# OpenDriveLab/kai0

Measured on AMD Instinct MI355X. Metric: train samples/sec pi0.5 full FT, higher is better.
Workload: dtype bf16; 1 GPU; pi0.5 full fine-tune bf16, batch 32 per MI355X, 3-cam 224x224 (BASELINE.json configs[1]); global_batch=32, seq_len=1018, parallelism=dp1

## Files before the change

### include/kai0hip.h

```cpp
#ifndef KAI0HIP_H
#define KAI0HIP_H

#include <stdint.h>

#ifdef __cplusplus
extern "C" {
#endif

typedef void* kai0_stream_t;

const char* kai0_last_error(void);
int kai0_abi_version(void);
int kai0_device_info(int device, int* n_cu, int* lds_bytes, char* arch_name64);

typedef struct kai0_gemm_desc {
    const void* A;
    const void* B;
    void* C;
    int32_t M, N, K;
    int32_t a_kc, b_kc;
    int64_t lda, ldb, ldc;
    int32_t batch, batch_inner;
    int64_t sA1, sA2, sB1, sB2, sC1, sC2;
    int32_t a_rpb, b_rpb, c_rpb, _pad0;
    int64_t a_bs, a_off, b_bs, b_off, c_bs, c_off;
    const void* bias;
    int32_t bias_f32;
    float scale;
    int32_t act;
    int32_t out_f32;
    void* pre_out;
    const void* gate;
    int32_t gate_rpb;
    int32_t accumulate;
    int64_t gate_ld;
    const void* residual;
    int64_t ldr;
    int64_t sR1, sR2;
    int32_t split_k;
    int32_t c_nontemporal;
    void* workspace;
    int64_t workspace_bytes;
    const void* aux1;
    const void* aux2;
    int32_t nseg, _pad2;
    struct {
        void* dst;
        int64_t ld;
        int32_t n_begin, _pad;
    } seg[3];
    const float* rowvec;
    int64_t rv_s1, rv_s2, rv_ld;
    const void* B2;
    void* pre_out2;
    void* norm_out;
    const void* norm_w;
    const void* norm_b;
    float norm_eps;
    int32_t norm_kind;
    const void* rope_cos;
    const void* rope_sin;
    int32_t rope_half, rope_n_end;
    int32_t persist, general_epilogue, small_w8, _pad3;
} kai0_gemm_desc;

int kai0_gemm_bf16(const kai0_gemm_desc* d, kai0_stream_t stream);
int kai0_gemm_desc_size(void);

#define KAI0_GEMM_LOOP_PLAIN2 0
#define KAI0_GEMM_LOOP_PLAIN4 1
#define KAI0_GEMM_LOOP_QUADRANT 2
#define KAI0_GEMM_LOOP_RING 3
#define KAI0_GEMM_LOOP_PERSISTENT 4
typedef struct kai0_gemm_plan_t {
    int32_t tile;
    int32_t waves;
    int32_t loop;
    int32_t tiles_m, tiles_n;
    int32_t k_chunk;
    int32_t simple_epilogue;
    int32_t _pad;
} kai0_gemm_plan_t;
int kai0_gemm_plan(const kai0_gemm_desc* d, kai0_gemm_plan_t* out);
int kai0_gemm_plan_size(void);

typedef struct kai0_skinny_seg {
    void* dst;
    int64_t ld;
    int32_t n_begin, n_end;
    int32_t rope, _pad;
} kai0_skinny_seg;

typedef struct kai0_skinny_desc {
    const void* A;
    const void* W;
    int64_t lda, ldw;
    int32_t M, N, K;
    int32_t pair_stride, mode, split_k;
    int32_t a_rpb, c_rpb;
    int64_t a_bs, a_off, c_bs, c_off;
    kai0_skinny_seg seg[3];
    int32_t nseg, gate_rpb;
    const void* gate;
    int64_t gate_ld;
    const void* residual;
    int64_t ldr;
    const float* rope_cos;
    const float* rope_sin;
    int32_t rope_half;
    int32_t w_packed;
    void* workspace;
    int64_t workspace_bytes;
    const float* mod;
    int64_t mod_ld;
    int32_t mod_rpb;
    float eps;
    const float* rowsq_in;
    const float* cvec;
    int32_t rowsq_parts, _pad2;
    int64_t rowsq_ld;
    float* rowsq_out;
    int64_t rowsq_out_ld;
} kai0_skinny_desc;

int kai0_gemm_skinny_bf16(const kai0_skinny_desc* d, kai0_stream_t stream);
int kai0_skinny_desc_size(void);
int64_t kai0_skinny_workspace_bytes(int M, int N, int split_k);
int kai0_attn_decode(const void* Q, const void* K, const void* Vt, void* O, const int32_t* qcode, const int32_t* kcode,
                     int batch, int rows, int H, int HD, int Sk, int q0, int64_t q_bs, int64_t k_bs, int64_t k_ld,
                     int k_rows, int64_t vt_bs, int64_t vt_ld, int64_t qcode_ld, int64_t kcode_ld, float scale,
                     void* workspace, int64_t workspace_bytes, kai0_stream_t stream);
int kai0_attn_bwd_dq(const void* dO, const void* O, const void* P, const void* K, const void* V, void* dS, void* dQ, int batch,
                     int rows, int Sk, int HD, int64_t ldo, int64_t ldk, int64_t ldv, int64_t ldp, int64_t sO, int64_t sK,
                     int64_t sV, int64_t sP, float scale, kai0_stream_t stream);
typedef struct kai0_attn_bwd_desc {
    const void* dO; const void* O; const void* Q; const void* K; const void* V;
    const float* lse; const int32_t* qcode; const int32_t* kcode;
    void* P; void* dS; void* dQ;
    int32_t batch, rows, Sk, HD, H, _pad0;
    int64_t ldo, ldk, ldv, ldp, sO, sK, sV, sP, s_lse, qcode_ld, kcode_ld;
    float scale; int32_t _pad1;
} kai0_attn_bwd_desc;
int kai0_attn_bwd_dq2(const kai0_attn_bwd_desc* d, kai0_stream_t stream);
int kai0_attn_bwd_desc_size(void);
int64_t kai0_attn_decode_workspace_bytes(int batch, int rows);
int kai0_transpose_strided_bf16(const void* src, void* dst, int R, int C, int64_t src_ld, int64_t dst_ld, int batch,
                                int64_t src_bs, int64_t dst_bs, kai0_stream_t stream);

int kai0_rope_table(const int32_t* pos, const float* inv_freq, void* cos_out, void* sin_out, int64_t rows, int half, int out_bf16,
                    kai0_stream_t stream);
int kai0_prefix_codes(const void* const* img_masks, int ncam, const void* lang_mask, int B, int n_img, int T, int Hs, int32_t* qcode,
                      int32_t* kcode, int32_t* pos, kai0_stream_t stream);
int kai0_prefix_state_codes(const void* const* img_masks, int ncam, const void* lang_mask, int B, int n_img, int T, int n_state, int Hs,
                            int32_t* qcode, int32_t* kcode, int32_t* pos, kai0_stream_t stream);

int kai0_gemm_f32(const float* A, int64_t sam, int64_t sak, const float* B, int64_t sbk, int64_t sbn,
                  float* C, int64_t ldc, int M, int N, int K, const float* bias, int accumulate, int split_k,
                  void* workspace, int64_t workspace_bytes, kai0_stream_t stream);
int64_t kai0_gemm_f32_workspace_bytes(int M, int N, int split_k);

int kai0_linear_rows_f32(const float* x, const float* W, const float* bias, float* out, int64_t ldo, int M, int N, int K,
                         kai0_stream_t stream);

int kai0_rmsnorm_fwd(const void* x, const float* w, void* y, float* rstd, int64_t rows, int D, float eps,
                     kai0_stream_t stream);
int kai0_rmsnorm_bwd(const void* dy, const void* x, const float* w, const float* rstd, void* dx,
                     float* dw_partial, int dw_blocks, const void* dres, int64_t rows, int D, kai0_stream_t stream);
int kai0_adarms_fwd(const void* x, const float* mod, void* y, void* gate_out, float* rstd, int64_t rows,
                    int rows_per_batch, int D, float eps, kai0_stream_t stream);
int kai0_adarms_bwd(const void* dy, const void* dgate, const void* x, const float* mod, const float* rstd,
                    void* dx, float* dmod, const void* dres, int64_t rows, int rows_per_batch, int D,
                    kai0_stream_t stream);
int kai0_adarms_combine(const float* partials, int splits, int64_t split_stride, const void* gate_prev,
                        const void* residual, void* x_out, const float* mod, void* y, void* gate_out, int64_t rows,
                        int rows_per_batch, int D, float eps, kai0_stream_t stream);
int kai0_layernorm_fwd(const void* x, const void* w, const void* b, void* y, float* mean, float* rstd,
                       int64_t rows, int D, float eps, kai0_stream_t stream);
int kai0_layernorm_bwd(const void* dy, const void* x, const void* w, const float* mean, const float* rstd,
                       void* dx, float* dwb_partial, int dwb_blocks, const void* dres, int64_t rows, int D,
                       kai0_stream_t stream);
int kai0_reduce_partials(const float* partial, int blocks, int ncols, int64_t ld, void* out, int out_f32,
                         kai0_stream_t stream);
typedef struct kai0_reduce_item {
    const float* partial;
    void* out;
    int64_t ld;
    int32_t blocks, ncols;
    int32_t out_f32, _pad;
} kai0_reduce_item;
int kai0_reduce_partials_batch(const kai0_reduce_item* items, int n, kai0_stream_t stream);
int kai0_colsum_partials_bf16(const void* dy, int64_t M, int N, int64_t ld, float* scratch, int scratch_blocks,
                              int* blocks_used, kai0_stream_t stream);
int kai0_colsum_bf16(const void* dy, int64_t M, int N, int64_t ld, float* scratch, int scratch_blocks,
                     void* out, int out_f32, kai0_stream_t stream);

int kai0_rope_inplace(void* x, const int32_t* pos, const float* inv_freq, int B, int S, int64_t s_ld_rows,
                      int64_t row0, int H, int HD, int inverse, kai0_stream_t stream);
int kai0_rope_inplace2(void* x, int H, void* x2, int H2, const int32_t* pos, const float* inv_freq, int B, int S,
                       int64_t s_ld_rows, int64_t row0, int HD, kai0_stream_t stream);
int kai0_rope_copy(const void* src, void* dst, const int32_t* pos, const float* inv_freq, int B, int S, int H, int HD,
                   int64_t src_bs, int64_t src_ld, int64_t dst_bs, int64_t dst_ld, int64_t pos_bs, int inverse,
                   kai0_stream_t stream);

int kai0_softmax_mask_fwd(const void* scores, void* probs, const int32_t* qcode, const int32_t* kcode,
                          int B, int Sq, int H, int Sk, int64_t ld, int64_t batch_stride, int q0,
                          int64_t qcode_ld, int64_t kcode_ld, kai0_stream_t stream);
int kai0_siglip_attn_bwd(const void* q, const void* k, const void* v, const void* dO, const void* O, const void* P,
                         void* dq, void* dk, void* dv, int n_img, int S, int NH, int HD, int64_t ldp, int64_t ld_grad,
                         float scale, kai0_stream_t stream);
int kai0_siglip_attn_fwd(const void* q, const void* k, const void* v, void* o, float* lse, int n_img, int S, int NH, int HD,
                         int64_t ldq, int64_t ldk, int64_t ldv, int64_t ldo, int64_t sq, int64_t sk, int64_t sv, int64_t so,
                         float scale, kai0_stream_t stream);
int kai0_siglip_attn_bwd2(const void* q, const void* k, const void* v, const void* dO, const void* O, const float* lse,
                          void* dq, void* dk, void* dv, int n_img, int S, int NH, int HD, int64_t ld_grad, float scale,
                          kai0_stream_t stream);
int kai0_rowdot_bf16(const void* a, const void* b, float* out, int64_t rows, int D, kai0_stream_t stream);
int kai0_softmax_bwd(const void* probs, const void* dprobs, int dprobs_f32, void* dscores, int64_t rows, int Sk,
                     int64_t ld, float scale, kai0_stream_t stream);

typedef struct kai0_attn_desc {
    const void* Q; const void* K; const void* V; void* O; void* P;
    const int32_t* qcode; const int32_t* kcode;
    int32_t rows, Sk, HD, H, q0, batch, batch_inner, _pad0;
    int64_t ldq, ldk, ldv, ldo, ldp;
    int64_t sQ1, sQ2, sK1, sK2, sV1, sV2, sO1, sO2, sP;
    int64_t qcode_ld, kcode_ld;
    float scale;
    int32_t online;
    float* lse;
    int64_t s_lse;
} kai0_attn_desc;
int kai0_attn_fwd(const kai0_attn_desc* d, kai0_stream_t stream);
int kai0_attn_combine(const void* o_parts, const float* lse_parts, void* O, int parts, int rows, int HD, int64_t ldo,
                      int64_t part_stride, int64_t lse_stride, kai0_stream_t stream);
// ... 113 lines not shown
```

### kai0_amd/_lib.py

```python

from __future__ import annotations

import ctypes as C
import os
import pathlib

_HERE = pathlib.Path(__file__).resolve().parent
LIB_PATH = _HERE / "lib" / "libkai0hip.so"
ABI_VERSION = 2

c_p = C.c_void_p
c_i = C.c_int
c_i64 = C.c_int64
c_f = C.c_float


class GemmSeg(C.Structure):
    _fields_ = [("dst", c_p), ("ld", c_i64), ("n_begin", C.c_int32), ("_pad", C.c_int32)]


class GemmDesc(C.Structure):

    _fields_ = [
        ("A", c_p), ("B", c_p), ("C", c_p),
        ("M", C.c_int32), ("N", C.c_int32), ("K", C.c_int32),
        ("a_kc", C.c_int32), ("b_kc", C.c_int32),
        ("lda", c_i64), ("ldb", c_i64), ("ldc", c_i64),
        ("batch", C.c_int32), ("batch_inner", C.c_int32),
        ("sA1", c_i64), ("sA2", c_i64), ("sB1", c_i64), ("sB2", c_i64), ("sC1", c_i64), ("sC2", c_i64),
        ("a_rpb", C.c_int32), ("b_rpb", C.c_int32), ("c_rpb", C.c_int32), ("_pad0", C.c_int32),
        ("a_bs", c_i64), ("a_off", c_i64), ("b_bs", c_i64), ("b_off", c_i64), ("c_bs", c_i64), ("c_off", c_i64),
        ("bias", c_p), ("bias_f32", C.c_int32), ("scale", c_f),
        ("act", C.c_int32), ("out_f32", C.c_int32),
        ("pre_out", c_p), ("gate", c_p), ("gate_rpb", C.c_int32), ("accumulate", C.c_int32),
        ("gate_ld", c_i64), ("residual", c_p), ("ldr", c_i64), ("sR1", c_i64), ("sR2", c_i64),
        ("split_k", C.c_int32), ("c_nontemporal", C.c_int32), ("workspace", c_p), ("workspace_bytes", c_i64),
        ("aux1", c_p), ("aux2", c_p),
        ("nseg", C.c_int32), ("_pad2", C.c_int32), ("seg", GemmSeg * 3),
        ("rowvec", c_p), ("rv_s1", c_i64), ("rv_s2", c_i64), ("rv_ld", c_i64),
        ("B2", c_p), ("pre_out2", c_p),
        ("norm_out", c_p), ("norm_w", c_p), ("norm_b", c_p), ("norm_eps", C.c_float), ("norm_kind", C.c_int32),
        ("rope_cos", c_p), ("rope_sin", c_p), ("rope_half", C.c_int32), ("rope_n_end", C.c_int32),
        ("persist", C.c_int32), ("general_epilogue", C.c_int32), ("small_w8", C.c_int32), ("_pad3", C.c_int32),
    ]


class GemmPlan(C.Structure):

    _fields_ = [("tile", C.c_int32), ("waves", C.c_int32), ("loop", C.c_int32), ("tiles_m", C.c_int32), ("tiles_n", C.c_int32),
                ("k_chunk", C.c_int32), ("simple_epilogue", C.c_int32), ("_pad", C.c_int32)]


GEMM_LOOPS = ("plain2", "plain4", "quadrant", "ring", "persistent")


class AttnDesc(C.Structure):

    _fields_ = [
        ("Q", c_p), ("K", c_p), ("V", c_p), ("O", c_p), ("P", c_p), ("qcode", c_p), ("kcode", c_p),
        ("rows", C.c_int32), ("Sk", C.c_int32), ("HD", C.c_int32), ("H", C.c_int32), ("q0", C.c_int32),
        ("batch", C.c_int32), ("batch_inner", C.c_int32), ("_pad0", C.c_int32),
        ("ldq", c_i64), ("ldk", c_i64), ("ldv", c_i64), ("ldo", c_i64), ("ldp", c_i64),
        ("sQ1", c_i64), ("sQ2", c_i64), ("sK1", c_i64), ("sK2", c_i64), ("sV1", c_i64), ("sV2", c_i64),
        ("sO1", c_i64), ("sO2", c_i64), ("sP", c_i64), ("qcode_ld", c_i64), ("kcode_ld", c_i64),
        ("scale", c_f), ("online", C.c_int32), ("lse", c_p), ("s_lse", c_i64),
    ]


class AttnBwdDesc(C.Structure):

    _fields_ = [
        ("dO", c_p), ("O", c_p), ("Q", c_p), ("K", c_p), ("V", c_p), ("lse", c_p), ("qcode", c_p), ("kcode", c_p),
        ("P", c_p), ("dS", c_p), ("dQ", c_p),
        ("batch", C.c_int32), ("rows", C.c_int32), ("Sk", C.c_int32), ("HD", C.c_int32), ("H", C.c_int32), ("_pad0", C.c_int32),
        ("ldo", c_i64), ("ldk", c_i64), ("ldv", c_i64), ("ldp", c_i64), ("sO", c_i64), ("sK", c_i64), ("sV", c_i64), ("sP", c_i64),
        ("s_lse", c_i64), ("qcode_ld", c_i64), ("kcode_ld", c_i64),
        ("scale", c_f), ("_pad1", C.c_int32),
    ]


class SkinnySeg(C.Structure):
    _fields_ = [("dst", c_p), ("ld", c_i64), ("n_begin", C.c_int32), ("n_end", C.c_int32), ("rope", C.c_int32),
                ("_pad", C.c_int32)]


class ReduceItem(C.Structure):

    _fields_ = [("partial", c_p), ("out", c_p), ("ld", c_i64), ("blocks", C.c_int32), ("ncols", C.c_int32),
                ("out_f32", C.c_int32), ("_pad", C.c_int32)]


class PackPart(C.Structure):

    _fields_ = [("src", c_p), ("dst", c_p), ("src_bs", c_i64), ("src_ld", c_i64), ("dst_bs", c_i64), ("dst_ld", c_i64),
                ("B", C.c_int32), ("rows", C.c_int32), ("cols", C.c_int32), ("mode", C.c_int32), ("pos_off", C.c_int32),
                ("_pad", C.c_int32)]


class SkinnyDesc(C.Structure):

    _fields_ = [
        ("A", c_p), ("W", c_p), ("lda", c_i64), ("ldw", c_i64),
        ("M", C.c_int32), ("N", C.c_int32), ("K", C.c_int32),
        ("pair_stride", C.c_int32), ("mode", C.c_int32), ("split_k", C.c_int32),
        ("a_rpb", C.c_int32), ("c_rpb", C.c_int32),
        ("a_bs", c_i64), ("a_off", c_i64), ("c_bs", c_i64), ("c_off", c_i64),
        ("seg", SkinnySeg * 3), ("nseg", C.c_int32), ("gate_rpb", C.c_int32),
        ("gate", c_p), ("gate_ld", c_i64), ("residual", c_p), ("ldr", c_i64),
        ("rope_cos", c_p), ("rope_sin", c_p), ("rope_half", C.c_int32), ("w_packed", C.c_int32),
        ("workspace", c_p), ("workspace_bytes", c_i64),
        ("mod", c_p), ("mod_ld", c_i64), ("mod_rpb", C.c_int32), ("eps", c_f),
        ("rowsq_in", c_p), ("cvec", c_p), ("rowsq_parts", C.c_int32), ("_pad2", C.c_int32), ("rowsq_ld", c_i64),
        ("rowsq_out", c_p), ("rowsq_out_ld", c_i64),
    ]


_PROTOS: dict[str, list] = {
    "kai0_abi_version": [],
    "kai0_gemm_desc_size": [],
    "kai0_device_info": [c_i, C.POINTER(c_i), C.POINTER(c_i), C.c_char_p],
    "kai0_gemm_bf16": [C.POINTER(GemmDesc), c_p],
    "kai0_gemm_plan": [C.POINTER(GemmDesc), C.POINTER(GemmPlan)],
    "kai0_gemm_plan_size": [],
    "kai0_attn_fwd": [C.POINTER(AttnDesc), c_p],
    "kai0_attn_desc_size": [],
    "kai0_attn_combine": [c_p, c_p, c_p, c_i, c_i, c_i, c_i64, c_i64, c_i64, c_p],
    "kai0_attn_bwd_dq2": [C.POINTER(AttnBwdDesc), c_p],
    "kai0_attn_bwd_desc_size": [],
    "kai0_siglip_attn_fwd": [c_p, c_p, c_p, c_p, c_p, c_i, c_i, c_i, c_i, c_i64, c_i64, c_i64, c_i64, c_i64, c_i64, c_i64, c_i64, c_f, c_p],
    "kai0_siglip_attn_bwd2": [c_p, c_p, c_p, c_p, c_p, c_p, c_p, c_p, c_p, c_i, c_i, c_i, c_i, c_i64, c_f, c_p],
    "kai0_gemm_skinny_bf16": [C.POINTER(SkinnyDesc), c_p],
    "kai0_skinny_desc_size": [],
    "kai0_attn_decode": [c_p, c_p, c_p, c_p, c_p, c_p, c_i, c_i, c_i, c_i, c_i, c_i, c_i64, c_i64, c_i64, c_i, c_i64, c_i64,
                         c_i64, c_i64, c_f, c_p, c_i64, c_p],
    "kai0_attn_bwd_dq": [c_p, c_p, c_p, c_p, c_p, c_p, c_p, c_i, c_i, c_i, c_i, c_i64, c_i64, c_i64, c_i64, c_i64, c_i64, c_i64, c_i64,
                         c_f, c_p],
    "kai0_transpose_strided_bf16": [c_p, c_p, c_i, c_i, c_i64, c_i64, c_i, c_i64, c_i64, c_p],
    "kai0_rope_table": [c_p, c_p, c_p, c_p, c_i64, c_i, c_i, c_p],
    "kai0_prefix_codes": [c_p, c_i, c_p, c_i, c_i, c_i, c_i, c_p, c_p, c_p, c_p],
    "kai0_prefix_state_codes": [c_p, c_i, c_p, c_i, c_i, c_i, c_i, c_i, c_p, c_p, c_p, c_p],
    "kai0_gemm_f32": [c_p, c_i64, c_i64, c_p, c_i64, c_i64, c_p, c_i64, c_i, c_i, c_i, c_p, c_i, c_i, c_p, c_i64, c_p],
    "kai0_linear_rows_f32": [c_p, c_p, c_p, c_p, c_i64, c_i, c_i, c_i, c_p],
    "kai0_rmsnorm_fwd": [c_p, c_p, c_p, c_p, c_i64, c_i, c_f, c_p],
    "kai0_rmsnorm_bwd": [c_p, c_p, c_p, c_p, c_p, c_p, c_i, c_p, c_i64, c_i, c_p],
    "kai0_adarms_fwd": [c_p, c_p, c_p, c_p, c_p, c_i64, c_i, c_i, c_f, c_p],
    "kai0_adarms_combine": [c_p, c_i, c_i64, c_p, c_p, c_p, c_p, c_p, c_p, c_i64, c_i, c_i, c_f, c_p],
    "kai0_adarms_bwd": [c_p, c_p, c_p, c_p, c_p, c_p, c_p, c_p, c_i64, c_i, c_i, c_p],
    "kai0_layernorm_fwd": [c_p, c_p, c_p, c_p, c_p, c_p, c_i64, c_i, c_f, c_p],
    "kai0_layernorm_bwd": [c_p, c_p, c_p, c_p, c_p, c_p, c_p, c_i, c_p, c_i64, c_i, c_p],
    "kai0_reduce_partials": [c_p, c_i, c_i, c_i64, c_p, c_i, c_p],
    "kai0_colsum_bf16": [c_p, c_i64, c_i, c_i64, c_p, c_i, c_p, c_i, c_p],
    "kai0_reduce_partials_batch": [c_p, c_i, c_p],
    "kai0_pack_rows": [c_p, c_i, c_p, c_i64, c_p, c_i, c_p],
    "kai0_sampled_checksum": [c_p, c_i, c_i, c_p, c_p],
    "kai0_colsum_partials_bf16": [c_p, c_i64, c_i, c_i64, c_p, c_i, c_p, c_p],
    "kai0_rope_inplace": [c_p, c_p, c_p, c_i, c_i, c_i64, c_i64, c_i, c_i, c_i, c_p],
    "kai0_rope_inplace2": [c_p, c_i, c_p, c_i, c_p, c_p, c_i, c_i, c_i64, c_i64, c_i, c_p],
    "kai0_rope_copy": [c_p, c_p, c_p, c_p, c_i, c_i, c_i, c_i, c_i64, c_i64, c_i64, c_i64, c_i64, c_i, c_p],
    "kai0_softmax_mask_fwd": [c_p, c_p, c_p, c_p, c_i, c_i, c_i, c_i, c_i64, c_i64, c_i, c_i64, c_i64, c_p],
    "kai0_siglip_attn_bwd": [c_p, c_p, c_p, c_p, c_p, c_p, c_p, c_p, c_p, c_i, c_i, c_i, c_i, c_i64, c_i64, c_f, c_p],
    "kai0_rowdot_bf16": [c_p, c_p, c_p, c_i64, c_i, c_p],
    "kai0_softmax_bwd": [c_p, c_p, c_i, c_p, c_i64, c_i, c_i64, c_f, c_p],
    "kai0_geglu_fwd": [c_p, c_p, c_p, c_i64, c_p],
    "kai0_geglu_bwd": [c_p, c_p, c_p, c_p, c_p, c_i64, c_p],
    "kai0_gelu_bwd": [c_p, c_p, c_p, c_i64, c_p],
    "kai0_silu_fwd_f32": [c_p, c_p, c_i64, c_p],
    "kai0_silu_bwd_f32": [c_p, c_p, c_p, c_i64, c_p],
    "kai0_gated_fwd": [c_p, c_p, c_p, c_p, c_i64, c_i, c_i, c_p],
    "kai0_gated_bwd": [c_p, c_p, c_p, c_p, c_p, c_i64, c_i, c_i, c_p],
    "kai0_embed_gather": [c_p, c_p, c_p, c_i, c_i, c_i, c_f, c_i64, c_i64, c_i64, c_p],
    "kai0_embed_grad": [c_p, c_p, c_p, c_i, c_i, c_i, c_f, c_i64, c_i64, c_i64, c_p],
    "kai0_cast_f32_to_bf16": [c_p, c_p, c_i64, c_p],
    "kai0_cast_bf16_to_f32": [c_p, c_p, c_i64, c_p],
    "kai0_add_bf16": [c_p, c_p, c_p, c_i64, c_p],
    "kai0_add_f32": [c_p, c_p, c_p, c_i64, c_p],
    "kai0_transpose_bf16": [c_p, c_p, c_i, c_i, c_p],
    "kai0_copy_rows_bf16": [c_p, c_p, c_i, c_i, c_i, c_i64, c_i64, c_i64, c_i64, c_i64, c_i64, c_p],
    "kai0_patch_im2col": [c_p, c_p, c_i, c_i, c_i, c_i, c_p],
    "kai0_add_pos_cast": [c_p, c_p, c_p, c_i64, c_i, c_i, c_p],
    "kai0_time_sincos": [c_p, c_p, c_i, c_i, C.c_double, C.c_double, c_p],
    "kai0_flow_mix": [c_p, c_p, c_p, c_p, c_p, c_i, c_i, c_p],
    "kai0_mse_fwd": [c_p, c_p, c_p, c_i64, c_p],
    "kai0_mse_bwd": [c_p, c_p, c_p, c_p, c_i64, c_p],
    "kai0_euler_step": [c_p, c_p, c_f, c_i64, c_p],
    "kai0_denoise_glue": [c_p, c_p, c_i64, c_i, c_f, c_p, c_p, c_p, c_f, c_p, c_p, c_p, c_i64, c_i, c_i, c_p, c_p],
    "kai0_denoise_glue_rows": [c_p, c_p, c_i64, c_i, c_f, c_p, c_p, c_p, c_f, c_p, c_p, c_p, c_i64, c_i, c_i, c_p, c_i, c_i64, c_i64, c_p],
    "kai0_linear_f32_rows": [c_p, c_i64, c_p, c_i64, c_p, c_i, c_i, c_i, c_i, c_p, c_i64, c_p, c_i64, c_i, c_i64, c_i64, c_p, c_i64, c_p],
    "kai0_rtc_error": [c_p, c_p, c_p, c_p, c_i, c_f, c_p, c_i64, c_i, c_i, c_p],
    "kai0_rtc_update": [c_p, c_p, c_p, c_p, c_f, c_f, c_f, c_i64, c_i, c_p],
    "kai0_sumsq": [c_p, c_i, c_i64, c_p, c_p, c_p],
    "kai0_sum_chunks": [c_p, c_i, c_i, c_i64, c_i64, c_p, c_p],
    "kai0_clip_coef": [c_p, c_f, c_p, c_p, c_p],
    "kai0_adamw": [c_p, c_p, c_p, c_p, c_i, c_p, c_i, c_i64, c_f, c_f, c_f, c_f, c_f, c_f, c_f, c_p, c_p],
    "kai0_adamw_rows": [c_p, c_p, c_p, c_p, c_i, c_p, c_i, c_i64, c_i, c_p, c_f, c_f, c_f, c_f, c_f, c_f, c_f, c_p, c_p],
    "kai0_adamw_ema": [c_p, c_p, c_p, c_p, c_p, c_i, c_p, c_i, c_i64, c_f, c_f, c_f, c_f, c_f, c_f, c_f, c_f, c_p, c_p],
    "kai0_adamw_rows_ema": [c_p, c_p, c_p, c_p, c_p, c_i, c_p, c_i, c_i64, c_i, c_p, c_f, c_f, c_f, c_f, c_f, c_f, c_f, c_f, c_p, c_p],
    "kai0_grad_accum": [c_p, c_p, c_i, c_i64, c_i, c_p, c_p, c_p],
    "kai0_mix": [C.POINTER(c_p), c_i, C.POINTER(c_f), c_i, c_p, c_i, c_i64, c_p],
    "kai0_multi_dot": [c_p, c_i, C.POINTER(c_p), c_i, c_i, c_i64, c_p, c_p, c_p],
    "kai0_lora_down": [c_p, c_i64, c_p, c_i64, c_p, c_i64, c_i, c_i, c_i, c_p],
    "kai0_lora_wgrad": [c_p, c_i64, c_p, c_i64, c_p, c_i64, c_i, c_i, c_i, c_f, c_i, c_i, c_p, c_i64, c_p],
    "kai0_frames_to_chw": [c_p, c_p, c_i, c_i, c_i, c_i, c_i, c_i, c_i, c_i, c_i, c_p],
    "kai0_prefix_gather": [c_p, c_p, c_p, c_p, c_i, c_i, c_i, c_i, c_i, c_i64, c_p],
# ... 65 lines not shown
```

### kai0_amd/csrc/gemm_bf16.hip

```cpp
#include "common.h"
#include "../../include/kai0hip.h"
#include <stdlib.h>
#include <algorithm>
#include <atomic>
#include <type_traits>

namespace {

constexpr int BK = 64;

#ifdef KAI0_ABLATE
#define KAI0_ABL(p) ((p).ablate)
#else
#define KAI0_ABL(p) 0
#endif

struct RowMap {
    int32_t rpb;
    int64_t bs, off;
    __device__ __forceinline__ int64_t operator()(int r) const {
        if (rpb == 0) return r;
        const int q = r / rpb;
        return (int64_t)q * bs + (r - q * rpb) + off;
    }
};

struct GemmArgs {
    const bf16_t* A;
    const bf16_t* B;
    void* C;
    int M, N, K;
    int64_t lda, ldb, ldc;
    int batch_inner;
    int64_t sA1, sA2, sB1, sB2, sC1, sC2;
    RowMap amap, bmap, cmap;
    const void* bias;
    int bias_f32;
    float scale;
    int act;
    int out_f32;
    bf16_t* pre_out;
    const bf16_t* aux1;
    const bf16_t* aux2;
    const bf16_t* gate;
    int gate_rpb;
    int accumulate;
    int64_t gate_ld;
    const bf16_t* residual;
    int64_t ldr, sR1, sR2;
    int tiles_m, tiles_n;
    int ablate;
    int nt_c;
    int simple_epi;
    int nt_pre;
    const float* rowvec;
    int64_t rv_s1, rv_s2, rv_ld;
    int nseg;
    bf16_t* seg_dst[3];
    int64_t seg_ld[3];
    int seg_begin[3];
    float* ws;
    int split_k, k_chunk;
    const bf16_t* B2;
    bf16_t* pre_out2;
    bf16_t* norm_out;
    const void* norm_w;
    const bf16_t* norm_b;
    float norm_eps;
    int norm_kind;
    const bf16_t* rope_cos;
    const bf16_t* rope_sin;
    int rope_half, rope_n_end;
};

typedef __attribute__((ext_vector_type(4))) int i32x4_t;
constexpr uint32_t OOB = 0x80000000u;
__device__ __forceinline__ void glds16(__amdgpu_buffer_rsrc_t rsrc, uint32_t voff, char* lds_dst_wave_uniform) {
    __builtin_amdgcn_raw_ptr_buffer_load_lds(rsrc, (LDS_PTR(void))lds_dst_wave_uniform, 16, (int)voff, 0, 0, 0);
}


__device__ __forceinline__ void store_pre8(bf16_t* dst, bf16x8 v, int nt) {
    if (nt) __builtin_nontemporal_store(v, reinterpret_cast<bf16x8*>(dst));
    else *reinterpret_cast<bf16x8*>(dst) = v;
}

__device__ __forceinline__ void epilogue8(const GemmArgs& p, float (&v)[8], int row, int ccol, int64_t cz, int64_t rz,
                                          int64_t vz, void* cbase, bool raw_f32, const bf16x8* res_pre = nullptr) {
    const bool rnd = !raw_f32;
    auto R = [rnd](float x) { return rnd ? rbf(x) : x; };
    const int64_t orow = p.cmap(row);
    if (p.act == 4) {
        const bf16x8 pv = *reinterpret_cast<const bf16x8*>(p.aux1 + cz + orow * p.ldc + ccol);
        const float dsum = p.rowvec[vz + (int64_t)row * p.rv_ld];
        bf16x8 ov;
#pragma unroll
        for (int e = 0; e < 8; ++e) ov[e] = f2bf((bf2f(pv[e]) * (v[e] - dsum)) * p.scale);
        *reinterpret_cast<bf16x8*>(reinterpret_cast<bf16_t*>(cbase) + cz + orow * p.ldc + ccol) = ov;
        return;
    }
    if (p.bias != nullptr) {
        if (p.bias_f32) {
            const float* bp = reinterpret_cast<const float*>(p.bias) + ccol;
#pragma unroll
            for (int e = 0; e < 8; ++e) v[e] += bp[e];
        } else {
            bf16x8 bv = *reinterpret_cast<const bf16x8*>(reinterpret_cast<const bf16_t*>(p.bias) + ccol);
#pragma unroll
            for (int e = 0; e < 8; ++e) v[e] += bf2f(bv[e]);
        }
    }
#pragma unroll
    for (int e = 0; e < 8; ++e) v[e] = R(v[e]);
    if (p.scale != 1.0f) {
#pragma unroll
        for (int e = 0; e < 8; ++e) v[e] = R(v[e] * p.scale);
    }
    if (p.act == 1) {
        if (p.pre_out != nullptr) {
            bf16x8 pv;
#pragma unroll
            for (int e = 0; e < 8; ++e) pv[e] = f2bf(v[e]);
            store_pre8(p.pre_out + cz + orow * p.ldc + ccol, pv, p.nt_pre);
        }
#pragma unroll
        for (int e = 0; e < 8; e += 2) {
            const f32x2 a = gelu_tanh2(f32x2{v[e], v[e + 1]});
            v[e] = R(a[0]);
            v[e + 1] = R(a[1]);
        }
    } else if (p.act == 2) {
        if (p.pre_out != nullptr) {
            bf16x8 uv;
#pragma unroll
            for (int e = 0; e < 8; ++e) uv[e] = f2bf(v[e]);
            *reinterpret_cast<bf16x8*>(p.pre_out + cz + orow * p.ldc + ccol) = uv;
        }
        const bf16x8 gv = *reinterpret_cast<const bf16x8*>(p.aux1 + cz + orow * p.ldc + ccol);
#pragma unroll
        for (int e = 0; e < 8; e += 2) {
            const f32x2 a = gelu_tanh2(f32x2{bf2f(gv[e]), bf2f(gv[e + 1])});
            v[e] = R(R(a[0]) * v[e]);
            v[e + 1] = R(R(a[1]) * v[e + 1]);
        }
    } else if (p.act == 3) {
        const bf16x8 gv = *reinterpret_cast<const bf16x8*>(p.aux1 + cz + orow * p.ldc + ccol);
        const bf16x8 uv = *reinterpret_cast<const bf16x8*>(p.aux2 + cz + orow * p.ldc + ccol);
        bf16x8 du;
#pragma unroll
        for (int e = 0; e < 8; e += 2) {
            f32x2 gl, gr;
            gelu_tanh_both2(f32x2{bf2f(gv[e]), bf2f(gv[e + 1])}, gl, gr);
            du[e] = f2bf(v[e] * R(gl[0]));
            du[e + 1] = f2bf(v[e + 1] * R(gl[1]));
            v[e] = R(R(v[e] * bf2f(uv[e])) * gr[0]);
            v[e + 1] = R(R(v[e + 1] * bf2f(uv[e + 1])) * gr[1]);
        }
        *reinterpret_cast<bf16x8*>(p.pre_out + cz + orow * p.ldc + ccol) = du;
    } else if (p.act == 5) {
        const bf16x8 pv = *reinterpret_cast<const bf16x8*>(p.aux1 + cz + orow * p.ldc + ccol);
#pragma unroll
        for (int e = 0; e < 8; e += 2) {
            f32x2 gl, gr;
            gelu_tanh_both2(f32x2{bf2f(pv[e]), bf2f(pv[e + 1])}, gl, gr);
            v[e] = R(v[e] * gr[0]);
            v[e + 1] = R(v[e + 1] * gr[1]);
        }
    }
    if (p.gate != nullptr) {
        bf16x8 gv = *reinterpret_cast<const bf16x8*>(p.gate + (int64_t)(row / p.gate_rpb) * p.gate_ld + ccol);
#pragma unroll
        for (int e = 0; e < 8; ++e) v[e] = R(v[e] * bf2f(gv[e]));
    }
    if (p.residual != nullptr) {
        bf16x8 rv = res_pre != nullptr ? *res_pre : *reinterpret_cast<const bf16x8*>(p.residual + rz + orow * p.ldr + ccol);
#pragma unroll
        for (int e = 0; e < 8; ++e) v[e] = R(v[e] + bf2f(rv[e]));
    }
    if (raw_f32) {
        float* cp = reinterpret_cast<float*>(cbase) + cz + orow * p.ldc + ccol;
        if (p.accumulate) {
            f32x4 o0 = *reinterpret_cast<const f32x4*>(cp);
            f32x4 o1 = *reinterpret_cast<const f32x4*>(cp + 4);
#pragma unroll
            for (int e = 0; e < 4; ++e) { v[e] += o0[e]; v[4 + e] += o1[e]; }
        }
        *reinterpret_cast<f32x4*>(cp) = f32x4{v[0], v[1], v[2], v[3]};
        *reinterpret_cast<f32x4*>(cp + 4) = f32x4{v[4], v[5], v[6], v[7]};
    } else {
        bf16_t* cp = reinterpret_cast<bf16_t*>(cbase) + cz + orow * p.ldc + ccol;
        if (p.nseg > 0) {
            int si = 0;
            if (p.nseg > 1 && ccol >= p.seg_begin[1]) si = 1;
            if (p.nseg > 2 && ccol >= p.seg_begin[2]) si = 2;
            cp = p.seg_dst[si] + orow * p.seg_ld[si] + (ccol - p.seg_begin[si]);
        }
        if (p.accumulate) {
            bf16x8 ov = *reinterpret_cast<const bf16x8*>(cp);
#pragma unroll
            for (int e = 0; e < 8; ++e) v[e] += bf2f(ov[e]);
        }
        bf16x8 ov;
#pragma unroll
        for (int e = 0; e < 8; ++e) ov[e] = f2bf(v[e]);
        store_pre8(cp, ov, p.nt_c);
    }
}

#define N_ALIGNED8(n) (((n) & 7) == 0)

#define SIMPLE_EPILOGUE_APPLIES(simple_epi, act, split_k, gate, out_f32, scale, c_rpb, n) \
    ((simple_epi) && (act) <= 1 && (split_k) == 1 && (gate) == nullptr && !(out_f32) && (scale) == 1.0f && (c_rpb) == 0 && (N_ALIGNED8(n)))

__device__ __forceinline__ void lds_barrier() {
    __builtin_amdgcn_sched_barrier(0);
    asm volatile("s_waitcnt lgkmcnt(0)" ::: "memory");
    __builtin_amdgcn_s_barrier();
    asm volatile("" ::: "memory");
    __builtin_amdgcn_sched_barrier(0);
}

template <bool A_KC, bool B_KC, int WM, int WN, int MT, int NT, bool PP, int NS = 2, int BKT = 64, int SCH = 0>
__global__ __launch_bounds__(WM * WN * 64, (WM * WN * 64) / 256) void gemm_bf16_kernel(const GemmArgs p) {
    static_assert(PP ? (WM == 2 && WN == 4 && MT == 8 && ((SCH == 1 && NS == 2 && BKT == 64) || (SCH == 3 && NS == 4 && BKT == 32)))
                     : (SCH == 0 && NS >= 2 && BKT == 64),
                  "K loops: plain multi-stage (SCH 0, 64 deep), quadrant (SCH 1: 256x256x64, 2 stages), ring (SCH 3: 256x256x32, 4 slots)");
    constexpr int BK = BKT;
    constexpr int NWAVES = WM * WN;
    constexpr int TBM = WM * MT * 16, TBN = WN * NT * 16;
    constexpr int A_TILE = TBM * BK * 2, B_TILE = TBN * BK * 2;
    constexpr int STAGE = A_TILE + B_TILE;
    constexpr int NA = A_TILE / 1024 / NWAVES;
    constexpr int NB = B_TILE / 1024 / NWAVES;
    constexpr int KC_CPR = BK / 8;
    constexpr int KC_RPP = 64 / KC_CPR;
    constexpr int A_ROWB = TBM * 2, B_ROWB = TBN * 2;
    constexpr int A_LPR = A_ROWB / 16, B_LPR = B_ROWB / 16;
    constexpr int A_RPP = 64 / A_LPR, B_RPP = 64 / B_LPR;
    constexpr int GROUP = TBM == 128 ? 8 : 4;
    static_assert(NA >= 1 && NB >= 1 && NT == 4 && ((MT % 4) == 0 || MT == 2), "unsupported tile configuration");
    constexpr int AH = MT >= 4 ? 4 : MT;
    static_assert(A_KC || (64 % A_LPR) == 0, "contraction-strided A needs a power-of-two tile height");
    extern __shared__ __attribute__((aligned(16))) char smem[];

    const int tid = threadIdx.x;
    const int lane = tid & 63;
    const int wave = __builtin_amdgcn_readfirstlane(tid >> 6);
    const int wm = wave / WN, wn = wave % WN;
    if constexpr (MT <= 4) {
        asm volatile("" ::"s"(p.A), "s"(p.B), "s"(p.M), "s"(p.N), "s"(p.K), "s"(p.lda), "s"(p.ldb), "s"(p.tiles_m), "s"(p.tiles_n),
                     "s"(p.split_k), "s"(p.k_chunk), "s"(p.batch_inner), "s"(p.amap.rpb), "s"(p.bmap.rpb), "s"(p.act), "s"(p.sA1),
                     "s"(p.sB1), "s"(p.sA2), "s"(p.sB2));
    }
    const int nwg = gridDim.x;
    int pid = blockIdx.x;
    {
        const int q = nwg >> 3, r = nwg & 7;
        const int xcd = pid & 7, idx = pid >> 3;
        pid = (xcd < r ? xcd * (q + 1) : r * (q + 1) + (xcd - r) * q) + idx;
    }
    int tile_m, tile_n;
    {
        const int width = GROUP * p.tiles_n;
        const int group = pid / width;
        const int first_m = group * GROUP;
        const int gsz = min(p.tiles_m - first_m, GROUP);
        const int in_g = pid - group * width;
        tile_m = first_m + in_g % gsz;
        tile_n = in_g / gsz;
    }
    const int ks_id = blockIdx.y % p.split_k;
    const int z = blockIdx.y / p.split_k;
    const int kbeg = ks_id * p.k_chunk;
    const int kend = min(p.K, kbeg + p.k_chunk);
    const int z1 = z / p.batch_inner, z2 = z - z1 * p.batch_inner;
    const bf16_t* __restrict__ Ab = p.A + z1 * p.sA1 + z2 * p.sA2;
    const bf16_t* __restrict__ Bb = p.B + z1 * p.sB1 + z2 * p.sB2;
    const int m0 = tile_m * TBM, n0 = tile_n * TBN;
    const __amdgpu_buffer_rsrc_t a_rsrc = __builtin_amdgcn_make_buffer_rsrc((void*)Ab, 0, (int)OOB, 0x00020000);
    const __amdgpu_buffer_rsrc_t b_rsrc = __builtin_amdgcn_make_buffer_rsrc((void*)Bb, 0, (int)OOB, 0x00020000);
    const bool pair = p.act == 6;
    const __amdgpu_buffer_rsrc_t b2_rsrc = __builtin_amdgcn_make_buffer_rsrc((void*)(pair ? p.B2 : Bb), 0, (int)OOB, 0x00020000);

    uint32_t a_off[NA], b_off[NB];
    const int kc_chunk = BK == 64 ? ((lane & 7) ^ (lane >> 3)) * 8 : ((lane & 3) ^ (((lane >> 2) & 8) ? 3 : 0)) * 8;
    if constexpr (A_KC) {
#pragma unroll
        for (int j = 0; j < NA; ++j) {
            const int R = m0 + (wave * NA + j) * KC_RPP + lane / KC_CPR;
            a_off[j] = R < p.M ? (uint32_t)((p.amap(R) * p.lda + kc_chunk) * 2) : OOB;
        }
    } else {
#pragma unroll
        for (int j = 0; j < NA; ++j) {
            const int r = (wave * NA + j) * A_RPP + lane / A_LPR;
            const int key = (r & 3) | (((r >> 3) & 1) << 2);
            const int col = m0 + ((lane % A_LPR) ^ (key << 1)) * 8;
            a_off[j] = col < p.M ? (uint32_t)(col * 2) : OOB;
        }
    }
    if constexpr (B_KC) {
#pragma unroll
        for (int j = 0; j < NB; ++j) {
            const int rt = (wave * NB + j) * KC_RPP + lane / KC_CPR;
            int R = n0 + rt;
            bool ok = R < p.N;
            if (pair) {
                R = (n0 >> 1) + ((rt >> 6) << 5) + (rt & 31);
                ok = R < (p.N >> 1);
            }
            b_off[j] = ok ? (uint32_t)((p.bmap(R) * p.ldb + kc_chunk) * 2) : OOB;
        }
    } else {
#pragma unroll
        for (int j = 0; j < NB; ++j) {
            const int r = (wave * NB + j) * B_RPP + lane / B_LPR;
            const int key = (r & 3) | (((r >> 3) & 1) << 2);
            const int col = n0 + ((lane % B_LPR) ^ (key << 1)) * 8;
            b_off[j] = col < p.N ? (uint32_t)(col * 2) : OOB;
        }
    }
    const uint32_t lda2 = (uint32_t)p.lda * 2, ldb2 = (uint32_t)p.ldb * 2;

    auto stage = [&](int kt, int slot) {
        char* sa = smem + slot * STAGE + wave * (NA * 1024);
        char* sb = smem + slot * STAGE + A_TILE + wave * (NB * 1024);
        const int k0 = kbeg + kt * BK;
        const bool kc_in = (k0 + kc_chunk) < kend;
#pragma unroll
        for (int j = 0; j < NA; ++j) {
            uint32_t off;
            if constexpr (A_KC) {
                off = kc_in ? a_off[j] + (uint32_t)k0 * 2 : OOB;
            } else {
                const int kr = k0 + (wave * NA + j) * A_RPP + lane / A_LPR;
                off = kr < kend ? a_off[j] + (uint32_t)p.amap(kr) * lda2 : OOB;
            }
            glds16(a_rsrc, off, sa + j * 1024);
        }
#pragma unroll
        for (int j = 0; j < NB; ++j) {
            uint32_t off;
            if constexpr (B_KC) {
                off = kc_in ? b_off[j] + (uint32_t)k0 * 2 : OOB;
            } else {
                const int kr = k0 + (wave * NB + j) * B_RPP + lane / B_LPR;
                off = kr < kend ? b_off[j] + (uint32_t)p.bmap(kr) * ldb2 : OOB;
            }
            glds16((B_KC && BK == 64 && pair && (((wave * NB + j) * KC_RPP) & 32)) ? b2_rsrc : b_rsrc, off, sb + j * 1024);
        }
    };

    auto piece_off = [&](int kt, int idx) -> uint32_t {
        const int k0 = kbeg + kt * BK;
        const bool kc_in = (k0 + kc_chunk) < kend;
        if (idx < NA) {
            if constexpr (A_KC) {
                return kc_in ? a_off[idx] + (uint32_t)k0 * 2 : OOB;
            } else {
                const int kr = k0 + (wave * NA + idx) * A_RPP + lane / A_LPR;
                return kr < kend ? a_off[idx] + (uint32_t)p.amap(kr) * lda2 : OOB;
            }
        } else {
            const int j = idx - NA;
            if constexpr (B_KC) {
                return kc_in ? b_off[j] + (uint32_t)k0 * 2 : OOB;
            } else {
                const int kr = k0 + (wave * NB + j) * B_RPP + lane / B_LPR;
                return kr < kend ? b_off[j] + (uint32_t)p.bmap(kr) * ldb2 : OOB;
            }
        }
    };
    auto piece_issue = [&](uint32_t off, int slot, int idx) {
        if (idx < NA) glds16(a_rsrc, off, smem + slot * STAGE + wave * (NA * 1024) + idx * 1024);
        else glds16(b_rsrc, off, smem + slot * STAGE + A_TILE + wave * (NB * 1024) + (idx - NA) * 1024);
    };
// ... 105 lines not shown
                    hb_lds[x] = h * 16384 + q * 1024;
                    hb_kr[x] = r;
                    hb_off[x] = col < p.N ? (uint32_t)(col * 2) : OOB;
                }
            }
        auto issue_half = [&](bool isb, int h, int t) {
            const int k0 = kbeg + t * BK;
            const bool kc_in = (k0 + kc_chunk) < kend;
            char* base = smem + (t & 1) * STAGE + (isb ? A_TILE : 0);
#pragma unroll
            for (int j = 0; j < 2; ++j) {
                const int x = h * 2 + j;
                const uint32_t o = isb ? hb_off[x] : ha_off[x];
                uint32_t off = OOB;
                if (isb ? B_KC : A_KC) {
                    if (kc_in && o != OOB) off = o + (uint32_t)k0 * 2;
                } else {
                    const int kr = k0 + (isb ? hb_kr[x] : ha_kr[x]);
                    if (kr < kend && o != OOB) off = o + (uint32_t)(isb ? p.bmap(kr) : p.amap(kr)) * (isb ? ldb2 : lda2);
                }
                if (KAI0_ABL(p) == 1) off = OOB;
                glds16(isb ? ((pair && h == 1) ? b2_rsrc : b_rsrc) : a_rsrc, off, base + (isb ? hb_lds[x] : ha_lds[x]));
            }
        };
        issue_half(false, 0, 0);
        issue_half(true, 1, 0);
        issue_half(true, 0, 0);
        issue_half(false, 1, 0);
        issue_half(false, 0, 1);
        issue_half(true, 1, 1);
        asm volatile("s_waitcnt vmcnt(6)" ::: "memory");
        lds_barrier();
        if (grp == 1) lds_barrier();
        bf16x8 af[4][2], bq[2][2];
        auto read_a = [&](const char* ta, int h) {
#pragma unroll
            for (int i = 0; i < 4; ++i)
#pragma unroll
                for (int ks = 0; ks < 2; ++ks)
                    af[i][ks] = A_KC ? load_frag(ta, true, A_ROWB, wm * 128 + (h * 4 + i) * 16, ks)
                                     : load_frag(ta + h * 16384, false, 256, wm * 64 + i * 16, ks);
        };
        auto read_b = [&](const char* tb, int h) {
#pragma unroll
            for (int j = 0; j < 2; ++j)
#pragma unroll
                for (int ks = 0; ks < 2; ++ks)
                    bq[j][ks] = B_KC ? load_frag(tb, true, B_ROWB, wn * 64 + (h * 2 + j) * 16, ks)
                                     : load_frag(tb + h * 16384, false, 256, wn * 32 + j * 16, ks);
        };
        auto quad = [&](auto ahc, auto bhc) {
            constexpr int ah = decltype(ahc)::value, bh = decltype(bhc)::value;
            __builtin_amdgcn_s_setprio(1);
#pragma unroll
            for (int ks = 0; ks < 2; ++ks)
#pragma unroll
                for (int i = 0; i < 4; ++i)
#pragma unroll
                    for (int j = 0; j < 2; ++j)
                        acc[ah * 4 + i][bh * 2 + j] =
                            __builtin_amdgcn_mfma_f32_16x16x32_bf16(af[i][ks], bq[j][ks], acc[ah * 4 + i][bh * 2 + j], 0, 0, 0);
            __builtin_amdgcn_s_setprio(0);
        };
        using I0 = std::integral_constant<int, 0>;
        using I1 = std::integral_constant<int, 1>;
        for (int t = 0; t < nk; ++t) {
            const char* ta = smem + (t & 1) * STAGE;
            const char* tb = ta + A_TILE;
            read_b(tb, 0);
            __builtin_amdgcn_sched_barrier(0);
            read_a(ta, 0);
            __builtin_amdgcn_sched_barrier(0);
            issue_half(true, 0, t + 1);
            lds_barrier();
            quad(I0{}, I0{});
            lds_barrier();
            read_b(tb, 1);
            __builtin_amdgcn_sched_barrier(0);
            issue_half(false, 1, t + 1);
            asm volatile("s_waitcnt vmcnt(8)" ::: "memory");
            lds_barrier();
            quad(I0{}, I1{});
            lds_barrier();
            read_a(ta, 1);
            __builtin_amdgcn_sched_barrier(0);
            issue_half(false, 0, t + 2);
            lds_barrier();
            quad(I1{}, I1{});
            lds_barrier();
            read_b(tb, 0);
            __builtin_amdgcn_sched_barrier(0);
            issue_half(true, 1, t + 2);
            asm volatile("s_waitcnt vmcnt(6)" ::: "memory");
            lds_barrier();
            quad(I1{}, I0{});
            lds_barrier();
        }
        asm volatile("s_waitcnt vmcnt(0)" ::: "memory");
        if (grp == 0) lds_barrier();
        lds_barrier();
    } else {
#pragma unroll
        for (int st = 0; st < NS - 1; ++st)
            if (st < nk) stage(st, st);
        int slot_c = 0, slot_p = NS - 1;
        for (int kt = 0; kt < nk; ++kt) {
            if constexpr (NS == 2) {
                asm volatile("s_waitcnt vmcnt(0)" ::: "memory");
            } else {
                if (kt + NS - 2 < nk) asm volatile("s_waitcnt vmcnt(%0)" ::"n"((NS - 2) * (NA + NB)) : "memory");
                else asm volatile("s_waitcnt vmcnt(0)" ::: "memory");
            }
            lds_barrier();
            if (kt + NS - 1 < nk && KAI0_ABL(p) != 1) stage(kt + NS - 1, slot_p);
            const char* ta = smem + slot_c * STAGE;
            const char* tb = ta + A_TILE;
    #pragma unroll
            for (int ks = 0; ks < BK / 32; ++ks) {
                bf16x8 bfr[NT];
    #pragma unroll
                for (int t = 0; t < NT; ++t) bfr[t] = load_frag(tb, B_KC, B_ROWB, wn * (NT * 16) + t * 16, ks);
    #pragma unroll
                for (int h = 0; h < MT / AH; ++h) {
                    bf16x8 af[AH];
    #pragma unroll
                    for (int t = 0; t < AH; ++t) af[t] = load_frag(ta, A_KC, A_ROWB, wm * (MT * 16) + (h * AH + t) * 16, ks);
    #pragma unroll
                    for (int i = 0; i < AH; ++i)
    #pragma unroll
                        for (int j = 0; j < NT; ++j)
                            acc[h * AH + i][j] = __builtin_amdgcn_mfma_f32_16x16x32_bf16(af[i], bfr[j], acc[h * AH + i][j], 0, 0, 0);
                }
            }
            slot_c = slot_c + 1 == NS ? 0 : slot_c + 1;
            slot_p = slot_p + 1 == NS ? 0 : slot_p + 1;
        }
        lds_barrier();
    }

    float* slab = reinterpret_cast<float*>(smem + wave * (AH * 4096));
    const int64_t cz = z1 * p.sC1 + z2 * p.sC2;
    const int64_t rz = z1 * p.sR1 + z2 * p.sR2;
    const int64_t vz = z1 * p.rv_s1 + z2 * p.rv_s2;
    constexpr bool ILM = SCH == 1 && !A_KC, ILN = SCH == 1 && !B_KC;
    const int ccol = ILN ? n0 + ((lane & 7) >> 2) * 128 + wn * 32 + ((lane & 7) & 3) * 8 : n0 + wn * 64 + (lane & 7) * 8;
    auto row_base = [&](int h) { return ILM ? m0 + h * 128 + wm * 64 : m0 + wm * (MT * 16) + h * 64; };
    const bool col_ok = ccol < ((p.N + 7) & ~7);
    const bool fused_fast = p.act >= 2 && p.split_k == 1 && p.bias == nullptr && p.gate == nullptr && p.residual == nullptr &&
                            !p.accumulate && !p.out_f32 && p.nseg == 0 && (p.act == 4 || p.scale == 1.0f) &&
                            (p.act != 3 || p.pre_out != nullptr);
    const bool plain_fast = p.act <= 1 && p.split_k == 1 && (p.bias != nullptr || p.residual != nullptr) && p.gate == nullptr &&
                            !p.accumulate && !p.out_f32 && p.nseg == 0 && (N_ALIGNED8(p.N));
    const bool simple_fast = MT == 8 && SIMPLE_EPILOGUE_APPLIES(p.simple_epi, p.act, p.split_k, p.gate, p.out_f32, p.scale, p.cmap.rpb, p.N);
    auto epi_half = [&](auto hc) {
        constexpr int h = decltype(hc)::value;
        if constexpr (((MT == 4 && WM == 2) || (MT == 2 && WM == 4)) && WN == 2 && A_KC && B_KC) if (p.act == 7) {
            const bool rot = n0 < p.rope_n_end;
            const int fi = ((n0 >> 7) & 1) * 64 + (lane & 7) * 8;
            const int rcol = rot ? (n0 >> 8) * 256 + wn * 128 + fi : n0 + wn * 64 + (lane & 7) * 8;
            const int rbase = row_base(h) + (lane >> 3);
            bf16x8 cs[AH * 2], sn[AH * 2];
#pragma unroll
            for (int it = 0; it < AH * 2; ++it) {
                const int64_t tr = (int64_t)min(rbase + it * 8, p.M - 1) * p.rope_half + fi;
                cs[it] = *reinterpret_cast<const bf16x8*>(p.rope_cos + (rot ? tr : 0));
                sn[it] = *reinterpret_cast<const bf16x8*>(p.rope_sin + (rot ? tr : 0));
            }
#pragma unroll
            for (int i = 0; i < AH; ++i)
#pragma unroll
                for (int j = 0; j < 4; ++j)
#pragma unroll
                    for (int r = 0; r < 4; ++r) slab[(i * 16 + 4 * g + r) * 64 + j * 16 + l15] = acc[i][j][r];
            lds_barrier();
            const float* pslab = reinterpret_cast<const float*>(smem + (wave ^ 1) * (AH * 4096));
            int si = 0;
            if (p.nseg > 1 && rcol >= p.seg_begin[1]) si = 1;
            if (p.nseg > 2 && rcol >= p.seg_begin[2]) si = 2;
            const bool rcol_ok = rcol < p.N;
#pragma unroll
            for (int it = 0; it < AH * 2; ++it) {
                const int lr = it * 8 + (lane >> 3);
                const int row = rbase + it * 8;
                const int so = lr * 64 + (lane & 7) * 8;
                const f32x4 v0 = *reinterpret_cast<const f32x4*>(slab + so), v1 = *reinterpret_cast<const f32x4*>(slab + so + 4);
                const f32x4 w0 = *reinterpret_cast<const f32x4*>(pslab + so), w1 = *reinterpret_cast<const f32x4*>(pslab + so + 4);
                if (row >= p.M || !rcol_ok) continue;
                const float x[8] = {v0[0], v0[1], v0[2], v0[3], v1[0], v1[1], v1[2], v1[3]};
                const float y[8] = {w0[0], w0[1], w0[2], w0[3], w1[0], w1[1], w1[2], w1[3]};
                bf16x8 ov;
#pragma unroll
                for (int e = 0; e < 8; ++e) {
                    const float xe = rbf(x[e]), ye = rbf(y[e]);
                    const float c = bf2f(cs[it][e]), sv = bf2f(sn[it][e]);
                    ov[e] = rot ? f2bf(rbf(xe * c) + rbf((wn == 0 ? -ye : ye) * sv)) : f2bf(xe);
                }
                const int64_t orow = p.cmap(row);
                bf16_t* cp = p.nseg > 0 ? p.seg_dst[si] + orow * p.seg_ld[si] + (rcol - p.seg_begin[si])
                                        : reinterpret_cast<bf16_t*>(p.C) + cz + orow * p.ldc + rcol;
                *reinterpret_cast<bf16x8*>(cp) = ov;
            }
            return;
        }
        if constexpr (MT != 2) if (pair) {
#pragma unroll
            for (int i = 0; i < 4; ++i)
#pragma unroll
                for (int j = 0; j < 4; ++j)
#pragma unroll
                    for (int r = 0; r < 4; ++r) slab[(i * 16 + 4 * g + r) * 64 + j * 16 + l15] = acc[h * 4 + i][j][r];
            asm volatile("s_waitcnt lgkmcnt(0)" ::: "memory");
            __builtin_amdgcn_wave_barrier();
            const int ocol = (n0 >> 1) + wn * 32 + (lane & 3) * 8;
            const bool ocol_ok = ocol < (p.N >> 1);
            bf16_t* cb = reinterpret_cast<bf16_t*>(p.C);
#pragma unroll
            for (int it = 0; it < 4; ++it) {
                const int lr = it * 16 + (lane >> 2);
                const int row = row_base(h) + lr;
                const float* sp = slab + lr * 64 + (lane & 3) * 8;
                const f32x4 g0 = *reinterpret_cast<const f32x4*>(sp), g1 = *reinterpret_cast<const f32x4*>(sp + 4);
                const f32x4 u0 = *reinterpret_cast<const f32x4*>(sp + 32), u1 = *reinterpret_cast<const f32x4*>(sp + 36);
                if (row >= p.M || !ocol_ok) continue;
                const float gv[8] = {g0[0], g0[1], g0[2], g0[3], g1[0], g1[1], g1[2], g1[3]};
                const float uv[8] = {u0[0], u0[1], u0[2], u0[3], u1[0], u1[1], u1[2], u1[3]};
                bf16x8 gb, ub, hb;
#pragma unroll
                for (int e = 0; e < 8; e += 2) {
                    const f32x2 gr = rbf2(f32x2{gv[e], gv[e + 1]}), ur = rbf2(f32x2{uv[e], uv[e + 1]});
                    const f32x2 hv = rbf2(gelu_tanh2(gr)) * ur;
                    gb[e] = f2bf(gr[0]);
                    gb[e + 1] = f2bf(gr[1]);
                    ub[e] = f2bf(ur[0]);
                    ub[e + 1] = f2bf(ur[1]);
                    hb[e] = f2bf(hv[0]);
                    hb[e + 1] = f2bf(hv[1]);
                }
                const int64_t o = cz + p.cmap(row) * p.ldc + ocol;
                *reinterpret_cast<bf16x8*>(cb + o) = hb;
                if (p.pre_out != nullptr) store_pre8(p.pre_out + o, gb, p.nt_pre);
                if (p.pre_out2 != nullptr) store_pre8(p.pre_out2 + o, ub, p.nt_pre);
            }
            asm volatile("s_waitcnt lgkmcnt(0)" ::: "memory");
            __builtin_amdgcn_wave_barrier();
            return;
        }
        if constexpr (MT != 2) if (fused_fast) {
            bf16x8 s0[8], s1[8];
            float ds[8];
            const int rbase = row_base(h) + (lane >> 3);
#pragma unroll
            for (int it = 0; it < 8; ++it) {
                const int row = rbase + it * 8;
                s0[it] = bf16x8{};
                s1[it] = bf16x8{};
                ds[it] = 0.f;
                if (row < p.M && col_ok) {
                    const int64_t o = cz + p.cmap(row) * p.ldc + ccol;
                    s0[it] = *reinterpret_cast<const bf16x8*>(p.aux1 + o);
                    if (p.act == 3) s1[it] = *reinterpret_cast<const bf16x8*>(p.aux2 + o);
                    if (p.act == 4) ds[it] = p.rowvec[vz + (int64_t)row * p.rv_ld];
                }
            }
#pragma unroll
            for (int i = 0; i < 4; ++i)
#pragma unroll
                for (int j = 0; j < 4; ++j)
#pragma unroll
                    for (int r = 0; r < 4; ++r) slab[(i * 16 + 4 * g + r) * 64 + j * 16 + l15] = acc[h * 4 + i][j][r];
            asm volatile("s_waitcnt lgkmcnt(0)" ::: "memory");
            __builtin_amdgcn_wave_barrier();
            bf16_t* cb = reinterpret_cast<bf16_t*>(p.C);
#pragma unroll
            for (int it = 0; it < 8; ++it) {
                const int row = rbase + it * 8;
                const float* sp = slab + (it * 8 + (lane >> 3)) * 64 + (lane & 7) * 8;
                const f32x4 v0 = *reinterpret_cast<const f32x4*>(sp);
                const f32x4 v1 = *reinterpret_cast<const f32x4*>(sp + 4);
                const float v[8] = {v0[0], v0[1], v0[2], v0[3], v1[0], v1[1], v1[2], v1[3]};
                if (row >= p.M || !col_ok) continue;
                const int64_t o = cz + p.cmap(row) * p.ldc + ccol;
                bf16x8 ov;
                if (p.act == 2) {
                    if (p.pre_out != nullptr) {
                        bf16x8 uv;
#pragma unroll
                        for (int e = 0; e < 8; ++e) uv[e] = f2bf(v[e]);
                        *reinterpret_cast<bf16x8*>(p.pre_out + o) = uv;
                    }
#pragma unroll
                    for (int e = 0; e < 8; e += 2) {
                        const f32x2 r = rbf2(gelu_tanh2(f32x2{bf2f(s0[it][e]), bf2f(s0[it][e + 1])})) * rbf2(f32x2{v[e], v[e + 1]});
                        ov[e] = f2bf(r[0]);
                        ov[e + 1] = f2bf(r[1]);
                    }
                } else if (p.act == 3) {
                    bf16x8 du;
#pragma unroll
                    for (int e = 0; e < 8; e += 2) {
                        const f32x2 dh = rbf2(f32x2{v[e], v[e + 1]});
                        f32x2 gl, gr;
                        gelu_tanh_both2(f32x2{bf2f(s0[it][e]), bf2f(s0[it][e + 1])}, gl, gr);
                        const f32x2 a = dh * rbf2(gl);
                        const f32x2 b = rbf2(dh * f32x2{bf2f(s1[it][e]), bf2f(s1[it][e + 1])}) * gr;
                        du[e] = f2bf(a[0]);
                        du[e + 1] = f2bf(a[1]);
                        ov[e] = f2bf(b[0]);
                        ov[e + 1] = f2bf(b[1]);
                    }
                    *reinterpret_cast<bf16x8*>(p.pre_out + o) = du;
                } else if (p.act == 5) {
#pragma unroll
                    for (int e = 0; e < 8; e += 2) {
                        f32x2 gl, gr;
                        gelu_tanh_both2(f32x2{bf2f(s0[it][e]), bf2f(s0[it][e + 1])}, gl, gr);
                        const f32x2 b = rbf2(f32x2{v[e], v[e + 1]}) * gr;
                        ov[e] = f2bf(b[0]);
                        ov[e + 1] = f2bf(b[1]);
                    }
                } else {
#pragma unroll
                    for (int e = 0; e < 8; ++e) ov[e] = f2bf((bf2f(s0[it][e]) * (v[e] - ds[it])) * p.scale);
                }
                *reinterpret_cast<bf16x8*>(cb + o) = ov;
            }
            asm volatile("s_waitcnt lgkmcnt(0)" ::: "memory");
            __builtin_amdgcn_wave_barrier();
            return;
        }
        if constexpr (MT <= 4) if (plain_fast) {
            float bv[8] = {0.f, 0.f, 0.f, 0.f, 0.f, 0.f, 0.f, 0.f};
            if (p.bias != nullptr && col_ok) {
                if (p.bias_f32) {
                    const f32x4 b0 = *reinterpret_cast<const f32x4*>(reinterpret_cast<const float*>(p.bias) + ccol);
                    const f32x4 b1 = *reinterpret_cast<const f32x4*>(reinterpret_cast<const float*>(p.bias) + ccol + 4);
#pragma unroll
                    for (int e = 0; e < 4; ++e) { bv[e] = b0[e]; bv[4 + e] = b1[e]; }
                } else {
                    const bf16x8 b = *reinterpret_cast<const bf16x8*>(reinterpret_cast<const bf16_t*>(p.bias) + ccol);
#pragma unroll
                    for (int e = 0; e < 8; ++e) bv[e] = bf2f(b[e]);
                }
            }
            bf16x8 rs[AH * 2];
            const int rbase = row_base(h) + (lane >> 3);
#pragma unroll
            for (int it = 0; it < AH * 2; ++it) {
                const int row = rbase + it * 8;
                rs[it] = bf16x8{};
                if (p.residual != nullptr && row < p.M && col_ok) rs[it] = *reinterpret_cast<const bf16x8*>(p.residual + rz + p.cmap(row) * p.ldr + ccol);
            }
#pragma unroll
            for (int i = 0; i < AH; ++i)
#pragma unroll
                for (int j = 0; j < 4; ++j)
#pragma unroll
                    for (int r = 0; r < 4; ++r) slab[(i * 16 + 4 * g + r) * 64 + j * 16 + l15] = acc[h * AH + i][j][r];
            asm volatile("s_waitcnt lgkmcnt(0)" ::: "memory");
            __builtin_amdgcn_wave_barrier();
            bf16_t* cb = reinterpret_cast<bf16_t*>(p.C);
#pragma unroll
            for (int it = 0; it < AH * 2; ++it) {
                const int row = rbase + it * 8;
                const float* sp = slab + (it * 8 + (lane >> 3)) * 64 + (lane & 7) * 8;
                const f32x4 v0 = *reinterpret_cast<const f32x4*>(sp);
                const f32x4 v1 = *reinterpret_cast<const f32x4*>(sp + 4);
                if (row >= p.M || !col_ok) continue;
                float v[8] = {v0[0], v0[1], v0[2], v0[3], v1[0], v1[1], v1[2], v1[3]};
                const int64_t o = cz + p.cmap(row) * p.ldc + ccol;
#pragma unroll
                for (int e = 0; e < 8; ++e) v[e] = rbf(v[e] + bv[e]);
                if (p.scale != 1.0f) {
#pragma unroll
                    for (int e = 0; e < 8; ++e) v[e] = rbf(v[e] * p.scale);
                }
                if (p.act == 1) {
                    if (p.pre_out != nullptr) {
                        bf16x8 pv;
#pragma unroll
                        for (int e = 0; e < 8; ++e) pv[e] = f2bf(v[e]);
                        store_pre8(p.pre_out + o, pv, p.nt_pre);
                    }
#pragma unroll
                    for (int e = 0; e < 8; e += 2) {
                        const f32x2 a = gelu_tanh2(f32x2{v[e], v[e + 1]});
                        v[e] = rbf(a[0]);
                        v[e + 1] = rbf(a[1]);
                    }
                }
                if (p.residual != nullptr) {
#pragma unroll
                    for (int e = 0; e < 8; ++e) v[e] = rbf(v[e] + bf2f(rs[it][e]));
                }
                bf16x8 ov;
#pragma unroll
                for (int e = 0; e < 8; ++e) ov[e] = f2bf(v[e]);
                *reinterpret_cast<bf16x8*>(cb + o) = ov;
            }
            asm volatile("s_waitcnt lgkmcnt(0)" ::: "memory");
            __builtin_amdgcn_wave_barrier();
            return;
        }
        if constexpr (MT == 8) if (simple_fast) {
            const bool has_bias = p.bias != nullptr, has_res = p.residual != nullptr, gelu = p.act == 1;
            const int M_ = p.M, nt_pre_ = p.nt_pre, nt_c_ = p.nt_c;
            const bf16_t* res_ = p.residual;
            bf16_t* pre_ = p.pre_out;
            const int64_t ldr_ = p.ldr, ldc_ = p.ldc;
            float bv[8] = {0.f, 0.f, 0.f, 0.f, 0.f, 0.f, 0.f, 0.f};
            if (has_bias && col_ok) {
                if (p.bias_f32) {
                    const f32x4 b0 = *reinterpret_cast<const f32x4*>(reinterpret_cast<const float*>(p.bias) + ccol);
                    const f32x4 b1 = *reinterpret_cast<const f32x4*>(reinterpret_cast<const float*>(p.bias) + ccol + 4);
#pragma unroll
                    for (int e = 0; e < 4; ++e) { bv[e] = b0[e]; bv[4 + e] = b1[e]; }
                } else {
                    const bf16x8 b = *reinterpret_cast<const bf16x8*>(reinterpret_cast<const bf16_t*>(p.bias) + ccol);
#pragma unroll
                    for (int e = 0; e < 8; ++e) bv[e] = bf2f(b[e]);
                }
            }
            bf16_t* cl = reinterpret_cast<bf16_t*>(p.C) + cz + ccol;
            int64_t ldl = p.ldc;
            if (p.nseg > 0) {
                cl = p.seg_dst[0] + (ccol - p.seg_begin[0]);
                ldl = p.seg_ld[0];
                if (p.nseg > 1 && ccol >= p.seg_begin[1]) {
                    cl = p.seg_dst[1] + (ccol - p.seg_begin[1]);
                    ldl = p.seg_ld[1];
                }
                if (p.nseg > 2 && ccol >= p.seg_begin[2]) {
                    cl = p.seg_dst[2] + (ccol - p.seg_begin[2]);
                    ldl = p.seg_ld[2];
                }
            }
            const int rbase = row_base(h) + (lane >> 3);
            auto res_row = [&](int it) -> bf16x8 {
                const int row = rbase + it * 8;
                return (has_res && row < M_ && col_ok) ? *reinterpret_cast<const bf16x8*>(res_ + rz + (int64_t)row * ldr_ + ccol) : bf16x8{};
            };
            const bool accum = p.accumulate != 0;
            auto old_row = [&](int it) -> bf16x8 {
                const int row = rbase + it * 8;
                return (accum && row < M_ && col_ok) ? *reinterpret_cast<const bf16x8*>(cl + (int64_t)row * ldl) : bf16x8{};
            };
            bf16x8 rnext = res_row(0), onext = old_row(0);
#pragma unroll
            for (int i = 0; i < 4; ++i)
#pragma unroll
                for (int j = 0; j < 4; ++j)
#pragma unroll
                    for (int r = 0; r < 4; ++r) slab[(i * 16 + 4 * g + r) * 64 + j * 16 + l15] = acc[h * 4 + i][j][r];
            asm volatile("s_waitcnt lgkmcnt(0)" ::: "memory");
            __builtin_amdgcn_wave_barrier();
#pragma unroll
            for (int it = 0; it < 8; ++it) {
                const int row = rbase + it * 8;
                const float* sp = slab + (it * 8 + (lane >> 3)) * 64 + (lane & 7) * 8;
                const f32x4 v0 = *reinterpret_cast<const f32x4*>(sp);
                const f32x4 v1 = *reinterpret_cast<const f32x4*>(sp + 4);
                const bf16x8 rv = rnext, ov0 = onext;
                if (it + 1 < 8) {
                    rnext = res_row(it + 1);
                    onext = old_row(it + 1);
                }
                if (row >= M_ || !col_ok) continue;
                float v[8] = {v0[0], v0[1], v0[2], v0[3], v1[0], v1[1], v1[2], v1[3]};
                if (has_bias) {
#pragma unroll
                    for (int e = 0; e < 8; ++e) v[e] += bv[e];
                }
#pragma unroll
                for (int e = 0; e < 8; ++e) v[e] = rbf(v[e]);
                if (gelu) {
                    if (pre_ != nullptr) {
                        bf16x8 pv;
#pragma unroll
                        for (int e = 0; e < 8; ++e) pv[e] = f2bf(v[e]);
                        store_pre8(pre_ + cz + (int64_t)row * ldc_ + ccol, pv, nt_pre_);
                    }
#pragma unroll
                    for (int e = 0; e < 8; e += 2) {
                        const f32x2 a = gelu_tanh2(f32x2{v[e], v[e + 1]});
                        v[e] = rbf(a[0]);
                        v[e + 1] = rbf(a[1]);
                    }
                }
                if (has_res) {
#pragma unroll
                    for (int e = 0; e < 8; ++e) v[e] = rbf(v[e] + bf2f(rv[e]));
                }
                if (accum) {
#pragma unroll
                    for (int e = 0; e < 8; ++e) v[e] += bf2f(ov0[e]);
                }
                bf16x8 ov;
#pragma unroll
                for (int e = 0; e < 8; ++e) ov[e] = f2bf(v[e]);
                store_pre8(cl + (int64_t)row * ldl, ov, nt_c_);
            }
            asm volatile("s_waitcnt lgkmcnt(0)" ::: "memory");
            __builtin_amdgcn_wave_barrier();
            return;
        }
#pragma unroll
        for (int i = 0; i < AH; ++i)
#pragma unroll
            for (int j = 0; j < 4; ++j)
#pragma unroll
                for (int r = 0; r < 4; ++r) slab[(i * 16 + 4 * g + r) * 64 + j * 16 + l15] = acc[h * AH + i][j][r];
        asm volatile("s_waitcnt lgkmcnt(0)" ::: "memory");
        __builtin_amdgcn_wave_barrier();
#pragma unroll 1
        for (int it = 0; it < AH * 2; ++it) {
            const int lr = it * 8 + (lane >> 3);
            const int row = row_base(h) + lr;
            if (row >= p.M || !col_ok) continue;
            const float* sp = slab + lr * 64 + (lane & 7) * 8;
            f32x4 v0 = *reinterpret_cast<const f32x4*>(sp);
            f32x4 v1 = *reinterpret_cast<const f32x4*>(sp + 4);
            float v[8] = {v0[0], v0[1], v0[2], v0[3], v1[0], v1[1], v1[2], v1[3]};
            if (p.split_k > 1) {
                float* wp = reinterpret_cast<float*>(p.ws) + ((int64_t)blockIdx.y * p.M + row) * p.N + ccol;
                *reinterpret_cast<f32x4*>(wp) = v0;
                *reinterpret_cast<f32x4*>(wp + 4) = v1;
            } else {
                epilogue8(p, v, row, ccol, cz, rz, vz, p.C, p.out_f32 != 0);
            }
        }
        asm volatile("s_waitcnt lgkmcnt(0)" ::: "memory");
        __builtin_amdgcn_wave_barrier();
    };
    epi_half(std::integral_constant<int, 0>{});
    if constexpr (MT / 4 > 1) epi_half(std::integral_constant<int, 1>{});
    if constexpr (MT / 4 > 2) epi_half(std::integral_constant<int, 2>{});
    static_assert(MT / 4 <= 3, "extend the epilogue parts");
}

constexpr int PS_SLOTS = 1024;
__device__ unsigned int g_ps_ctr[PS_SLOTS][16];

#ifdef KAI0_PS_TRACE
__device__ long long g_ps_trace[256][8];
#define PS_STAMP(i)                                              \
    do {                                                         \
        const long long n_ = __builtin_amdgcn_s_memrealtime();   \
        t_acc[i] += n_ - t_prev;                                 \
        t_prev = n_;                                             \
    } while (0)
#else
#define PS_STAMP(i) do { } while (0)
#endif

__global__ __launch_bounds__(512, 1) void gemm_nt_persistent_kernel(const GemmArgs p, unsigned int* __restrict__ ctr) {
    constexpr int TBM = 256, TBN = 256, A_TILE = TBM * BK * 2, STAGE = 2 * A_TILE, GROUP = 4, MT = 8;
    extern __shared__ __attribute__((aligned(16))) char smem[];
    const int tid = threadIdx.x, lane = tid & 63;
    const int wave = __builtin_amdgcn_readfirstlane(tid >> 6);
    const int wm = wave >> 2, wn = wave & 3, grp = wm;
    const int l15 = lane & 15, g = lane >> 4;
    int* mbox = reinterpret_cast<int*>(smem + 2 * STAGE);
    float* slab = reinterpret_cast<float*>(smem + 2 * STAGE + wave * 4096);
    const int ntile = p.tiles_m * p.tiles_n;
    const int qq = ntile >> 3, rr = ntile & 7;
    const int x0 = blockIdx.x & 7;
    auto draw = [&]() -> unsigned { return __hip_atomic_fetch_add(ctr + x0, 1u, __ATOMIC_RELAXED, __HIP_MEMORY_SCOPE_AGENT); };
    auto resolve = [&](unsigned t) -> int {
        for (int a = 0; a < 8; ++a) {
            const int x = (x0 + a) & 7;
            const int len = qq + (x < rr ? 1 : 0);
            if (a > 0) t = __hip_atomic_fetch_add(ctr + x, 1u, __ATOMIC_RELAXED, __HIP_MEMORY_SCOPE_AGENT);
            if ((int)t < len) return (x < rr ? x * (qq + 1) : rr * (qq + 1) + (x - rr) * qq) + (int)t;
        }
        return -1;
    };
    auto next_ticket = [&]() -> int { return resolve(draw()); };
    const __amdgpu_buffer_rsrc_t a_rsrc = __builtin_amdgcn_make_buffer_rsrc((void*)p.A, 0, (int)OOB, 0x00020000);
    const __amdgpu_buffer_rsrc_t b_rsrc = __builtin_amdgcn_make_buffer_rsrc((void*)p.B, 0, (int)OOB, 0x00020000);
    const bool pair = p.act == 6;
    const __amdgpu_buffer_rsrc_t b2_rsrc = __builtin_amdgcn_make_buffer_rsrc((void*)(pair ? p.B2 : p.B), 0, (int)OOB, 0x00020000);
    const int kc_chunk = ((lane & 7) ^ (lane >> 3)) * 8;
    const int nk = (p.K + BK - 1) / BK;

    const uint32_t lda2 = (uint32_t)p.lda * 2, ldb2 = (uint32_t)p.ldb * 2, kc2 = (uint32_t)kc_chunk * 2;
    auto arow_fix = [](int) -> uint32_t { return 0u; };
    int m0 = 0, n0 = 0;
    uint32_t ha_off[4], hb_off[4];
    int ha_lds[4], hb_lds[4];
#pragma unroll
    for (int h = 0; h < 2; ++h)
#pragma unroll
        for (int j = 0; j < 2; ++j) {
            const int q = 2 * wave + j, x = h * 2 + j;
            ha_lds[x] = ((q >> 3) * 128 + h * 64 + (q & 7) * 8) * 128;
            hb_lds[x] = ((q >> 2) * 64 + h * 32 + (q & 3) * 8) * 128;
        }
    auto setup = [&](int pid) {
        const int width = GROUP * p.tiles_n;
        const int group = pid / width, first_m = group * GROUP;
        const int gsz = min(p.tiles_m - first_m, GROUP);
        const int in_g = pid - group * width;
        m0 = (first_m + in_g % gsz) * TBM;
        n0 = (in_g / gsz) * TBN;
#pragma unroll
        for (int h = 0; h < 2; ++h)
#pragma unroll
            for (int j = 0; j < 2; ++j) {
                const int q = 2 * wave + j, x = h * 2 + j;
                const int Ra = m0 + (q >> 3) * 128 + h * 64 + (q & 7) * 8 + (lane >> 3);
                ha_off[x] = Ra < p.M ? (uint32_t)Ra * lda2 + kc2 + arow_fix(Ra) : OOB;
                int Rb = n0 + (q >> 2) * 64 + h * 32 + (q & 3) * 8 + (lane >> 3);
                bool ok = Rb < p.N;
                if (pair) {
                    Rb = (n0 >> 1) + (q >> 2) * 32 + (q & 3) * 8 + (lane >> 3);
                    ok = Rb < (p.N >> 1);
                }
                hb_off[x] = ok ? (uint32_t)Rb * ldb2 + kc2 : OOB;
            }
    };
    auto issue_half = [&](bool isb, int h, int t) {
        const int k0 = t * BK;
        const bool kc_in = (k0 + kc_chunk) < p.K;
        char* base = smem + (t & 1) * STAGE + (isb ? A_TILE : 0);
#pragma unroll
        for (int j = 0; j < 2; ++j) {
            const int x = h * 2 + j;
            const uint32_t o = isb ? hb_off[x] : ha_off[x];
            const uint32_t off = (kc_in && o != OOB) ? o + (uint32_t)k0 * 2 : OOB;
            glds16(isb ? ((pair && h == 1) ? b2_rsrc : b_rsrc) : a_rsrc, off, base + (isb ? hb_lds[x] : ha_lds[x]));
        }
    };
    auto prologue_issue = [&]() {
        issue_half(false, 0, 0);
        issue_half(true, 1, 0);
        issue_half(true, 0, 0);
        issue_half(false, 1, 0);
        issue_half(false, 0, 1);
        issue_half(true, 1, 1);
    };
    auto frag = [&](const char* tile, int row0, int ks) -> bf16x8 {
        const int row = row0 + l15;
        return *reinterpret_cast<const bf16x8*>(tile + row * 128 + (((ks * 4 + g) ^ (row & 7)) << 4));
    };

    if (tid == 0) {
        const int t0 = next_ticket();
        mbox[0] = t0;
        mbox[1] = t0 >= 0 ? next_ticket() : -1;
    }
    __syncthreads();
    int cur = mbox[0], nxt = mbox[1];
    __syncthreads();
    if (cur >= 0) {
        setup(cur);
        prologue_issue();
        asm volatile("s_waitcnt vmcnt(6)" ::: "memory");
        lds_barrier();
        if (grp == 1) lds_barrier();
    }
    const int64_t cz = 0, rz = 0, vz = 0;
#ifdef KAI0_PS_TRACE
    long long t_acc[5] = {0, 0, 0, 0, 0};
    long long t_prev = __builtin_amdgcn_s_memrealtime();
#endif
    while (cur >= 0) {
        f32x4 acc[MT][4];
#pragma unroll
        for (int i = 0; i < MT; ++i)
#pragma unroll
            for (int j = 0; j < 4; ++j) acc[i][j] = f32x4{0.f, 0.f, 0.f, 0.f};
        bf16x8 af[4][2], bq[2][2];
        auto read_a = [&](const char* ta, int h) {
#pragma unroll
            for (int i = 0; i < 4; ++i)
#pragma unroll
                for (int ks = 0; ks < 2; ++ks) af[i][ks] = frag(ta, wm * 128 + (h * 4 + i) * 16, ks);
        };
        auto read_b = [&](const char* tb, int h) {
#pragma unroll
            for (int j = 0; j < 2; ++j)
#pragma unroll
                for (int ks = 0; ks < 2; ++ks) bq[j][ks] = frag(tb, wn * 64 + (h * 2 + j) * 16, ks);
        };
        auto quad = [&](auto ahc, auto bhc) {
            constexpr int ah = decltype(ahc)::value, bh = decltype(bhc)::value;
            __builtin_amdgcn_s_setprio(1);
#pragma unroll
            for (int ks = 0; ks < 2; ++ks)
#pragma unroll
                for (int i = 0; i < 4; ++i)
#pragma unroll
                    for (int j = 0; j < 2; ++j)
                        acc[ah * 4 + i][bh * 2 + j] =
                            __builtin_amdgcn_mfma_f32_16x16x32_bf16(af[i][ks], bq[j][ks], acc[ah * 4 + i][bh * 2 + j], 0, 0, 0);
            __builtin_amdgcn_s_setprio(0);
        };
        using I0 = std::integral_constant<int, 0>;
        using I1 = std::integral_constant<int, 1>;
        PS_STAMP(0);
        for (int t = 0; t < nk; ++t) {
            const char* ta = smem + (t & 1) * STAGE;
            const char* tb = ta + A_TILE;
            read_b(tb, 0);
            __builtin_amdgcn_sched_barrier(0);
            read_a(ta, 0);
            __builtin_amdgcn_sched_barrier(0);
            issue_half(true, 0, t + 1);
            lds_barrier();
            quad(I0{}, I0{});
            lds_barrier();
            read_b(tb, 1);
            __builtin_amdgcn_sched_barrier(0);
            issue_half(false, 1, t + 1);
            asm volatile("s_waitcnt vmcnt(8)" ::: "memory");
            lds_barrier();
            quad(I0{}, I1{});
            lds_barrier();
            read_a(ta, 1);
            __builtin_amdgcn_sched_barrier(0);
            issue_half(false, 0, t + 2);
            lds_barrier();
            quad(I1{}, I1{});
            lds_barrier();
            read_b(tb, 0);
            __builtin_amdgcn_sched_barrier(0);
            issue_half(true, 1, t + 2);
            asm volatile("s_waitcnt vmcnt(6)" ::: "memory");
            lds_barrier();
            quad(I1{}, I0{});
            lds_barrier();
        }
        asm volatile("s_waitcnt vmcnt(0)" ::: "memory");
        if (grp == 0) lds_barrier();
        lds_barrier();

        PS_STAMP(1);
        const int m0c = m0, n0c = n0;
        int nn = -1;
        unsigned raw = 0;
        if (tid == 0 && nxt >= 0) raw = draw();
        if (nxt >= 0) {
            setup(nxt);
            prologue_issue();
        }
        const int ccol = n0c + wn * 64 + (lane & 7) * 8;
        const bool col_ok = ccol < ((p.N + 7) & ~7);
        const bool fused_fast = p.act >= 2 && p.act <= 5 && p.bias == nullptr && p.gate == nullptr && p.residual == nullptr && !p.accumulate &&
                                !p.out_f32 && p.nseg == 0 && (p.act == 4 || p.scale == 1.0f) && (p.act != 3 || p.pre_out != nullptr);
        const bool simple_fast = SIMPLE_EPILOGUE_APPLIES(p.simple_epi, p.act, p.split_k, p.gate, p.out_f32, p.scale, p.cmap.rpb, p.N);
        auto to_slab = [&](int ti) {
            __builtin_amdgcn_wave_barrier();
#pragma unroll
            for (int j = 0; j < 4; ++j)
#pragma unroll
                for (int r = 0; r < 4; ++r) slab[(4 * g + r) * 64 + j * 16 + l15] = acc[ti][j][r];
            asm volatile("s_waitcnt lgkmcnt(0)" ::: "memory");
            __builtin_amdgcn_wave_barrier();
        };
        if (pair) {
            const int ocol = (n0c >> 1) + wn * 32 + (lane & 3) * 8;
            const bool ocol_ok = ocol < (p.N >> 1);
            bf16_t* cb = reinterpret_cast<bf16_t*>(p.C);
#pragma unroll
            for (int ti = 0; ti < MT; ++ti) {
                to_slab(ti);
                const int row = m0c + wm * 128 + ti * 16 + (lane >> 2);
                const float* sp = slab + (lane >> 2) * 64 + (lane & 3) * 8;
                const f32x4 g0 = *reinterpret_cast<const f32x4*>(sp), g1 = *reinterpret_cast<const f32x4*>(sp + 4);
                const f32x4 u0 = *reinterpret_cast<const f32x4*>(sp + 32), u1 = *reinterpret_cast<const f32x4*>(sp + 36);
                if (row < p.M && ocol_ok) {
                    const float gv[8] = {g0[0], g0[1], g0[2], g0[3], g1[0], g1[1], g1[2], g1[3]};
                    const float uv[8] = {u0[0], u0[1], u0[2], u0[3], u1[0], u1[1], u1[2], u1[3]};
                    bf16x8 gb, ub, hb;
#pragma unroll
                    for (int e = 0; e < 8; e += 2) {
                        const f32x2 gr = rbf2(f32x2{gv[e], gv[e + 1]}), ur = rbf2(f32x2{uv[e], uv[e + 1]});
                        const f32x2 hv = rbf2(gelu_tanh2(gr)) * ur;
                        gb[e] = f2bf(gr[0]); gb[e + 1] = f2bf(gr[1]);
                        ub[e] = f2bf(ur[0]); ub[e + 1] = f2bf(ur[1]);
                        hb[e] = f2bf(hv[0]); hb[e + 1] = f2bf(hv[1]);
                    }
                    const int64_t o = p.cmap(row) * p.ldc + ocol;
                    *reinterpret_cast<bf16x8*>(cb + o) = hb;
                    if (p.pre_out != nullptr) store_pre8(p.pre_out + o, gb, p.nt_pre);
                    if (p.pre_out2 != nullptr) store_pre8(p.pre_out2 + o, ub, p.nt_pre);
                }
            }
        } else if (fused_fast) {
            bf16_t* cb = reinterpret_cast<bf16_t*>(p.C);
#pragma unroll
            for (int h = 0; h < 2; ++h) {
                bf16x8 s0[8], s1[8];
                float ds[8];
                const int rbase = m0c + wm * 128 + h * 64 + (lane >> 3);
#pragma unroll
                for (int it = 0; it < 8; ++it) {
                    const int row = rbase + it * 8;
                    s0[it] = bf16x8{};
                    s1[it] = bf16x8{};
                    ds[it] = 0.f;
                    if (row < p.M && col_ok) {
                        const int64_t o = p.cmap(row) * p.ldc + ccol;
                        s0[it] = *reinterpret_cast<const bf16x8*>(p.aux1 + o);
                        if (p.act == 3) s1[it] = *reinterpret_cast<const bf16x8*>(p.aux2 + o);
                        if (p.act == 4) ds[it] = p.rowvec[(int64_t)row * p.rv_ld];
                    }
                }
#pragma unroll
                for (int i = 0; i < 4; ++i) {
                    to_slab(h * 4 + i);
#pragma unroll
                    for (int it2 = 0; it2 < 2; ++it2) {
                        const int it = 2 * i + it2;
                        const int row = rbase + it * 8;
                        const float* sp = slab + (it2 * 8 + (lane >> 3)) * 64 + (lane & 7) * 8;
                        const f32x4 v0 = *reinterpret_cast<const f32x4*>(sp), v1 = *reinterpret_cast<const f32x4*>(sp + 4);
                        const float v[8] = {v0[0], v0[1], v0[2], v0[3], v1[0], v1[1], v1[2], v1[3]};
                        if (row >= p.M || !col_ok) continue;
                        const int64_t o = p.cmap(row) * p.ldc + ccol;
                        bf16x8 ov;
                        if (p.act == 2) {
                            if (p.pre_out != nullptr) {
                                bf16x8 uv;
#pragma unroll
                                for (int e = 0; e < 8; ++e) uv[e] = f2bf(v[e]);
                                *reinterpret_cast<bf16x8*>(p.pre_out + o) = uv;
                            }
#pragma unroll
                            for (int e = 0; e < 8; e += 2) {
                                const f32x2 r = rbf2(gelu_tanh2(f32x2{bf2f(s0[it][e]), bf2f(s0[it][e + 1])})) * rbf2(f32x2{v[e], v[e + 1]});
                                ov[e] = f2bf(r[0]);
                                ov[e + 1] = f2bf(r[1]);
                            }
                        } else if (p.act == 3) {
                            bf16x8 du;
#pragma unroll
                            for (int e = 0; e < 8; e += 2) {
                                const f32x2 dh = rbf2(f32x2{v[e], v[e + 1]});
                                f32x2 gl, gr;
                                gelu_tanh_both2(f32x2{bf2f(s0[it][e]), bf2f(s0[it][e + 1])}, gl, gr);
                                const f32x2 a = dh * rbf2(gl);
                                const f32x2 b = rbf2(dh * f32x2{bf2f(s1[it][e]), bf2f(s1[it][e + 1])}) * gr;
                                du[e] = f2bf(a[0]); du[e + 1] = f2bf(a[1]);
                                ov[e] = f2bf(b[0]); ov[e + 1] = f2bf(b[1]);
                            }
                            *reinterpret_cast<bf16x8*>(p.pre_out + o) = du;
                        } else if (p.act == 5) {
#pragma unroll
                            for (int e = 0; e < 8; e += 2) {
                                f32x2 gl, gr;
                                gelu_tanh_both2(f32x2{bf2f(s0[it][e]), bf2f(s0[it][e + 1])}, gl, gr);
                                const f32x2 b = rbf2(f32x2{v[e], v[e + 1]}) * gr;
                                ov[e] = f2bf(b[0]); ov[e + 1] = f2bf(b[1]);
                            }
                        } else {
#pragma unroll
                            for (int e = 0; e < 8; ++e) ov[e] = f2bf((bf2f(s0[it][e]) * (v[e] - ds[it])) * p.scale);
                        }
                        *reinterpret_cast<bf16x8*>(cb + o) = ov;
                    }
                }
            }
        } else if (simple_fast) {
            const bool has_bias = p.bias != nullptr, has_res = p.residual != nullptr, gelu = p.act == 1;
            const int M_ = p.M, nt_pre_ = p.nt_pre, nt_c_ = p.nt_c;
            const bf16_t* res_ = p.residual;
            bf16_t* pre_ = p.pre_out;
            const int64_t ldr_ = p.ldr, ldc_ = p.ldc;
            float bv[8] = {0.f, 0.f, 0.f, 0.f, 0.f, 0.f, 0.f, 0.f};
            if (has_bias && col_ok) {
                if (p.bias_f32) {
                    const f32x4 b0 = *reinterpret_cast<const f32x4*>(reinterpret_cast<const float*>(p.bias) + ccol);
                    const f32x4 b1 = *reinterpret_cast<const f32x4*>(reinterpret_cast<const float*>(p.bias) + ccol + 4);
#pragma unroll
                    for (int e = 0; e < 4; ++e) { bv[e] = b0[e]; bv[4 + e] = b1[e]; }
                } else {
                    const bf16x8 b = *reinterpret_cast<const bf16x8*>(reinterpret_cast<const bf16_t*>(p.bias) + ccol);
#pragma unroll
                    for (int e = 0; e < 8; ++e) bv[e] = bf2f(b[e]);
                }
            }
            bf16_t* cl = reinterpret_cast<bf16_t*>(p.C) + ccol;
            int64_t ldl = p.ldc;
            if (p.nseg > 0) {
                cl = p.seg_dst[0] + (ccol - p.seg_begin[0]);
                ldl = p.seg_ld[0];
                if (p.nseg > 1 && ccol >= p.seg_begin[1]) {
                    cl = p.seg_dst[1] + (ccol - p.seg_begin[1]);
                    ldl = p.seg_ld[1];
                }
                if (p.nseg > 2 && ccol >= p.seg_begin[2]) {
                    cl = p.seg_dst[2] + (ccol - p.seg_begin[2]);
                    ldl = p.seg_ld[2];
                }
            }
            const int rbase = m0c + wm * 128 + (lane >> 3);
            auto res_row = [&](int k) -> bf16x8 {
                const int row = rbase + k * 8;
                return (has_res && row < M_ && col_ok) ? *reinterpret_cast<const bf16x8*>(res_ + (int64_t)row * ldr_ + ccol) : bf16x8{};
            };
            const bool accum = p.accumulate != 0;
            auto old_row = [&](int k) -> bf16x8 {
                const int row = rbase + k * 8;
                return (accum && row < M_ && col_ok) ? *reinterpret_cast<const bf16x8*>(cl + (int64_t)row * ldl) : bf16x8{};
            };
            bf16x8 rnext = res_row(0), onext = old_row(0);
#pragma unroll
            for (int ti = 0; ti < MT; ++ti) {
                to_slab(ti);
#pragma unroll
                for (int it2 = 0; it2 < 2; ++it2) {
                    const int k = ti * 2 + it2;
                    const int row = rbase + k * 8;
                    const float* sp = slab + (it2 * 8 + (lane >> 3)) * 64 + (lane & 7) * 8;
                    const f32x4 v0 = *reinterpret_cast<const f32x4*>(sp), v1 = *reinterpret_cast<const f32x4*>(sp + 4);
                    const bf16x8 rv = rnext, ov0 = onext;
                    if (k + 1 < 2 * MT) {
                        rnext = res_row(k + 1);
                        onext = old_row(k + 1);
                    }
                    if (row >= M_ || !col_ok) continue;
                    float v[8] = {v0[0], v0[1], v0[2], v0[3], v1[0], v1[1], v1[2], v1[3]};
                    if (has_bias) {
#pragma unroll
                        for (int e = 0; e < 8; ++e) v[e] += bv[e];
                    }
#pragma unroll
                    for (int e = 0; e < 8; ++e) v[e] = rbf(v[e]);
                    if (gelu) {
                        if (pre_ != nullptr) {
                            bf16x8 pv;
#pragma unroll
                            for (int e = 0; e < 8; ++e) pv[e] = f2bf(v[e]);
                            store_pre8(pre_ + (int64_t)row * ldc_ + ccol, pv, nt_pre_);
                        }
#pragma unroll
                        for (int e = 0; e < 8; e += 2) {
                            const f32x2 a = gelu_tanh2(f32x2{v[e], v[e + 1]});
                            v[e] = rbf(a[0]);
                            v[e + 1] = rbf(a[1]);
                        }
                    }
                    if (has_res) {
#pragma unroll
                        for (int e = 0; e < 8; ++e) v[e] = rbf(v[e] + bf2f(rv[e]));
                    }
                    if (accum) {
#pragma unroll
                        for (int e = 0; e < 8; ++e) v[e] += bf2f(ov0[e]);
                    }
                    bf16x8 ov;
#pragma unroll
                    for (int e = 0; e < 8; ++e) ov[e] = f2bf(v[e]);
                    store_pre8(cl + (int64_t)row * ldl, ov, nt_c_);
                }
            }
        } else {
#pragma unroll
            for (int ti = 0; ti < MT; ++ti) {
                to_slab(ti);
#pragma unroll 1
                for (int it2 = 0; it2 < 2; ++it2) {
                    const int lr = it2 * 8 + (lane >> 3);
                    const int row = m0c + wm * 128 + ti * 16 + lr;
                    if (row >= p.M || !col_ok) continue;
                    const float* sp = slab + lr * 64 + (lane & 7) * 8;
                    const f32x4 v0 = *reinterpret_cast<const f32x4*>(sp), v1 = *reinterpret_cast<const f32x4*>(sp + 4);
                    float v[8] = {v0[0], v0[1], v0[2], v0[3], v1[0], v1[1], v1[2], v1[3]};
                    epilogue8(p, v, row, ccol, cz, rz, vz, p.C, p.out_f32 != 0);
                }
            }
        }
        PS_STAMP(2);
        __builtin_amdgcn_wave_barrier();
        if (tid == 0) mbox[0] = nxt >= 0 ? resolve(raw) : -1;
        asm volatile("s_waitcnt vmcnt(0)" ::: "memory");
        lds_barrier();
        nn = mbox[0];
        cur = nxt;
        nxt = nn;
        lds_barrier();
        if (cur >= 0 && grp == 1) lds_barrier();
        PS_STAMP(3);
#ifdef KAI0_PS_TRACE
        t_acc[4] += 1;
#endif
    }
#ifdef KAI0_PS_TRACE
    if (tid == 0 && blockIdx.x < 256)
        for (int i = 0; i < 5; ++i) g_ps_trace[blockIdx.x][i] = t_acc[i];
#endif
    if (tid == 0) {
        __builtin_amdgcn_fence(__ATOMIC_RELEASE, "agent");
        const unsigned done = __hip_atomic_fetch_add(ctr + 8, 1u, __ATOMIC_RELAXED, __HIP_MEMORY_SCOPE_AGENT);
        if (done == gridDim.x - 1) {
#pragma unroll
            for (int i = 0; i < 9; ++i) __hip_atomic_store(ctr + i, 0u, __ATOMIC_RELAXED, __HIP_MEMORY_SCOPE_AGENT);
        }
    }
}

__global__ __launch_bounds__(256) void splitk_reduce_kernel(const GemmArgs p) {
    const int z = blockIdx.y;
    const int z1 = z / p.batch_inner, z2 = z - z1 * p.batch_inner;
    const int n8 = (p.N + 7) >> 3;
    const int64_t total = (int64_t)p.M * n8;
    const float* w0 = p.ws + (int64_t)z * p.split_k * p.M * p.N;
    const int64_t cz = z1 * p.sC1 + z2 * p.sC2, rz = z1 * p.sR1 + z2 * p.sR2, vz = z1 * p.rv_s1 + z2 * p.rv_s2;
    for (int64_t i = (int64_t)blockIdx.x * 256 + threadIdx.x; i < total; i += (int64_t)gridDim.x * 256) {
        const int row = (int)(i / n8);
        const int col = (int)(i - (int64_t)row * n8) * 8;
        float acc[8] = {0.f, 0.f, 0.f, 0.f, 0.f, 0.f, 0.f, 0.f};
        bf16x8 rpre = {};
        const bool has_res = p.residual != nullptr && p.act != 4;
        if (has_res) rpre = *reinterpret_cast<const bf16x8*>(p.residual + rz + p.cmap(row) * p.ldr + col);
        if (p.split_k <= 8) {
            f32x4 a[8], b[8];
#pragma unroll
            for (int sp = 0; sp < 8; ++sp) {
                const float* wp = w0 + ((int64_t)min(sp, p.split_k - 1) * p.M + row) * p.N + col;
                a[sp] = *reinterpret_cast<const f32x4*>(wp);
                b[sp] = *reinterpret_cast<const f32x4*>(wp + 4);
            }
#pragma unroll
            for (int sp = 0; sp < 8; ++sp) {
                const float m = sp < p.split_k ? 1.0f : 0.0f;
                acc[0] += m * a[sp][0]; acc[1] += m * a[sp][1]; acc[2] += m * a[sp][2]; acc[3] += m * a[sp][3];
                acc[4] += m * b[sp][0]; acc[5] += m * b[sp][1]; acc[6] += m * b[sp][2]; acc[7] += m * b[sp][3];
            }
        } else
        for (int sp = 0; sp < p.split_k; ++sp) {
            const float* wp = w0 + ((int64_t)sp * p.M + row) * p.N + col;
            f32x4 a = *reinterpret_cast<const f32x4*>(wp);
            f32x4 b = *reinterpret_cast<const f32x4*>(wp + 4);
            acc[0] += a[0]; acc[1] += a[1]; acc[2] += a[2]; acc[3] += a[3];
            acc[4] += b[0]; acc[5] += b[1]; acc[6] += b[2]; acc[7] += b[3];
        }
        epilogue8(p, acc, row, col, cz, rz, vz, p.C, p.out_f32 != 0, has_res ? &rpre : nullptr);
    }
}

template <int KIND>
__global__ __launch_bounds__(256) void splitk_reduce_norm_kernel(const GemmArgs p) {
    __shared__ float red[4];
    const int row = blockIdx.x;
    const int n8 = p.N >> 3;
    const bool live = (int)threadIdx.x < n8;
    const int col = min((int)threadIdx.x, n8 - 1) * 8;
    float wv[8], bv[8];
    if constexpr (KIND == 1) {
        const f32x4 w0 = *reinterpret_cast<const f32x4*>(reinterpret_cast<const float*>(p.norm_w) + col);
        const f32x4 w1 = *reinterpret_cast<const f32x4*>(reinterpret_cast<const float*>(p.norm_w) + col + 4);
#pragma unroll
        for (int e = 0; e < 4; ++e) { wv[e] = w0[e]; wv[4 + e] = w1[e]; bv[e] = bv[4 + e] = 0.f; }
    } else {
        const bf16x8 w8 = *reinterpret_cast<const bf16x8*>(reinterpret_cast<const bf16_t*>(p.norm_w) + col);
        const bf16x8 b8 = *reinterpret_cast<const bf16x8*>(p.norm_b + col);
#pragma unroll
        for (int e = 0; e < 8; ++e) { wv[e] = bf2f(w8[e]); bv[e] = bf2f(b8[e]); }
    }
    bf16x8 rpre = {};
    const bool has_res = p.residual != nullptr;
    if (has_res) rpre = *reinterpret_cast<const bf16x8*>(p.residual + p.cmap(row) * p.ldr + col);
    float acc[8] = {0.f, 0.f, 0.f, 0.f, 0.f, 0.f, 0.f, 0.f};
    if (p.split_k <= 8) {
        f32x4 a[8], b[8];
#pragma unroll
        for (int sp = 0; sp < 8; ++sp) {
            const float* wp = p.ws + ((int64_t)min(sp, p.split_k - 1) * p.M + row) * p.N + col;
            a[sp] = *reinterpret_cast<const f32x4*>(wp);
            b[sp] = *reinterpret_cast<const f32x4*>(wp + 4);
        }
#pragma unroll
        for (int sp = 0; sp < 8; ++sp) {
            const float m = sp < p.split_k ? 1.0f : 0.0f;
            acc[0] += m * a[sp][0]; acc[1] += m * a[sp][1]; acc[2] += m * a[sp][2]; acc[3] += m * a[sp][3];
            acc[4] += m * b[sp][0]; acc[5] += m * b[sp][1]; acc[6] += m * b[sp][2]; acc[7] += m * b[sp][3];
        }
    } else {
        for (int sp = 0; sp < p.split_k; ++sp) {
            const float* wp = p.ws + ((int64_t)sp * p.M + row) * p.N + col;
            const f32x4 a = *reinterpret_cast<const f32x4*>(wp), b = *reinterpret_cast<const f32x4*>(wp + 4);
            acc[0] += a[0]; acc[1] += a[1]; acc[2] += a[2]; acc[3] += a[3];
            acc[4] += b[0]; acc[5] += b[1]; acc[6] += b[2]; acc[7] += b[3];
        }
    }
    if (live) epilogue8(p, acc, row, col, 0, 0, 0, p.C, false, has_res ? &rpre : nullptr);
    float x[8];
#pragma unroll
    for (int e = 0; e < 8; ++e) x[e] = live ? rbf(acc[e]) : 0.f;
    float y[8];
    if constexpr (KIND == 1) {
        float ss = 0.f;
#pragma unroll
        for (int e = 0; e < 8; ++e) ss += x[e] * x[e];
        const float rstd = rsqrtf(block_sum<4>(ss, red) / (float)p.N + p.norm_eps);
#pragma unroll
        for (int e = 0; e < 8; ++e) y[e] = (x[e] * rstd) * (1.0f + wv[e]);
    } else {
        float sm = 0.f;
#pragma unroll
        for (int e = 0; e < 8; ++e) sm += x[e];
        const float mean = block_sum<4>(sm, red) / (float)p.N;
        float vs = 0.f;
#pragma unroll
        for (int e = 0; e < 8; ++e) {
            const float d = x[e] - mean;
            vs += live ? d * d : 0.f;
        }
        const float rstd = rsqrtf(block_sum<4>(vs, red) / (float)p.N + p.norm_eps);
#pragma unroll
        for (int e = 0; e < 8; ++e) y[e] = (x[e] - mean) * rstd * wv[e] + bv[e];
    }
    if (live) {
        bf16x8 o;
#pragma unroll
        for (int e = 0; e < 8; ++e) o[e] = f2bf(y[e]);
        *reinterpret_cast<bf16x8*>(p.norm_out + (int64_t)row * p.N + col) = o;
    }
}

constexpr int layout_bit(bool a_kc, bool b_kc) { return 1 << (2 * a_kc + b_kc); }
constexpr int L_NT = layout_bit(true, true), L_NN = layout_bit(true, false), L_TT = layout_bit(false, true), L_TN = layout_bit(false, false);
constexpr int L_ALL = L_NT | L_NN | L_TT | L_TN;

template <int LAYOUTS, int WM, int WN, int MT, int NT, bool PP, int NS = 2, int BKT = 64, int SCH = 0>
int launch_cfg(const kai0_gemm_desc* d, GemmArgs& p, int batch, hipStream_t s) {
    constexpr int TBM = WM * MT * 16, TBN = WN * NT * 16;
    constexpr int LDS = NS * (TBM + TBN) * BKT * 2;
    p.tiles_m = (d->M + TBM - 1) / TBM;
    p.tiles_n = (p.N + TBN - 1) / TBN;
    dim3 grid(p.tiles_m * p.tiles_n, batch * p.split_k, 1), block(WM * WN * 64, 1, 1);
#define KAI0_LAUNCH(AK, BK_)                                                                                      \
    if constexpr ((LAYOUTS & layout_bit(AK, BK_)) != 0)                                                          \
        if ((d->a_kc != 0) == AK && (d->b_kc != 0) == BK_) {                                                      \
            static bool attr_set = false;                                                                         \
            auto kern = gemm_bf16_kernel<AK, BK_, WM, WN, MT, NT, PP, NS, BKT, SCH>;                              \
            if (!attr_set) {                                                                                      \
                hipError_t e = hipFuncSetAttribute((const void*)kern, hipFuncAttributeMaxDynamicSharedMemorySize, LDS); \
                if (e != hipSuccess) {                                                                            \
                    kai0_set_error("kai0_gemm_bf16: cannot reserve %d B of LDS: %s", LDS, hipGetErrorString(e));  \
                    return -2;                                                                                    \
                }                                                                                                 \
                attr_set = true;                                                                                  \
            }                                                                                                     \
            hipLaunchKernelGGL(kern, grid, block, LDS, s, p);                                                     \
            return 0;                                                                                             \
        }
    KAI0_LAUNCH(true, true)
    KAI0_LAUNCH(true, false)
    KAI0_LAUNCH(false, true)
    KAI0_LAUNCH(false, false)
#undef KAI0_LAUNCH
    kai0_set_error("kai0_gemm_bf16: the %d x %d tile configuration (%d waves, %d stages) is not built for a_kc=%d b_kc=%d", TBM, TBN,
                   WM * WN, NS, d->a_kc, d->b_kc);
    return -3;
}

}

#ifdef KAI0_PS_TRACE
KAI0_API int kai0_debug_ps_trace(long long* host_out) {
    return (int)hipMemcpyFromSymbol(host_out, HIP_SYMBOL(g_ps_trace), sizeof(long long) * 256 * 8);
}
#endif

static int gemm_validate(const kai0_gemm_desc* d) {
    KAI0_REQUIRE(d != nullptr, "kai0_gemm_bf16: null descriptor");
    KAI0_REQUIRE(d->M > 0 && d->N > 0 && d->K > 0, "kai0_gemm_bf16: empty problem M=%d N=%d K=%d", d->M, d->N,
                 d->K);
    KAI0_REQUIRE(d->A && d->B && d->C, "kai0_gemm_bf16: null operand");
    KAI0_REQUIRE((d->lda % 8) == 0 && (d->ldb % 8) == 0 && (d->ldc % 8) == 0,
                 "kai0_gemm_bf16: leading dims must be multiples of 8 (lda=%lld ldb=%lld ldc=%lld)",
                 (long long)d->lda, (long long)d->ldb, (long long)d->ldc);
    KAI0_REQUIRE((d->N % 8) == 0 || (d->b_kc && d->ldc >= ((d->N + 7) & ~7) && !d->bias && !d->gate && !d->residual &&
                                     !d->pre_out && !d->accumulate),
                 "kai0_gemm_bf16: N=%d not a multiple of 8 needs b_kc, padded C rows and a plain epilogue", d->N);
    KAI0_REQUIRE((d->K % 8) == 0 || (!d->a_kc && !d->b_kc), "kai0_gemm_bf16: K=%d must be a multiple of 8 for "
                 "K-contiguous operands", d->K);
    KAI0_REQUIRE(d->a_kc || (d->M % 8) == 0, "kai0_gemm_bf16: M=%d must be a multiple of 8 when A is [K][M]",
                 d->M);
    KAI0_REQUIRE(((uintptr_t)d->A % 16) == 0 && ((uintptr_t)d->B % 16) == 0 && ((uintptr_t)d->C % 16) == 0,
                 "kai0_gemm_bf16: operands must be 16-byte aligned");
    KAI0_REQUIRE(d->batch <= 1 || (((d->sA1 | d->sA2 | d->sB1 | d->sB2) & 7) == 0 && ((d->sC1 | d->sC2) & (d->out_f32 ? 3 : 7)) == 0),
                 "kai0_gemm_bf16: batch strides must be multiples of 8 elements (16 B)");
    KAI0_REQUIRE(d->gate == nullptr || d->gate_rpb > 0, "kai0_gemm_bf16: gate needs gate_rpb > 0");
    KAI0_REQUIRE(d->act >= 0 && d->act <= 7, "kai0_gemm_bf16: unknown act %d", d->act);
    KAI0_REQUIRE(d->persist >= 0 && d->persist <= 2 && d->small_w8 >= 0 && d->small_w8 <= 2 && d->general_epilogue >= 0 &&
                     d->general_epilogue <= 1,
                 "kai0_gemm_bf16: hook out of range (persist=%d, small_w8=%d: 0..2; general_epilogue=%d: 0..1)", d->persist, d->small_w8,
                 d->general_epilogue);
    KAI0_REQUIRE(d->act != 7 || (d->rope_cos && d->rope_sin && d->rope_half == 128 && d->rope_n_end > 0 && (d->rope_n_end % 256) == 0 &&
                                 d->rope_n_end <= d->N && (d->N % 128) == 0 && d->a_kc && d->b_kc && d->batch <= 1 && d->split_k <= 1 &&
                                 !d->out_f32 && !d->accumulate && !d->bias && !d->gate && !d->residual && !d->pre_out &&
                                 (d->scale == 0.0f || d->scale == 1.0f) && d->b_rpb == 0 && ((uintptr_t)d->rope_cos % 16) == 0 &&
                                 ((uintptr_t)d->rope_sin % 16) == 0),
                 "kai0_gemm_bf16: act=7 (RoPE epilogue) needs bf16 cos / sin tables [M][128], rope_n_end %% 256 == 0, N %% 128 == 0, K-contiguous "
                 "operands, one batch entry, no split-K, a plain bf16 output");
    KAI0_REQUIRE(d->act != 6 || (d->B2 && d->a_kc && d->b_kc && d->batch <= 1 && d->split_k <= 1 && !d->out_f32 && !d->accumulate &&
                                 d->nseg == 0 && !d->bias && !d->gate && !d->residual && (d->scale == 0.0f || d->scale == 1.0f) &&
                                 (d->N % 32) == 0 && d->b_rpb == 0 && ((uintptr_t)d->B2 % 16) == 0),
                 "kai0_gemm_bf16: act=6 (GeGLU pair) needs B2 = up weight, K-contiguous operands, N %% 32 == 0, one batch entry, a "
                 "plain bf16 output");
    KAI0_REQUIRE(d->norm_kind == 0 ||
                     ((d->norm_kind == 1 || d->norm_kind == 2) && d->split_k > 1 && d->norm_out && d->norm_w && (d->norm_kind == 1 || d->norm_b) &&
                      d->batch <= 1 && !d->out_f32 && d->nseg == 0 && (d->N % 8) == 0 && d->N <= 2048 && d->act == 0 && !d->gate &&
                      !d->rowvec && ((uintptr_t)d->norm_out % 16) == 0 && ((uintptr_t)d->norm_w % 16) == 0),
                 "kai0_gemm_bf16: a fused norm (norm_kind=%d) needs split_k > 1, norm_out / norm_w (/ norm_b), one batch entry, a plain "
                 "bf16 output with N %% 8 == 0, N <= 2048, no activation / gate", d->norm_kind);
    KAI0_REQUIRE(d->act != 5 || (d->aux1 && !d->out_f32 && !d->accumulate && d->nseg == 0 && (d->N % 8) == 0),
                 "kai0_gemm_bf16: act=5 (fused GELU backward) needs aux1 = pre-activation, plain bf16 output");
    KAI0_REQUIRE(d->act != 4 || (d->aux1 && d->rowvec && !d->out_f32 && !d->accumulate && d->nseg == 0 && (d->N % 8) == 0),
                 "kai0_gemm_bf16: act=4 (fused softmax backward) needs aux1 = P, rowvec = D, plain bf16 output");
    KAI0_REQUIRE(d->act < 2 || d->act >= 4 || ((d->pre_out || d->act == 2) && d->aux1 && (d->act == 2 || d->aux2) && !d->out_f32 && (d->N % 8) == 0),
                 "kai0_gemm_bf16: act=%d (fused GeGLU) needs pre_out and aux inputs, bf16 output", d->act);
    KAI0_REQUIRE(d->nseg >= 0 && d->nseg <= 3, "kai0_gemm_bf16: nseg=%d", d->nseg);
    if (d->nseg > 0) {
        KAI0_REQUIRE(!d->out_f32 && !d->accumulate && (d->batch <= 1) && (d->act < 2 || d->act == 7) && !d->pre_out && (d->N % 8) == 0,
                     "kai0_gemm_bf16: column segments need a plain bf16 epilogue, batch 1");
        KAI0_REQUIRE(d->act != 4, "kai0_gemm_bf16: column segments and act=4 are exclusive");
        for (int i = 0; i < d->nseg; ++i)
            KAI0_REQUIRE(d->seg[i].dst && (d->seg[i].ld % 8) == 0 && (d->seg[i].n_begin % 8) == 0 &&
                             ((uintptr_t)d->seg[i].dst % 16) == 0 && d->seg[i].n_begin == (i ? d->seg[i].n_begin : 0) &&
                             (i == 0 || d->seg[i].n_begin > d->seg[i - 1].n_begin),
                         "kai0_gemm_bf16: segment %d (dst, ld %% 8, ascending n_begin %% 8, first at 0)", i);
    }
    {
        const int64_t a_rows = d->a_rpb ? ((int64_t)((d->a_kc ? d->M : d->K) / d->a_rpb) + 1) * d->a_bs + d->a_off
                                        : (d->a_kc ? d->M : d->K);
        const int64_t b_rows = d->b_rpb ? ((int64_t)((d->b_kc ? d->N : d->K) / d->b_rpb) + 1) * d->b_bs + d->b_off
                                        : (d->b_kc ? d->N : d->K);
        KAI0_REQUIRE(a_rows * d->lda * 2 < (int64_t)0x7FFF0000 && b_rows * d->ldb * 2 < (int64_t)0x7FFF0000,
                     "kai0_gemm_bf16: an operand spans more than 2 GiB per batch entry (A %lld rows, B %lld rows)",
                     (long long)a_rows, (long long)b_rows);
    }
    if (d->split_k > 1) {
        const int batch = d->batch > 0 ? d->batch : 1;
        KAI0_REQUIRE(d->workspace != nullptr && d->workspace_bytes >= (int64_t)batch * d->split_k * d->M * d->N * 4,
                     "kai0_gemm_bf16: split_k=%d needs a workspace of batch*split*M*N*4 bytes", d->split_k);
        KAI0_REQUIRE((d->N % 8) == 0, "kai0_gemm_bf16: split_k needs N %% 8 == 0");
    }
    return 0;
}

static kai0_gemm_plan_t gemm_select(const kai0_gemm_desc* d) {
    kai0_gemm_plan_t pl{};
    const int batch = d->batch > 0 ? d->batch : 1;
    const int split = d->split_k > 1 ? d->split_k : 1;
    const int N = d->act == 6 ? 2 * d->N : d->N;
    const int k_chunk = split > 1 ? ((d->K + split - 1) / split + BK - 1) / BK * BK : d->K;
    const int64_t big_tiles = (int64_t)((d->M + 255) / 256) * ((N + 255) / 256) * batch * split;
    const bool big = d->act != 7 && big_tiles >= 160 && d->K >= 256;
    const int64_t small_blocks = (int64_t)((d->M + 127) / 128) * ((N + 127) / 128) * batch * split;
    const bool deep = small_blocks <= 256 && k_chunk >= 256;
    const bool w8 = !big && d->a_kc && d->b_kc && (d->act <= 1 || d->act == 7) && (d->small_w8 == 2 || (d->small_w8 == 0 && deep));
    const int persist = d->persist == 1 ? 0 : (d->persist == 2 ? 2 : 1);
    const bool ps_ok = persist && big && d->a_kc && d->b_kc && batch == 1 && split == 1 &&
                       big_tiles >= (persist == 2 ? 512 : 2048) &&
                       (d->K % 8) == 0 && !d->rowvec && d->a_rpb == 0 && d->b_rpb == 0;
    const bool ps_rule = N >= 8192 || d->K >= 8192;
    pl.tile = big ? 256 : 128;
    pl.waves = big || w8 ? 8 : 4;
    if (ps_ok && (persist == 2 || ps_rule)) pl.loop = KAI0_GEMM_LOOP_PERSISTENT;
    else if (big && d->a_kc && d->b_kc) pl.loop = KAI0_GEMM_LOOP_QUADRANT;
    else if (big && !d->a_kc && !d->b_kc) pl.loop = KAI0_GEMM_LOOP_RING;
    else if (big) pl.loop = KAI0_GEMM_LOOP_PLAIN2;
    else if (w8 || deep) pl.loop = KAI0_GEMM_LOOP_PLAIN4;
    else pl.loop = KAI0_GEMM_LOOP_PLAIN2;
    pl.tiles_m = (d->M + pl.tile - 1) / pl.tile;
    pl.tiles_n = (N + pl.tile - 1) / pl.tile;
    pl.k_chunk = k_chunk;
    pl.simple_epilogue = big && SIMPLE_EPILOGUE_APPLIES(d->general_epilogue == 0, d->act, split, d->gate, d->out_f32,
                                                        (d->scale == 0.0f ? 1.0f : d->scale), d->c_rpb, N);
    return pl;
}

KAI0_API int kai0_gemm_plan_size(void) { return (int)sizeof(kai0_gemm_plan_t); }

KAI0_API int kai0_gemm_plan(const kai0_gemm_desc* d, kai0_gemm_plan_t* out) {
    KAI0_REQUIRE(out != nullptr, "kai0_gemm_plan: null result");
    if (int rc = gemm_validate(d)) return rc;
    *out = gemm_select(d);
    return 0;
}

KAI0_API int kai0_gemm_bf16(const kai0_gemm_desc* d, kai0_stream_t stream) {
    if (int rc = gemm_validate(d)) return rc;
    const int batch = d->batch > 0 ? d->batch : 1;
    GemmArgs p;
    p.A = (const bf16_t*)d->A;
    p.B = (const bf16_t*)d->B;
    p.C = d->C;
    p.M = d->M; p.N = d->act == 6 ? 2 * d->N : d->N; p.K = d->K;
    p.B2 = (const bf16_t*)d->B2;
    p.pre_out2 = (bf16_t*)d->pre_out2;
    p.norm_out = (bf16_t*)d->norm_out;
    p.norm_w = d->norm_w;
    p.norm_b = (const bf16_t*)d->norm_b;
    p.norm_eps = d->norm_eps;
    p.norm_kind = d->norm_kind;
    p.rope_cos = (const bf16_t*)d->rope_cos;
    p.rope_sin = (const bf16_t*)d->rope_sin;
    p.rope_half = d->rope_half;
    p.rope_n_end = d->rope_n_end;
    p.lda = d->lda; p.ldb = d->ldb; p.ldc = d->ldc;
    p.batch_inner = d->batch_inner > 0 ? d->batch_inner : 1;
    p.sA1 = d->sA1; p.sA2 = d->sA2; p.sB1 = d->sB1; p.sB2 = d->sB2; p.sC1 = d->sC1; p.sC2 = d->sC2;
    p.amap = RowMap{d->a_rpb, d->a_bs, d->a_off};
    p.bmap = RowMap{d->b_rpb, d->b_bs, d->b_off};
    p.cmap = RowMap{d->c_rpb, d->c_bs, d->c_off};
    p.bias = d->bias; p.bias_f32 = d->bias_f32;
    p.scale = d->scale == 0.0f ? 1.0f : d->scale;
    p.act = d->act; p.out_f32 = d->out_f32;
    p.pre_out = (bf16_t*)d->pre_out;
    p.aux1 = (const bf16_t*)d->aux1;
    p.aux2 = (const bf16_t*)d->aux2;
    p.gate = (const bf16_t*)d->gate; p.gate_rpb = d->gate_rpb; p.gate_ld = d->gate_ld;
    p.accumulate = d->accumulate;
    p.residual = (const bf16_t*)d->residual; p.ldr = d->ldr; p.sR1 = d->sR1; p.sR2 = d->sR2;
#ifdef KAI0_ABLATE
    static const int ablate = [] { const char* e = getenv("KAI0_GEMM_ABLATE"); return e ? atoi(e) : 0; }();
    p.ablate = ablate;
#else
    p.ablate = 0;
#endif
    p.nt_pre = 1;
    p.nt_c = d->c_nontemporal != 0;
    p.simple_epi = d->general_epilogue == 0;
    p.rowvec = d->rowvec; p.rv_s1 = d->rv_s1; p.rv_s2 = d->rv_s2; p.rv_ld = d->rv_ld;
    p.nseg = d->nseg;
    for (int i = 0; i < 3; ++i) {
        p.seg_dst[i] = i < d->nseg ? (bf16_t*)d->seg[i].dst : nullptr;
        p.seg_ld[i] = i < d->nseg ? d->seg[i].ld : 0;
        p.seg_begin[i] = i < d->nseg ? d->seg[i].n_begin : 0;
    }
    const kai0_gemm_plan_t pl = gemm_select(d);
    const int split = d->split_k > 1 ? d->split_k : 1;
    p.split_k = split;
    p.k_chunk = pl.k_chunk;
    p.ws = split > 1 ? (float*)d->workspace : nullptr;
    hipStream_t s = (hipStream_t)stream;
    int rc;
    if (pl.loop == KAI0_GEMM_LOOP_PERSISTENT) {
        const int64_t big_tiles = (int64_t)pl.tiles_m * pl.tiles_n;
        constexpr int LDS = 2 * 2 * 256 * 64 * 2 + 8 * 4096;
        struct PsDev { unsigned int* ctr = nullptr; int cus = 0; };
        static PsDev ps_dev[64];
        static std::atomic<unsigned> next_slot{0};
        int dv = 0;
        KAI0_REQUIRE(hipGetDevice(&dv) == hipSuccess && dv >= 0 && dv < 64, "kai0_gemm_bf16: hipGetDevice");
        PsDev& pd = ps_dev[dv];
        if (pd.ctr == nullptr) {
            void* sym = nullptr;
            hipError_t e = hipGetSymbolAddress(&sym, HIP_SYMBOL(g_ps_ctr));
            if (e == hipSuccess) e = hipFuncSetAttribute((const void*)gemm_nt_persistent_kernel, hipFuncAttributeMaxDynamicSharedMemorySize, LDS);
            hipDeviceProp_t pr;
            if (e == hipSuccess) e = hipGetDeviceProperties(&pr, dv);
            KAI0_REQUIRE(e == hipSuccess, "kai0_gemm_bf16: persistent kernel setup failed: %s", hipGetErrorString(e));
            pd.cus = pr.multiProcessorCount > 0 ? pr.multiProcessorCount : 256;
            pd.ctr = (unsigned int*)sym;
        }
        unsigned int* ctr_base = pd.ctr;
        p.tiles_m = (d->M + 255) / 256;
        p.tiles_n = (p.N + 255) / 256;
        const int nblk = (int)std::min<int64_t>(big_tiles, pd.cus);
        unsigned int* ctr = ctr_base + (size_t)(next_slot.fetch_add(1) % PS_SLOTS) * 16;
        hipLaunchKernelGGL(gemm_nt_persistent_kernel, dim3(nblk), dim3(512), LDS, s, p, ctr);
        return kai0_check_launch("kai0_gemm_bf16 (persistent)");
    }
    if (pl.tile == 256 && pl.loop == KAI0_GEMM_LOOP_QUADRANT) rc = launch_cfg<L_NT, 2, 4, 8, 4, true, 2, 64, 1>(d, p, batch, s);
    else if (pl.tile == 256 && pl.loop == KAI0_GEMM_LOOP_RING) rc = launch_cfg<L_TN, 2, 4, 8, 4, true, 4, 32, 3>(d, p, batch, s);
    else if (pl.tile == 256) rc = launch_cfg<L_NN | L_TT, 2, 4, 8, 4, false>(d, p, batch, s);
    else if (pl.waves == 8) rc = launch_cfg<L_NT, 4, 2, 2, 4, false, 4>(d, p, batch, s);
    else if (pl.loop == KAI0_GEMM_LOOP_PLAIN4) rc = launch_cfg<L_ALL, 2, 2, 4, 4, false, 4>(d, p, batch, s);
    else rc = launch_cfg<L_ALL, 2, 2, 4, 4, false>(d, p, batch, s);
    if (rc) return rc;
    rc = kai0_check_launch("kai0_gemm_bf16");
    if (rc || split == 1) return rc;
    if (d->norm_kind != 0) {
        if (d->norm_kind == 1) hipLaunchKernelGGL(splitk_reduce_norm_kernel<1>, dim3(d->M), dim3(256), 0, s, p);
        else hipLaunchKernelGGL(splitk_reduce_norm_kernel<2>, dim3(d->M), dim3(256), 0, s, p);
        return kai0_check_launch("kai0_gemm_bf16(split-K reduce + norm)");
    }
    const int64_t items = (int64_t)d->M * (d->N / 8);
    int rb = (int)((items + 255) / 256);
    if (rb > 2048) rb = 2048;
    hipLaunchKernelGGL(splitk_reduce_kernel, dim3(rb, batch, 1), dim3(256), 0, s, p);
    return kai0_check_launch("kai0_gemm_bf16(split-K reduce)");
}
```

### kai0_amd/ops.py

```python

from __future__ import annotations

import contextlib
import ctypes as C
import os
import math

import torch

from . import _lib
from ._lib import AttnBwdDesc, AttnDesc, GemmDesc

BF16 = torch.bfloat16
F32 = torch.float32

NORM_PARTIAL_BLOCKS = 512
COLSUM_BLOCKS = 256


def _stream() -> int:
    return torch.cuda.current_stream().cuda_stream


def _p(t: torch.Tensor | None) -> int | None:
    return None if t is None else t.data_ptr()


def _chk(t: torch.Tensor, dtype, name: str) -> None:
    if not t.is_cuda:
        raise _lib.Kai0HipError(f"{name}: expected a CUDA (HIP) tensor; the product path has no CPU fallback")
    if t.dtype != dtype:
        raise TypeError(f"{name}: expected {dtype}, got {t.dtype}")
    if not t.is_contiguous():
        raise ValueError(f"{name}: expected a contiguous tensor")


GEMM_TUNING = {"persist": {"0": 1, "2": 2}.get(os.environ.get("KAI0_GEMM_PERSIST", "1"), 0), "general_epilogue": 0,
               "small_w8": {"0": 1, "2": 2}.get(os.environ.get("KAI0_GEMM_W8", "1"), 0)}


@contextlib.contextmanager
def gemm_tuning(**kw):
    unknown = set(kw) - set(GEMM_TUNING)
    if unknown:
        raise KeyError(f"gemm_tuning: unknown hook(s) {sorted(unknown)}")
    old = dict(GEMM_TUNING)
    GEMM_TUNING.update(kw)
    try:
        yield
    finally:
        GEMM_TUNING.update(old)


def gemm(
    A: torch.Tensor, B: torch.Tensor, out: torch.Tensor, *, M: int, N: int, K: int, a_kc: bool = True,
    b_kc: bool = True, lda: int, ldb: int, ldc: int, batch: int = 1, batch_inner: int = 1,
    sA=(0, 0), sB=(0, 0), sC=(0, 0), a_map=None, b_map=None, c_map=None, bias: torch.Tensor | None = None,
    scale: float = 1.0, act: int = 0, pre_out: torch.Tensor | None = None, gate: torch.Tensor | None = None,
    gate_rpb: int = 0, gate_ld: int = 0, residual: torch.Tensor | None = None, ldr: int = 0, sR=(0, 0),
    accumulate: bool = False, a_off_elems: int = 0, b_off_elems: int = 0, c_off_elems: int = 0, split_k: int = 1,
    aux1: torch.Tensor | None = None, aux2: torch.Tensor | None = None, segs=None, rowvec=None, rv=(0, 0, 1),
    B2: torch.Tensor | None = None, pre_out2: torch.Tensor | None = None, norm=None, nt_out: bool = False, rope=None,
    _plan: "_lib.GemmPlan | None" = None,
) -> torch.Tensor:
    for t in (A, B, out):
        if not t.is_cuda:
            raise _lib.Kai0HipError("gemm: expected CUDA (HIP) tensors; the product path has no CPU fallback")
    if A.dtype != BF16 or B.dtype != BF16:
        raise TypeError(f"gemm: bf16 operands expected, got {A.dtype} / {B.dtype}")
    d = GemmDesc()
    d.A = A.data_ptr() + 2 * a_off_elems
    d.B = B.data_ptr() + 2 * b_off_elems
    out_f32 = out.dtype == F32
    d.C = out.data_ptr() + (4 if out_f32 else 2) * c_off_elems
    d.M, d.N, d.K = M, N, K
    d.a_kc, d.b_kc = int(a_kc), int(b_kc)
    d.lda, d.ldb, d.ldc = lda, ldb, ldc
    d.batch, d.batch_inner = batch, batch_inner
    d.sA1, d.sA2 = sA
    d.sB1, d.sB2 = sB
    d.sC1, d.sC2 = sC
    if a_map:
        d.a_rpb, d.a_bs, d.a_off = a_map
    if b_map:
        d.b_rpb, d.b_bs, d.b_off = b_map
    if c_map:
        d.c_rpb, d.c_bs, d.c_off = c_map
    if bias is not None:
        d.bias = bias.data_ptr()
        d.bias_f32 = int(bias.dtype == F32)
    d.scale = scale
    d.act = act
    d.out_f32 = int(out_f32)
    d.pre_out = _p(pre_out)
    d.aux1, d.aux2 = _p(aux1), _p(aux2)
    if rope is not None:
        rc, rs, half, n_end = rope
        if rc.dtype != BF16 or rs.dtype != BF16 or not rc.is_contiguous() or not rs.is_contiguous() or rc.shape != (M, half) or rs.shape != (M, half):
            raise TypeError("gemm: rope tables must be contiguous bf16 [M, half]")
        d.rope_cos, d.rope_sin, d.rope_half, d.rope_n_end = rc.data_ptr(), rs.data_ptr(), half, n_end
    if B2 is not None:
        if B2.dtype != BF16 or not B2.is_cuda:
            raise TypeError("gemm: B2 must be a bf16 HIP tensor")
        d.B2 = B2.data_ptr()
    d.pre_out2 = _p(pre_out2)
    if gate is not None:
        d.gate = gate.data_ptr()
        d.gate_rpb = gate_rpb
        d.gate_ld = gate_ld
    if residual is not None:
        d.residual = residual.data_ptr()
        d.ldr = ldr
        d.sR1, d.sR2 = sR
    d.accumulate = int(accumulate)
    d.c_nontemporal = int(nt_out)
    if rowvec is not None:
        if rowvec.dtype != F32:
            raise TypeError("gemm: rowvec must be f32")
        d.rowvec = rowvec.data_ptr()
        d.rv_s1, d.rv_s2, d.rv_ld = rv
    if segs:
        d.nseg = len(segs)
        for i, (dst, ld, nb) in enumerate(segs):
            d.seg[i].dst, d.seg[i].ld, d.seg[i].n_begin = dst.data_ptr(), ld, nb
    if split_k > 1 and _plan is not None:
        d.split_k, d.workspace, d.workspace_bytes = split_k, d.A, batch * split_k * M * N * 4
    elif split_k > 1:
        ws = _workspace(batch * split_k * M * N * 4, A.device)
        d.split_k, d.workspace, d.workspace_bytes = split_k, ws.data_ptr(), ws.numel()
    if norm is not None:
        kind, nout, nw, nb, neps = norm
        _chk(nout, BF16, "gemm: norm_out")
        _chk(nw, F32 if kind == 1 else BF16, "gemm: norm weight")
        d.norm_kind, d.norm_out, d.norm_w, d.norm_eps = int(kind), nout.data_ptr(), nw.data_ptr(), float(neps)
        if nb is not None:
            _chk(nb, BF16, "gemm: norm bias")
            d.norm_b = nb.data_ptr()
    d.persist, d.general_epilogue, d.small_w8 = GEMM_TUNING["persist"], GEMM_TUNING["general_epilogue"], GEMM_TUNING["small_w8"]
    if _plan is not None:
        _lib.call("kai0_gemm_plan", C.byref(d), C.byref(_plan))
        return out
    _lib.call("kai0_gemm_bf16", C.byref(d), _stream())
    return out


def gemm_plan(A: torch.Tensor, B: torch.Tensor, out: torch.Tensor, **kw) -> dict:
    pl = _lib.GemmPlan()
    gemm(A, B, out, _plan=pl, **kw)
    return {"tile": pl.tile, "waves": pl.waves, "loop": _lib.GEMM_LOOPS[pl.loop], "tiles_m": pl.tiles_m, "tiles_n": pl.tiles_n,
            "k_chunk": pl.k_chunk, "simple_epilogue": bool(pl.simple_epilogue)}


def skinny_split_k(N: int, K: int) -> int:
    if K % 512:
        raise _lib.Kai0HipError(f"skinny gemm: K={K} must be a multiple of 512")
    tiles = N // 32
    if K % 1024 == 0 and tiles * (K // 1024) >= 190:
        return K // 1024
    return K // 512


def skinny_workspace(M: int, N: int, split_k: int, device) -> torch.Tensor:
    return torch.empty((max(split_k, 1), M, N), dtype=F32, device=device)


def skinny_gemm(A, W, *, M: int, N: int, K: int, lda: int, ldw: int, mode: int = 0, pair_stride: int = 16, segs=None,
                split_k: int = 1, workspace=None, a_map=None, c_map=None, gate=None, gate_rpb: int = 0, gate_ld: int = 0,
                residual=None, ldr: int = 0, rope_cos=None, rope_sin=None, rope_half: int = 0, mod=None, mod_ld: int = 0,
                mod_rpb: int = 0, eps: float = 1e-6, w_packed: bool = False, rowsq_in=None, rowsq_parts: int = 0, cvec=None,
                rowsq_out=None):
    for t in (A, W):
        if not t.is_cuda or t.dtype != BF16:
            raise _lib.Kai0HipError("skinny_gemm: expected bf16 CUDA (HIP) tensors; the product path has no CPU fallback")
    d = _lib.SkinnyDesc()
    d.A, d.W, d.lda, d.ldw = A.data_ptr(), W.data_ptr(), lda, ldw
    d.M, d.N, d.K = M, N, K
    d.pair_stride, d.mode, d.split_k = pair_stride, mode, split_k
    d.w_packed = int(w_packed)
    if a_map:
        d.a_rpb, d.a_bs, d.a_off = a_map
    if c_map:
        d.c_rpb, d.c_bs, d.c_off = c_map
    d.nseg = len(segs or ())
    for i, (dst, ld, nb, ne, rope) in enumerate(segs or ()):
        if not dst.is_cuda or dst.dtype != BF16:
            raise _lib.Kai0HipError("skinny_gemm: destinations must be bf16 CUDA (HIP) tensors")
        d.seg[i].dst, d.seg[i].ld, d.seg[i].n_begin, d.seg[i].n_end, d.seg[i].rope = dst.data_ptr(), ld, nb, ne, int(rope)
    if gate is not None:
        d.gate, d.gate_rpb, d.gate_ld = gate.data_ptr(), gate_rpb, gate_ld
    if residual is not None:
        d.residual, d.ldr = residual.data_ptr(), ldr
    if rope_cos is not None:
        d.rope_cos, d.rope_sin, d.rope_half = rope_cos.data_ptr(), rope_sin.data_ptr(), rope_half
    if split_k > 1:
        if workspace is None or workspace.dtype != F32:
            raise _lib.Kai0HipError("skinny_gemm: split_k > 1 writes f32 partial products into `workspace` (skinny_workspace)")
        d.workspace, d.workspace_bytes = workspace.data_ptr(), workspace.numel() * 4
    elif split_k == -1 and workspace is not None:
        d.workspace, d.workspace_bytes = workspace.data_ptr(), workspace.numel() * workspace.element_size()
    if mod is not None:
        if mod.dtype != F32 or not mod.is_cuda or mod.stride(-1) != 1:
            raise _lib.Kai0HipError("skinny_gemm: mod must be an f32 CUDA (HIP) tensor with unit inner stride")
        d.mod, d.mod_ld, d.mod_rpb, d.eps = mod.data_ptr(), mod_ld, mod_rpb, eps
    if rowsq_in is not None:
        _chk(rowsq_in, F32, "rowsq_in")
        _chk(cvec, F32, "cvec")
        d.rowsq_in, d.cvec, d.rowsq_parts, d.rowsq_ld, d.eps = rowsq_in.data_ptr(), cvec.data_ptr(), rowsq_parts, rowsq_in.stride(0), eps
    if rowsq_out is not None:
        _chk(rowsq_out, F32, "rowsq_out")
        d.rowsq_out, d.rowsq_out_ld = rowsq_out.data_ptr(), rowsq_out.stride(0)
    _lib.call("kai0_gemm_skinny_bf16", C.byref(d), _stream())


def pack_skinny_weight(w: torch.Tensor) -> torch.Tensor:
    N, K = w.shape
    if N % 16 or K % 32:
        raise ValueError(f"pack_skinny_weight: N % 16 == 0 and K % 32 == 0 required, got {tuple(w.shape)}")
    return w.view(N // 16, 16, K // 32, 4, 8).permute(0, 2, 3, 1, 4).contiguous().view(N, K)


def adarms_combine(partials, gate_prev, residual, mod, rows_per_batch: int, eps: float = 1e-6):
    S, rows, D = partials.shape
    Bn = rows // rows_per_batch
    dev = partials.device
    x = torch.empty((rows, D), dtype=BF16, device=dev)
    y = torch.empty((rows, D), dtype=BF16, device=dev)
    gate = torch.empty((Bn, D), dtype=BF16, device=dev)
    _lib.call("kai0_adarms_combine", partials.data_ptr(), S, rows * D, _p(gate_prev), _p(residual), x.data_ptr(),
              mod.data_ptr(), y.data_ptr(), gate.data_ptr(), rows, rows_per_batch, D, eps, _stream())
    return x, y, gate


def attn_decode(Q, K, Vt, O, qcode, kcode, *, batch, rows, H, HD, Sk, q0, q_bs, k_bs, k_ld, k_rows, vt_bs, vt_ld, scale):
    for t in (Q, K, Vt, O):
        if not t.is_cuda or t.dtype != BF16:
            raise _lib.Kai0HipError("attn_decode: expected bf16 CUDA (HIP) tensors; the product path has no CPU fallback")
    ws = _workspace(int(_lib.load().kai0_attn_decode_workspace_bytes(batch, rows)), Q.device)
    _lib.call("kai0_attn_decode", Q.data_ptr(), K.data_ptr(), Vt.data_ptr(), O.data_ptr(), _p(qcode), _p(kcode), batch, rows,
              H, HD, Sk, q0, q_bs, k_bs, k_ld, k_rows, vt_bs, vt_ld, qcode.stride(0) if qcode is not None else 0,
              kcode.stride(0) if kcode is not None else 0, scale, ws.data_ptr(), ws.numel(), _stream())


def transpose_strided(src, dst, *, R, C, src_ld, dst_ld, batch=1, src_bs=0, dst_bs=0):
    _lib.call("kai0_transpose_strided_bf16", src.data_ptr(), dst.data_ptr(), R, C, src_ld, dst_ld, batch, src_bs, dst_bs,
              _stream())


def rowdot(a, b, D: int):
    if a.dtype != BF16 or b.dtype != BF16 or not a.is_contiguous() or not b.is_contiguous() or a.numel() != b.numel():
        raise _lib.Kai0HipError("rowdot: two contiguous bf16 tensors of the same size expected")
    rows = a.numel() // D
    out = torch.empty((rows,), dtype=F32, device=a.device)
    _lib.call("kai0_rowdot_bf16", a.data_ptr(), b.data_ptr(), out.data_ptr(), rows, D, _stream())
    return out


def rope_permutation(n_total: int, n_rope_end: int, half: int = 128) -> torch.Tensor:
    if half != 128 or n_rope_end % 256 != 0 or n_rope_end > n_total:
        raise ValueError("rope_permutation: head_dim 256 (half 128), rotated range a whole number of heads")
    pc = torch.arange(n_total)
    real = (pc // 256) * 256 + ((pc % 128) // 64) * 128 + 64 * ((pc % 256) // 128) + pc % 64
    return torch.where(pc < n_rope_end, real, pc)


def rope_table(pos, inv_freq, bf16: bool = False):
    pos = pos.contiguous()
    if pos.dtype != torch.int32:
        raise TypeError("rope_table: pos must be int32")
    rows, half = pos.numel(), inv_freq.numel()
    cos = torch.empty((rows, half), dtype=BF16 if bf16 else F32, device=pos.device)
    sin = torch.empty((rows, half), dtype=BF16 if bf16 else F32, device=pos.device)
    _lib.call("kai0_rope_table", pos.data_ptr(), inv_freq.data_ptr(), cos.data_ptr(), sin.data_ptr(), rows, half, int(bf16), _stream())
    return cos, sin


def prefix_codes(img_masks, lang_mask, n_img: int, Hs: int, n_state: int = 0):
    B, T = lang_mask.shape
    ms = [m.contiguous() for m in img_masks]
    lm = lang_mask.contiguous()
    for m in (*ms, lm):
        if m.dtype != torch.bool or not m.is_cuda:
            raise TypeError("prefix_codes: bool CUDA (HIP) masks expected")
    if any(m.shape != (B,) for m in ms):
        raise ValueError("prefix_codes: camera masks must be [B]")
    S = len(ms) * n_img + T + n_state + Hs
    q, k, p = (torch.empty((B, S), dtype=torch.int32, device=lm.device) for _ in range(3))
    ptrs = (C.c_void_p * len(ms))(*[m.data_ptr() for m in ms])
    if n_state:
        _lib.call("kai0_prefix_state_codes", C.addressof(ptrs), len(ms), lm.data_ptr(), B, n_img, T, n_state, Hs, q.data_ptr(), k.data_ptr(),
                  p.data_ptr(), _stream())
        return q, k, p
    _lib.call("kai0_prefix_codes", C.addressof(ptrs), len(ms), lm.data_ptr(), B, n_img, T, Hs, q.data_ptr(), k.data_ptr(), p.data_ptr(), _stream())
    return q, k, p


_WS: dict = {}


def _workspace(nbytes: int, device) -> torch.Tensor:
    key = (device.index, _stream())
    ws = _WS.get(key)
    if ws is None or ws.numel() < nbytes:
        ws = torch.empty(max(nbytes, 64 << 20), dtype=torch.uint8, device=device)
# ... 433 lines not shown
        _chk(w, F32, "rmsnorm.w")
        rows, D = x.shape
        y = torch.empty_like(x)
        rstd = torch.empty((rows,), dtype=F32, device=x.device)
        _lib.call("kai0_rmsnorm_fwd", x.data_ptr(), w.data_ptr(), y.data_ptr(), rstd.data_ptr(), rows, D, eps, _stream())
        ctx.save_for_backward(x, w, rstd)
        return x.view_as(x), y

    @staticmethod
    def backward(ctx, dres, dy):
        x, w, rstd = ctx.saved_tensors
        rows, D = x.shape
        if dy is None:
            return dres, None, None
        dy = dy.contiguous()
        dres = dres.contiguous() if dres is not None else None
        dx = torch.empty_like(x)
        nb = NORM_PARTIAL_BLOCKS
        part = torch.empty((nb, D), dtype=F32, device=x.device)
        _lib.call("kai0_rmsnorm_bwd", dy.data_ptr(), x.data_ptr(), w.data_ptr(), rstd.data_ptr(), dx.data_ptr(),
                  part.data_ptr(), nb, _p(dres), rows, D, _stream())
        dw = None
        if ctx.needs_input_grad[1]:
            dw = _grad_dst(w, F32)
            _reduce_partials(w, part, nb, D, D, dw)
        return dx, _grad_ret(w, dw), None


def rmsnorm_res(x, w, eps=1e-6):
    return RMSNormFn.apply(x, w, eps)


def rmsnorm(x, w, eps=1e-6):
    return RMSNormFn.apply(x, w, eps)[1]


class AdaRMSFn(torch.autograd.Function):

    @staticmethod
    def forward(ctx, x, mod, rows_per_batch: int, eps: float):
        _chk(x, BF16, "adarms.x")
        _chk(mod, F32, "adarms.mod")
        rows, D = x.shape
        Bn = rows // rows_per_batch
        y = torch.empty_like(x)
        gate = torch.empty((Bn, D), dtype=BF16, device=x.device)
        rstd = torch.empty((rows,), dtype=F32, device=x.device)
        _lib.call("kai0_adarms_fwd", x.data_ptr(), mod.data_ptr(), y.data_ptr(), gate.data_ptr(), rstd.data_ptr(), rows,
                  rows_per_batch, D, eps, _stream())
        ctx.save_for_backward(x, mod, rstd)
        ctx.rpb = rows_per_batch
        return x.view_as(x), y, gate

    @staticmethod
    def backward(ctx, dres, dy, dgate):
        x, mod, rstd = ctx.saved_tensors
        rows, D = x.shape
        if dy is None:
            dy = torch.zeros_like(x)
        dy = dy.contiguous()
        dgate = dgate.contiguous() if dgate is not None else None
        dres = dres.contiguous() if dres is not None else None
        dx = torch.empty_like(x)
        dmod = torch.empty_like(mod)
        _lib.call("kai0_adarms_bwd", dy.data_ptr(), _p(dgate), x.data_ptr(), mod.data_ptr(), rstd.data_ptr(),
                  dx.data_ptr(), dmod.data_ptr(), _p(dres), rows, ctx.rpb, D, _stream())
        return dx, dmod, None, None


def adarms_res(x, mod, rows_per_batch, eps=1e-6):
    return AdaRMSFn.apply(x, mod, rows_per_batch, eps)


def adarms(x, mod, rows_per_batch, eps=1e-6):
    _, y, gate = AdaRMSFn.apply(x, mod, rows_per_batch, eps)
    return y, gate


class LayerNormFn(torch.autograd.Function):

    @staticmethod
    def forward(ctx, x, w, b, eps: float):
        _chk(x, BF16, "layernorm.x")
        rows, D = x.shape
        y = torch.empty_like(x)
        mean = torch.empty((rows,), dtype=F32, device=x.device)
        rstd = torch.empty((rows,), dtype=F32, device=x.device)
        _lib.call("kai0_layernorm_fwd", x.data_ptr(), w.data_ptr(), b.data_ptr(), y.data_ptr(), mean.data_ptr(),
                  rstd.data_ptr(), rows, D, eps, _stream())
        ctx.save_for_backward(x, w, b, mean, rstd)
        return x.view_as(x), y

    @staticmethod
    def backward(ctx, dres, dy):
        x, w, b, mean, rstd = ctx.saved_tensors
        if dy is None:
            return dres, None, None, None
        dy = dy.contiguous()
        dres = dres.contiguous() if dres is not None else None
        rows, D = x.shape
        dx = torch.empty_like(x)
        nb = NORM_PARTIAL_BLOCKS
        part = torch.empty((nb, 2 * D), dtype=F32, device=x.device)
        _lib.call("kai0_layernorm_bwd", dy.data_ptr(), x.data_ptr(), w.data_ptr(), mean.data_ptr(), rstd.data_ptr(),
                  dx.data_ptr(), part.data_ptr(), nb, _p(dres), rows, D, _stream())
        dw, db = _grad_dst(w, w.dtype), _grad_dst(b, b.dtype)
        _reduce_partials(w, part, nb, D, 2 * D, dw)
        _reduce_partials(b, part, nb, D, 2 * D, db, col0=D)
        return dx, _grad_ret(w, dw), _grad_ret(b, db), None


def layernorm_res(x, w, b, eps=1e-6):
    return LayerNormFn.apply(x, w, b, eps)


def layernorm(x, w, b, eps=1e-6):
    return LayerNormFn.apply(x, w, b, eps)[1]


class GegluFn(torch.autograd.Function):
    @staticmethod
    def forward(ctx, g, u):
        _chk(g, BF16, "geglu.g")
        _chk(u, BF16, "geglu.u")
        h = torch.empty_like(g)
        _lib.call("kai0_geglu_fwd", g.data_ptr(), u.data_ptr(), h.data_ptr(), g.numel(), _stream())
        ctx.save_for_backward(g, u)
        return h

    @staticmethod
    def backward(ctx, dh):
        g, u = ctx.saved_tensors
        dh = dh.contiguous()
        dg = torch.empty_like(g)
        du = torch.empty_like(u)
        _lib.call("kai0_geglu_bwd", dh.data_ptr(), g.data_ptr(), u.data_ptr(), dg.data_ptr(), du.data_ptr(), g.numel(),
                  _stream())
        return dg, du


def geglu(g, u):
    return GegluFn.apply(g, u)


_GEGLU_PAIR = True


def set_geglu_pair(on: bool) -> bool:
    global _GEGLU_PAIR
    old, _GEGLU_PAIR = _GEGLU_PAIR, bool(on)
    return old


class GegluMlpFn(torch.autograd.Function):

    @staticmethod
    def forward(ctx, x, wg, wu, wd, residual):
        _chk(x, BF16, "geglu_mlp.x")
        M, D = x.shape
        F = wg.shape[0]
        u = torch.empty((M, F), dtype=BF16, device=x.device)
        h = torch.empty((M, F), dtype=BF16, device=x.device)
        if _GEGLU_PAIR and F % 32 == 0:
            g = torch.empty((M, F), dtype=BF16, device=x.device)
            gemm(x, wg, h, M=M, N=F, K=D, lda=D, ldb=D, ldc=F, act=6, B2=wu, pre_out=g, pre_out2=u)
        else:
            g = linear_fwd(x, wg)
            gemm(x, wu, h, M=M, N=F, K=D, lda=D, ldb=D, ldc=F, act=2, pre_out=u, aux1=g, split_k=1)
        out = linear_fwd(h, wd, residual=residual)
        ctx.save_for_backward(x, wg, wu, wd, g, u, h)
        ctx.has_res = residual is not None
        return out

    @staticmethod
    def backward(ctx, dout):
        x, wg, wu, wd, g, u, h = ctx.saved_tensors
        dout = dout.contiguous()
        M, D = x.shape
        F = wg.shape[0]
        dev = x.device

        def wgrad(dy, inp, w, n, k):
            dw = _grad_dst(w, BF16)
            gemm(dy, inp, dw, M=n, N=k, K=M, a_kc=False, b_kc=False, lda=n, ldb=k, ldc=k, split_k=pick_split_k_wgrad(n, k, M), nt_out=True)
            return dw

        dwd = wgrad(dout, h, wd, D, F) if ctx.needs_input_grad[3] else None
        dg = torch.empty((M, F), dtype=BF16, device=dev)
        du = torch.empty((M, F), dtype=BF16, device=dev)
        wdt = transpose(wd)
        gemm(dout, wdt, dg, M=M, N=F, K=D, lda=D, ldb=D, ldc=F, act=3, pre_out=du, aux1=g, aux2=u)
        del wdt
        dwg = wgrad(dg, x, wg, F, D) if ctx.needs_input_grad[1] else None
        dwu = wgrad(du, x, wu, F, D) if ctx.needs_input_grad[2] else None
        dx = None
        if ctx.needs_input_grad[0]:
            dx = torch.empty((M, D), dtype=BF16, device=dev)
            wgt = transpose(wg)
            gemm(dg, wgt, dx, M=M, N=D, K=F, lda=F, ldb=F, ldc=D, split_k=1)
            wut = transpose(wu)
            gemm(du, wut, dx, M=M, N=D, K=F, lda=F, ldb=F, ldc=D, accumulate=True, split_k=1)
            del wgt, wut
        return dx, _grad_ret(wg, dwg), _grad_ret(wu, dwu), _grad_ret(wd, dwd), (dout if ctx.has_res else None)


_PAD_MLP_ROWS = True


class GeluMlpFn(torch.autograd.Function):

    @staticmethod
    def forward(ctx, x, w1, b1, w2, b2, residual):
        _chk(x, BF16, "gelu_mlp.x")
        M, D = x.shape
        F = w1.shape[0]
        ldh = round_up(F, 64) if _PAD_MLP_ROWS else F
        dev = x.device
        pre = torch.empty((M, ldh), dtype=BF16, device=dev)
        h = torch.empty((M, ldh), dtype=BF16, device=dev)
        gemm(x, w1, h, M=M, N=F, K=D, lda=D, ldb=D, ldc=ldh, bias=b1, act=1, pre_out=pre, split_k=1)
        out = torch.empty((M, w2.shape[0]), dtype=BF16, device=dev)
        gemm(h, w2, out, M=M, N=w2.shape[0], K=F, lda=ldh, ldb=F, ldc=w2.shape[0], bias=b2, residual=residual,
             ldr=w2.shape[0], split_k=pick_split_k(M, w2.shape[0], F))
        ctx.save_for_backward(x, w1, w2, pre, h)
        ctx.biases = (b1, b2)
        ctx.has_res = residual is not None
        return out

    @staticmethod
    def backward(ctx, dout):
        x, w1, w2, pre, h = ctx.saved_tensors
        b1, b2 = ctx.biases
        dout = dout.contiguous()
        M, D = x.shape
        F, Do = w1.shape[0], w2.shape[0]
        ldh = pre.shape[1]
        dev = x.device
        big = M >= 4096

        def colsum(dy, N, ld, b):
            return _bias_grads(dy, M, N, ld, [(b, 0, N)])[0]

        dw2 = db2 = dw1 = db1 = dx = None
        if ctx.needs_input_grad[3]:
            dw2 = _grad_dst(w2, BF16)
            gemm(dout, h, dw2, M=Do, N=F, K=M, a_kc=False, b_kc=False, lda=Do, ldb=ldh, ldc=F, split_k=pick_split_k_wgrad(Do, F, M), nt_out=True)
            dw2 = _grad_ret(w2, dw2)
        if b2 is not None and ctx.needs_input_grad[4]:
            db2 = colsum(dout, Do, Do, b2)
        dpre = torch.empty((M, ldh), dtype=BF16, device=dev)
        if big:
            w2t = transpose(w2)
            gemm(dout, w2t, dpre, M=M, N=F, K=Do, lda=Do, ldb=Do, ldc=ldh, act=5, aux1=pre)
            del w2t
        else:
            gemm(dout, w2, dpre, M=M, N=F, K=Do, a_kc=True, b_kc=False, lda=Do, ldb=F, ldc=ldh, act=5, aux1=pre)
        if ctx.needs_input_grad[1]:
            dw1 = _grad_dst(w1, BF16)
            gemm(dpre, x, dw1, M=F, N=D, K=M, a_kc=False, b_kc=False, lda=ldh, ldb=D, ldc=D, split_k=pick_split_k_wgrad(F, D, M), nt_out=True)
            dw1 = _grad_ret(w1, dw1)
        if b1 is not None and ctx.needs_input_grad[2]:
            db1 = colsum(dpre, F, ldh, b1)
        if ctx.needs_input_grad[0]:
            dx = torch.empty((M, D), dtype=BF16, device=dev)
            if big:
                w1t = transpose(w1)
                gemm(dpre, w1t, dx, M=M, N=D, K=F, lda=ldh, ldb=F, ldc=D)
                del w1t
            else:
                gemm(dpre, w1, dx, M=M, N=D, K=F, a_kc=True, b_kc=False, lda=ldh, ldb=D, ldc=D, split_k=pick_split_k(M, D, F))
        return dx, dw1, db1, dw2, db2, (dout if ctx.has_res else None)


def gelu_mlp(x, w1, b1, w2, b2, residual=None):
    return GeluMlpFn.apply(x, w1, b1, w2, b2, residual)


def geglu_mlp(x, wg, wu, wd, residual=None):
    return GegluMlpFn.apply(x, wg, wu, wd, residual)


class GatedResidualFn(torch.autograd.Function):

    @staticmethod
    def forward(ctx, x, y, gate, rows_per_batch: int):
        rows, D = x.shape
        out = torch.empty_like(x)
        _lib.call("kai0_gated_fwd", x.data_ptr(), y.data_ptr(), gate.data_ptr(), out.data_ptr(), rows, rows_per_batch, D,
                  _stream())
        ctx.save_for_backward(y, gate)
        ctx.rpb = rows_per_batch
        return out

    @staticmethod
    def backward(ctx, dout):
        y, gate = ctx.saved_tensors
        dout = dout.contiguous()
        rows, D = y.shape
        dy = torch.empty_like(y)
        dgate = torch.empty_like(gate)
        _lib.call("kai0_gated_bwd", dout.data_ptr(), y.data_ptr(), gate.data_ptr(), dy.data_ptr(), dgate.data_ptr(), rows,
                  ctx.rpb, D, _stream())
        return dout, dy, dgate, None


def gated_residual(x, y, gate, rows_per_batch):
    return GatedResidualFn.apply(x, y, gate, rows_per_batch)


class SiluF32Fn(torch.autograd.Function):
    @staticmethod
    def forward(ctx, x):
        _chk(x, F32, "silu.x")
        y = torch.empty_like(x)
        _lib.call("kai0_silu_fwd_f32", x.data_ptr(), y.data_ptr(), x.numel(), _stream())
        ctx.save_for_backward(x)
        return y

    @staticmethod
    def backward(ctx, dy):
        (x,) = ctx.saved_tensors
        dy = dy.contiguous()
        dx = torch.empty_like(x)
        _lib.call("kai0_silu_bwd_f32", dy.data_ptr(), x.data_ptr(), dx.data_ptr(), x.numel(), _stream())
        return dx


def silu_f32(x):
    return SiluF32Fn.apply(x)


class CastFn(torch.autograd.Function):

    @staticmethod
    def forward(ctx, x, to_bf16: bool):
        ctx.to_bf16 = to_bf16
        return cast(x, BF16 if to_bf16 else F32)

    @staticmethod
    def backward(ctx, dy):
        return cast(dy.contiguous(), F32 if ctx.to_bf16 else BF16), None


def cast(x: torch.Tensor, dtype) -> torch.Tensor:
    if x.dtype == dtype:
        return x
    y = torch.empty(x.shape, dtype=dtype, device=x.device)
# ... 590 lines not shown
```

Measured before the change: 69.17 samples/s.

## Emit transposed GEGLU MLP activations from GEMM epilogues for NT weight-gradient GEMMs

```diff
diff --git a/include/kai0hip.h b/include/kai0hip.h
--- a/include/kai0hip.h
+++ b/include/kai0hip.h
@@ -61,6 +61,10 @@
     const void* rope_cos;
     const void* rope_sin;
     int32_t rope_half, rope_n_end;
+    void* ct;
+    int64_t ldct;
+    void* ct2;
+    int64_t ldct2;
     int32_t persist, general_epilogue, small_w8, _pad3;
 } kai0_gemm_desc;
 
@@ -79,7 +83,7 @@
     int32_t tiles_m, tiles_n;
     int32_t k_chunk;
     int32_t simple_epilogue;
-    int32_t _pad;
+    int32_t transposed_store;
 } kai0_gemm_plan_t;
 int kai0_gemm_plan(const kai0_gemm_desc* d, kai0_gemm_plan_t* out);
 int kai0_gemm_plan_size(void);
diff --git a/kai0_amd/_lib.py b/kai0_amd/_lib.py
--- a/kai0_amd/_lib.py
+++ b/kai0_amd/_lib.py
@@ -41,6 +41,7 @@
         ("B2", c_p), ("pre_out2", c_p),
         ("norm_out", c_p), ("norm_w", c_p), ("norm_b", c_p), ("norm_eps", C.c_float), ("norm_kind", C.c_int32),
         ("rope_cos", c_p), ("rope_sin", c_p), ("rope_half", C.c_int32), ("rope_n_end", C.c_int32),
+        ("ct", c_p), ("ldct", c_i64), ("ct2", c_p), ("ldct2", c_i64),
         ("persist", C.c_int32), ("general_epilogue", C.c_int32), ("small_w8", C.c_int32), ("_pad3", C.c_int32),
     ]
 
@@ -48,7 +49,7 @@
 class GemmPlan(C.Structure):
 
     _fields_ = [("tile", C.c_int32), ("waves", C.c_int32), ("loop", C.c_int32), ("tiles_m", C.c_int32), ("tiles_n", C.c_int32),
-                ("k_chunk", C.c_int32), ("simple_epilogue", C.c_int32), ("_pad", C.c_int32)]
+                ("k_chunk", C.c_int32), ("simple_epilogue", C.c_int32), ("transposed_store", C.c_int32)]
 
 
 GEMM_LOOPS = ("plain2", "plain4", "quadrant", "ring", "persistent")
diff --git a/kai0_amd/csrc/gemm_bf16.hip b/kai0_amd/csrc/gemm_bf16.hip
--- a/kai0_amd/csrc/gemm_bf16.hip
+++ b/kai0_amd/csrc/gemm_bf16.hip
@@ -71,6 +71,9 @@
     const bf16_t* rope_cos;
     const bf16_t* rope_sin;
     int rope_half, rope_n_end;
+    bf16_t* ct;
+    bf16_t* ct2;
+    int64_t ldct, ldct2;
 };
 
 typedef __attribute__((ext_vector_type(4))) int i32x4_t;
@@ -83,6 +86,57 @@
 __device__ __forceinline__ void store_pre8(bf16_t* dst, bf16x8 v, int nt) {
     if (nt) __builtin_nontemporal_store(v, reinterpret_cast<bf16x8*>(dst));
     else *reinterpret_cast<bf16x8*>(dst) = v;
+}
+
+__device__ __forceinline__ void geglu_bwd8(const float (&v)[8], bf16x8 g, bf16x8 u, bf16x8& du, bf16x8& dg) {
+#pragma unroll
+    for (int e = 0; e < 8; e += 2) {
+        const f32x2 dh = rbf2(f32x2{v[e], v[e + 1]});
+        f32x2 gl, gr;
+        gelu_tanh_both2(f32x2{bf2f(g[e]), bf2f(g[e + 1])}, gl, gr);
+        const f32x2 a = dh * rbf2(gl);
+        const f32x2 b = rbf2(dh * f32x2{bf2f(u[e]), bf2f(u[e + 1])}) * gr;
+        du[e] = f2bf(a[0]);
+        du[e + 1] = f2bf(a[1]);
+        dg[e] = f2bf(b[0]);
+        dg[e + 1] = f2bf(b[1]);
+    }
+}
+
+template <int COLS>
+__device__ __forceinline__ void ct_pass(char* img, bf16x8 v, int lane, bf16_t* ct, int64_t ldct, int row0, int col0, int M, int ncols) {
+    constexpr int LD = COLS == 32 ? 32 : 96;
+    constexpr int CB = COLS / 16;
+    const int wr = COLS == 32 ? lane >> 2 : lane >> 3, wc = (COLS == 32 ? lane & 3 : lane & 7) * 8;
+    asm volatile("" ::: "memory");
+    *reinterpret_cast<bf16x8*>(img + (wr * LD + wc) * 2) = v;
+    asm volatile("s_waitcnt lgkmcnt(0)" ::: "memory");
+    __builtin_amdgcn_wave_barrier();
+    const int l15 = lane & 15, g = lane >> 4, cb = g % CB, ro = g / CB;
+    const char* q = img + ((8 * ro + (l15 >> 2)) * LD + 16 * cb + 4 * (l15 & 3)) * 2;
+    const bf16x4 lo = __builtin_amdgcn_ds_read_tr16_b64_v4bf16((LDS_PTR(bf16x4))(q));
+    const bf16x4 hi = __builtin_amdgcn_ds_read_tr16_b64_v4bf16((LDS_PTR(bf16x4))(q + 4 * LD * 2));
+    asm volatile("s_waitcnt lgkmcnt(0)" ::: "memory");
+    __builtin_amdgcn_wave_barrier();
+    const int col = col0 + 16 * cb + l15, row = row0 + 8 * ro;
+    if (col < ncols && row < M) *reinterpret_cast<bf16x8*>(ct + (int64_t)col * ldct + row) = __builtin_shufflevector(lo, hi, 0, 1, 2, 3, 4, 5, 6, 7);
+}
+
+__device__ __forceinline__ void ct_round(const char* img, int lane, bf16_t* ct, int64_t ldct, int row0, int col0, int M, int ncols) {
+    asm volatile("s_waitcnt lgkmcnt(0)" ::: "memory");
+    __builtin_amdgcn_wave_barrier();
+    const int l15 = lane & 15, g = lane >> 4;
+#pragma unroll
+    for (int j = 0; j < 4; ++j) {
+        const int cb = j & 1, oct = (j >> 1) * 4 + g;
+        const char* q = img + ((8 * oct + (l15 >> 2)) * 32 + 16 * cb + 4 * (l15 & 3)) * 2;
+        const bf16x4 lo = __builtin_amdgcn_ds_read_tr16_b64_v4bf16((LDS_PTR(bf16x4))(q));
+        const bf16x4 hi = __builtin_amdgcn_ds_read_tr16_b64_v4bf16((LDS_PTR(bf16x4))(q + 4 * 64));
+        const int col = col0 + 16 * cb + l15, row = row0 + 8 * oct;
+        if (col < ncols && row < M) *reinterpret_cast<bf16x8*>(ct + (int64_t)col * ldct + row) = __builtin_shufflevector(lo, hi, 0, 1, 2, 3, 4, 5, 6, 7);
+    }
+    asm volatile("s_waitcnt lgkmcnt(0)" ::: "memory");
+    __builtin_amdgcn_wave_barrier();
 }
 
 __device__ __forceinline__ void epilogue8(const GemmArgs& p, float (&v)[8], int row, int ccol, int64_t cz, int64_t rz,
@@ -220,8 +274,9 @@
     __builtin_amdgcn_sched_barrier(0);
 }
 
-template <bool A_KC, bool B_KC, int WM, int WN, int MT, int NT, bool PP, int NS = 2, int BKT = 64, int SCH = 0>
+template <bool A_KC, bool B_KC, int WM, int WN, int MT, int NT, bool PP, int NS = 2, int BKT = 64, int SCH = 0, bool CT = false>
 __global__ __launch_bounds__(WM * WN * 64, (WM * WN * 64) / 256) void gemm_bf16_kernel(const GemmArgs p) {
+    static_assert(!CT || (MT == 8 && A_KC && B_KC && SCH == 1), "the transposed store is built for the 256 x 256 NT quadrant tile only");
     static_assert(PP ? (WM == 2 && WN == 4 && MT == 8 && ((SCH == 1 && NS == 2 && BKT == 64) || (SCH == 3 && NS == 4 && BKT == 32)))
                      : (SCH == 0 && NS >= 2 && BKT == 64),
                   "K loops: plain multi-stage (SCH 0, 64 deep), quadrant (SCH 1: 256x256x64, 2 stages), ring (SCH 3: 256x256x32, 4 slots)");
@@ -633,6 +688,7 @@
     const bool plain_fast = p.act <= 1 && p.split_k == 1 && (p.bias != nullptr || p.residual != nullptr) && p.gate == nullptr &&
                             !p.accumulate && !p.out_f32 && p.nseg == 0 && (N_ALIGNED8(p.N));
     const bool simple_fast = MT == 8 && SIMPLE_EPILOGUE_APPLIES(p.simple_epi, p.act, p.split_k, p.gate, p.out_f32, p.scale, p.cmap.rpb, p.N);
+    constexpr bool CT_TILE = CT;
     auto epi_half = [&](auto hc) {
         constexpr int h = decltype(hc)::value;
         if constexpr (((MT == 4 && WM == 2) || (MT == 2 && WM == 4)) && WN == 2 && A_KC && B_KC) if (p.act == 7) {
@@ -702,25 +758,59 @@
                 const float* sp = slab + lr * 64 + (lane & 3) * 8;
                 const f32x4 g0 = *reinterpret_cast<const f32x4*>(sp), g1 = *reinterpret_cast<const f32x4*>(sp + 4);
                 const f32x4 u0 = *reinterpret_cast<const f32x4*>(sp + 32), u1 = *reinterpret_cast<const f32x4*>(sp + 36);
-                if (row >= p.M || !ocol_ok) continue;
-                const float gv[8] = {g0[0], g0[1], g0[2], g0[3], g1[0], g1[1], g1[2], g1[3]};
-                const float uv[8] = {u0[0], u0[1], u0[2], u0[3], u1[0], u1[1], u1[2], u1[3]};
-                bf16x8 gb, ub, hb;
-#pragma unroll
-                for (int e = 0; e < 8; e += 2) {
-                    const f32x2 gr = rbf2(f32x2{gv[e], gv[e + 1]}), ur = rbf2(f32x2{uv[e], uv[e + 1]});
-                    const f32x2 hv = rbf2(gelu_tanh2(gr)) * ur;
-                    gb[e] = f2bf(gr[0]);
-                    gb[e + 1] = f2bf(gr[1]);
-                    ub[e] = f2bf(ur[0]);
-                    ub[e + 1] = f2bf(ur[1]);
-                    hb[e] = f2bf(hv[0]);
-                    hb[e + 1] = f2bf(hv[1]);
-                }
-                const int64_t o = cz + p.cmap(row) * p.ldc + ocol;
-                *reinterpret_cast<bf16x8*>(cb + o) = hb;
-                if (p.pre_out != nullptr) store_pre8(p.pre_out + o, gb, p.nt_pre);
-                if (p.pre_out2 != nullptr) store_pre8(p.pre_out2 + o, ub, p.nt_pre);
+                bf16x8 hb = bf16x8{};
+                if (row < p.M && ocol_ok) {
+                    const float gv[8] = {g0[0], g0[1], g0[2], g0[3], g1[0], g1[1], g1[2], g1[3]};
+                    const float uv[8] = {u0[0], u0[1], u0[2], u0[3], u1[0], u1[1], u1[2], u1[3]};
+                    bf16x8 gb, ub;
+#pragma unroll
+                    for (int e = 0; e < 8; e += 2) {
+                        const f32x2 gr = rbf2(f32x2{gv[e], gv[e + 1]}), ur = rbf2(f32x2{uv[e], uv[e + 1]});
+                        const f32x2 hv = rbf2(gelu_tanh2(gr)) * ur;
+                        gb[e] = f2bf(gr[0]);
+                        gb[e + 1] = f2bf(gr[1]);
+                        ub[e] = f2bf(ur[0]);
+                        ub[e + 1] = f2bf(ur[1]);
+                        hb[e] = f2bf(hv[0]);
+                        hb[e + 1] = f2bf(hv[1]);
+                    }
+                    const int64_t o = cz + p.cmap(row) * p.ldc + ocol;
+                    *reinterpret_cast<bf16x8*>(cb + o) = hb;
+                    if (p.pre_out != nullptr) store_pre8(p.pre_out + o, gb, p.nt_pre);
+                    if (p.pre_out2 != nullptr) store_pre8(p.pre_out2 + o, ub, p.nt_pre);
+                }
+                if constexpr (CT_TILE)
+                    ct_pass<32>(reinterpret_cast<char*>(slab + it * 16 * 64), hb, lane, p.ct, p.ldct, row_base(h) + it * 16,
+                                (n0 >> 1) + wn * 32, p.M, p.N >> 1);
+            }
+            asm volatile("s_waitcnt lgkmcnt(0)" ::: "memory");
+            __builtin_amdgcn_wave_barrier();
+            return;
+        }
+        if constexpr (CT_TILE) if (p.act == 0) {
+#pragma unroll
+            for (int i = 0; i < 4; ++i)
+#pragma unroll
+                for (int j = 0; j < 4; ++j)
+#pragma unroll
+                    for (int r = 0; r < 4; ++r) slab[(i * 16 + 4 * g + r) * 64 + j * 16 + l15] = acc[h * 4 + i][j][r];
+            asm volatile("s_waitcnt lgkmcnt(0)" ::: "memory");
+            __builtin_amdgcn_wave_barrier();
+            bf16_t* cb = reinterpret_cast<bf16_t*>(p.C);
+            const int rbase = row_base(h) + (lane >> 3);
+#pragma unroll
+            for (int it = 0; it < 8; ++it) {
+                const int row = rbase + it * 8;
+                const float* sp = slab + (it * 8 + (lane >> 3)) * 64 + (lane & 7) * 8;
+                const f32x4 v0 = *reinterpret_cast<const f32x4*>(sp), v1 = *reinterpret_cast<const f32x4*>(sp + 4);
+                const float v[8] = {v0[0], v0[1], v0[2], v0[3], v1[0], v1[1], v1[2], v1[3]};
+                bf16x8 ov = bf16x8{};
+                if (row < p.M && col_ok) {
+#pragma unroll
+                    for (int e = 0; e < 8; ++e) ov[e] = f2bf(rbf(v[e]));
+                    store_pre8(cb + cz + p.cmap(row) * p.ldc + ccol, ov, p.nt_c);
+                }
+                ct_pass<64>(reinterpret_cast<char*>(slab + it * 8 * 64), ov, lane, p.ct, p.ldct, row_base(h) + it * 8, n0 + wn * 64, p.M, p.N);
             }
             asm volatile("s_waitcnt lgkmcnt(0)" ::: "memory");
             __builtin_amdgcn_wave_barrier();
@@ -759,6 +849,19 @@
                 const f32x4 v0 = *reinterpret_cast<const f32x4*>(sp);
                 const f32x4 v1 = *reinterpret_cast<const f32x4*>(sp + 4);
                 const float v[8] = {v0[0], v0[1], v0[2], v0[3], v1[0], v1[1], v1[2], v1[3]};
+                if constexpr (CT_TILE) {
+                    bf16x8 du = bf16x8{}, dgv = bf16x8{};
+                    if (row < p.M && col_ok) {
+                        const int64_t o = cz + p.cmap(row) * p.ldc + ccol;
+                        geglu_bwd8(v, s0[it], s1[it], du, dgv);
+                        *reinterpret_cast<bf16x8*>(p.pre_out + o) = du;
+                        *reinterpret_cast<bf16x8*>(cb + o) = dgv;
+                    }
+                    char* img = reinterpret_cast<char*>(slab + it * 8 * 64);
+                    ct_pass<64>(img, dgv, lane, p.ct, p.ldct, row_base(h) + it * 8, n0 + wn * 64, p.M, p.N);
+                    ct_pass<64>(img, du, lane, p.ct2, p.ldct2, row_base(h) + it * 8, n0 + wn * 64, p.M, p.N);
+                    continue;
+                }
                 if (row >= p.M || !col_ok) continue;
                 const int64_t o = cz + p.cmap(row) * p.ldc + ccol;
                 bf16x8 ov;
@@ -1033,6 +1136,7 @@
 #define PS_STAMP(i) do { } while (0)
 #endif
 
+template <bool CT>
 __global__ __launch_bounds__(512, 1) void gemm_nt_persistent_kernel(const GemmArgs p, unsigned int* __restrict__ ctr) {
     constexpr int TBM = 256, TBN = 256, A_TILE = TBM * BK * 2, STAGE = 2 * A_TILE, GROUP = 4, MT = 8;
     extern __shared__ __attribute__((aligned(16))) char smem[];
@@ -1242,6 +1346,7 @@
             const int ocol = (n0c >> 1) + wn * 32 + (lane & 3) * 8;
             const bool ocol_ok = ocol < (p.N >> 1);
             bf16_t* cb = reinterpret_cast<bf16_t*>(p.C);
+            bf16x8 hk[4];
 #pragma unroll
             for (int ti = 0; ti < MT; ++ti) {
                 to_slab(ti);
@@ -1249,10 +1354,11 @@
                 const float* sp = slab + (lane >> 2) * 64 + (lane & 3) * 8;
                 const f32x4 g0 = *reinterpret_cast<const f32x4*>(sp), g1 = *reinterpret_cast<const f32x4*>(sp + 4);
                 const f32x4 u0 = *reinterpret_cast<const f32x4*>(sp + 32), u1 = *reinterpret_cast<const f32x4*>(sp + 36);
+                bf16x8 hb = bf16x8{};
                 if (row < p.M && ocol_ok) {
                     const float gv[8] = {g0[0], g0[1], g0[2], g0[3], g1[0], g1[1], g1[2], g1[3]};
                     const float uv[8] = {u0[0], u0[1], u0[2], u0[3], u1[0], u1[1], u1[2], u1[3]};
-                    bf16x8 gb, ub, hb;
+                    bf16x8 gb, ub;
 #pragma unroll
                     for (int e = 0; e < 8; e += 2) {
                         const f32x2 gr = rbf2(f32x2{gv[e], gv[e + 1]}), ur = rbf2(f32x2{uv[e], uv[e + 1]});
@@ -1266,12 +1372,23 @@
                     if (p.pre_out != nullptr) store_pre8(p.pre_out + o, gb, p.nt_pre);
                     if (p.pre_out2 != nullptr) store_pre8(p.pre_out2 + o, ub, p.nt_pre);
                 }
+                if constexpr (CT) {
+                    hk[ti & 3] = hb;
+                    if ((ti & 3) == 3) {
+                        char* img = reinterpret_cast<char*>(slab);
+                        asm volatile("" ::: "memory");
+#pragma unroll
+                        for (int k = 0; k < 4; ++k) *reinterpret_cast<bf16x8*>(img + ((k * 16 + (lane >> 2)) * 32 + (lane & 3) * 8) * 2) = hk[k];
+                        ct_round(img, lane, p.ct, p.ldct, m0c + wm * 128 + (ti - 3) * 16, (n0c >> 1) + wn * 32, p.M, p.N >> 1);
+                    }
+                }
             }
         } else if (fused_fast) {
             bf16_t* cb = reinterpret_cast<bf16_t*>(p.C);
 #pragma unroll
             for (int h = 0; h < 2; ++h) {
                 bf16x8 s0[8], s1[8];
+                bf16x8 rdg[8], rdu[8];
                 float ds[8];
                 const int rbase = m0c + wm * 128 + h * 64 + (lane >> 3);
 #pragma unroll
@@ -1297,6 +1414,17 @@
                         const float* sp = slab + (it2 * 8 + (lane >> 3)) * 64 + (lane & 7) * 8;
                         const f32x4 v0 = *reinterpret_cast<const f32x4*>(sp), v1 = *reinterpret_cast<const f32x4*>(sp + 4);
                         const float v[8] = {v0[0], v0[1], v0[2], v0[3], v1[0], v1[1], v1[2], v1[3]};
+                        if constexpr (CT) {
+                            rdg[it] = bf16x8{};
+                            rdu[it] = bf16x8{};
+                            if (row < p.M && col_ok) {
+                                const int64_t o = p.cmap(row) * p.ldc + ccol;
+                                geglu_bwd8(v, s0[it], s1[it], rdu[it], rdg[it]);
+                                *reinterpret_cast<bf16x8*>(p.pre_out + o) = rdu[it];
+                                *reinterpret_cast<bf16x8*>(cb + o) = rdg[it];
+                            }
+                            continue;
+                        }
                         if (row >= p.M || !col_ok) continue;
                         const int64_t o = p.cmap(row) * p.ldc + ccol;
                         bf16x8 ov;
@@ -1340,6 +1468,39 @@
                         }
                         *reinterpret_cast<bf16x8*>(cb + o) = ov;
                     }
+                }
+                if constexpr (CT) {
+                    char* img = reinterpret_cast<char*>(slab);
+#pragma unroll
+                    for (int r = 0; r < 4; ++r) {
+                        asm volatile("" ::: "memory");
+                        if (((lane & 7) >> 2) == (r & 1)) {
+#pragma unroll
+                            for (int it = 0; it < 8; ++it)
+                                *reinterpret_cast<bf16x8*>(img + ((it * 8 + (lane >> 3)) * 32 + (lane & 3) * 8) * 2) = r < 2 ? rdg[it] : rdu[it];
+                        }
+                        ct_round(img, lane, r < 2 ? p.ct : p.ct2, r < 2 ? p.ldct : p.ldct2, m0c + wm * 128 + h * 64, n0c + wn * 64 + (r & 1) * 32, p.M, p.N);
+                    }
+                }
+            }
+        } else if (CT && p.act == 0) {
+            bf16_t* cb = reinterpret_cast<bf16_t*>(p.C);
+#pragma unroll
+            for (int ti = 0; ti < MT; ++ti) {
+                to_slab(ti);
+#pragma unroll
+                for (int it2 = 0; it2 < 2; ++it2) {
+                    const int row0 = m0c + wm * 128 + ti * 16 + it2 * 8, row = row0 + (lane >> 3);
+                    const float* sp = slab + (it2 * 8 + (lane >> 3)) * 64 + (lane & 7) * 8;
+                    const f32x4 v0 = *reinterpret_cast<const f32x4*>(sp), v1 = *reinterpret_cast<const f32x4*>(sp + 4);
+                    const float v[8] = {v0[0], v0[1], v0[2], v0[3], v1[0], v1[1], v1[2], v1[3]};
+                    bf16x8 ov = bf16x8{};
+                    if (row < p.M && col_ok) {
+#pragma unroll
+                        for (int e = 0; e < 8; ++e) ov[e] = f2bf(rbf(v[e]));
+                        store_pre8(cb + p.cmap(row) * p.ldc + ccol, ov, p.nt_c);
+                    }
+                    ct_pass<64>(reinterpret_cast<char*>(slab + it2 * 8 * 64), ov, lane, p.ct, p.ldct, row0, n0c + wn * 64, p.M, p.N);
                 }
             }
         } else if (simple_fast) {
@@ -1605,7 +1766,7 @@
 constexpr int L_NT = layout_bit(true, true), L_NN = layout_bit(true, false), L_TT = layout_bit(false, true), L_TN = layout_bit(false, false);
 constexpr int L_ALL = L_NT | L_NN | L_TT | L_TN;
 
-template <int LAYOUTS, int WM, int WN, int MT, int NT, bool PP, int NS = 2, int BKT = 64, int SCH = 0>
+template <int LAYOUTS, int WM, int WN, int MT, int NT, bool PP, int NS = 2, int BKT = 64, int SCH = 0, bool CT = false>
 int launch_cfg(const kai0_gemm_desc* d, GemmArgs& p, int batch, hipStream_t s) {
     constexpr int TBM = WM * MT * 16, TBN = WN * NT * 16;
     constexpr int LDS = NS * (TBM + TBN) * BKT * 2;
@@ -1616,7 +1777,7 @@
     if constexpr ((LAYOUTS & layout_bit(AK, BK_)) != 0)                                                          \
         if ((d->a_kc != 0) == AK && (d->b_kc != 0) == BK_) {                                                      \
             static bool attr_set = false;                                                                         \
-            auto kern = gemm_bf16_kernel<AK, BK_, WM, WN, MT, NT, PP, NS, BKT, SCH>;                              \
+            auto kern = gemm_bf16_kernel<AK, BK_, WM, WN, MT, NT, PP, NS, BKT, SCH, CT>;                             \
             if (!attr_set) {                                                                                      \
                 hipError_t e = hipFuncSetAttribute((const void*)kern, hipFuncAttributeMaxDynamicSharedMemorySize, LDS); \
                 if (e != hipSuccess) {                                                                            \
@@ -1645,6 +1806,8 @@
     return (int)hipMemcpyFromSymbol(host_out, HIP_SYMBOL(g_ps_trace), sizeof(long long) * 256 * 8);
 }
 #endif
+
+static kai0_gemm_plan_t gemm_select(const kai0_gemm_desc* d);
 
 static int gemm_validate(const kai0_gemm_desc* d) {
     KAI0_REQUIRE(d != nullptr, "kai0_gemm_bf16: null descriptor");
@@ -1721,6 +1884,21 @@
                      "kai0_gemm_bf16: split_k=%d needs a workspace of batch*split*M*N*4 bytes", d->split_k);
         KAI0_REQUIRE((d->N % 8) == 0, "kai0_gemm_bf16: split_k needs N %% 8 == 0");
     }
+    if (d->ct != nullptr || d->ct2 != nullptr) {
+        KAI0_REQUIRE(((d->act == 6 || d->act == 0) && d->ct && !d->ct2) || (d->act == 3 && d->ct && d->ct2),
+                     "kai0_gemm_bf16: a transposed store needs act=0 or act=6 with ct (no ct2), or act=3 with ct and ct2 (act=%d)", d->act);
+        KAI0_REQUIRE(d->split_k <= 1 && !d->out_f32 && d->nseg == 0 && d->c_rpb == 0 && d->batch <= 1,
+                     "kai0_gemm_bf16: a transposed store excludes split-K, an f32 output, column segments, an output row map and batches");
+        KAI0_REQUIRE((d->M % 8) == 0 && (d->ldct % 8) == 0 && d->ldct >= d->M && ((uintptr_t)d->ct % 16) == 0 &&
+                         (!d->ct2 || ((d->ldct2 % 8) == 0 && d->ldct2 >= d->M && ((uintptr_t)d->ct2 % 16) == 0)),
+                     "kai0_gemm_bf16: a transposed store needs M %% 8 == 0, ldct %% 8 == 0, ldct >= M and 16-byte aligned ct / ct2 (M=%d ldct=%lld "
+                     "ldct2=%lld)", d->M, (long long)d->ldct, (long long)d->ldct2);
+        KAI0_REQUIRE(d->act == 6 || (!d->bias && !d->gate && !d->residual && !d->accumulate && (d->scale == 0.0f || d->scale == 1.0f)),
+                     "kai0_gemm_bf16: a transposed store with act=0 / act=3 needs the plain form (no bias / gate / residual / accumulate / scale)");
+        KAI0_REQUIRE(d->act != 0 || ((d->N % 8) == 0 && !d->pre_out), "kai0_gemm_bf16: a transposed store with act=0 needs N %% 8 == 0 and no pre_out");
+        KAI0_REQUIRE(d->a_kc && d->b_kc && gemm_select(d).tile == 256,
+                     "kai0_gemm_bf16: a transposed store needs K-contiguous operands and a problem of the 256 x 256 tile (>= 160 tiles, K >= 256)");
+    }
     return 0;
 }
 
@@ -1753,6 +1931,7 @@
     pl.k_chunk = k_chunk;
     pl.simple_epilogue = big && SIMPLE_EPILOGUE_APPLIES(d->general_epilogue == 0, d->act, split, d->gate, d->out_f32,
                                                         (d->scale == 0.0f ? 1.0f : d->scale), d->c_rpb, N);
+    pl.transposed_store = d->ct != nullptr;
     return pl;
 }
 
@@ -1784,6 +1963,7 @@
     p.rope_sin = (const bf16_t*)d->rope_sin;
     p.rope_half = d->rope_half;
     p.rope_n_end = d->rope_n_end;
+    p.ct = (bf16_t*)d->ct; p.ct2 = (bf16_t*)d->ct2; p.ldct = d->ldct; p.ldct2 = d->ldct2;
     p.lda = d->lda; p.ldb = d->ldb; p.ldc = d->ldc;
     p.batch_inner = d->batch_inner > 0 ? d->batch_inner : 1;
     p.sA1 = d->sA1; p.sA2 = d->sA2; p.sB1 = d->sB1; p.sB2 = d->sB2; p.sC1 = d->sC1; p.sC2 = d->sC2;
@@ -1834,7 +2014,8 @@
         if (pd.ctr == nullptr) {
             void* sym = nullptr;
             hipError_t e = hipGetSymbolAddress(&sym, HIP_SYMBOL(g_ps_ctr));
-            if (e == hipSuccess) e = hipFuncSetAttribute((const void*)gemm_nt_persistent_kernel, hipFuncAttributeMaxDynamicSharedMemorySize, LDS);
+            if (e == hipSuccess) e = hipFuncSetAttribute((const void*)gemm_nt_persistent_kernel<false>, hipFuncAttributeMaxDynamicSharedMemorySize, LDS);
+            if (e == hipSuccess) e = hipFuncSetAttribute((const void*)gemm_nt_persistent_kernel<true>, hipFuncAttributeMaxDynamicSharedMemorySize, LDS);
             hipDeviceProp_t pr;
             if (e == hipSuccess) e = hipGetDeviceProperties(&pr, dv);
             KAI0_REQUIRE(e == hipSuccess, "kai0_gemm_bf16: persistent kernel setup failed: %s", hipGetErrorString(e));
@@ -1846,10 +2027,12 @@
         p.tiles_n = (p.N + 255) / 256;
         const int nblk = (int)std::min<int64_t>(big_tiles, pd.cus);
         unsigned int* ctr = ctr_base + (size_t)(next_slot.fetch_add(1) % PS_SLOTS) * 16;
-        hipLaunchKernelGGL(gemm_nt_persistent_kernel, dim3(nblk), dim3(512), LDS, s, p, ctr);
+        if (p.ct != nullptr) hipLaunchKernelGGL(gemm_nt_persistent_kernel<true>, dim3(nblk), dim3(512), LDS, s, p, ctr);
+        else hipLaunchKernelGGL(gemm_nt_persistent_kernel<false>, dim3(nblk), dim3(512), LDS, s, p, ctr);
         return kai0_check_launch("kai0_gemm_bf16 (persistent)");
     }
-    if (pl.tile == 256 && pl.loop == KAI0_GEMM_LOOP_QUADRANT) rc = launch_cfg<L_NT, 2, 4, 8, 4, true, 2, 64, 1>(d, p, batch, s);
+    if (pl.tile == 256 && pl.loop == KAI0_GEMM_LOOP_QUADRANT && p.ct != nullptr) rc = launch_cfg<L_NT, 2, 4, 8, 4, true, 2, 64, 1, true>(d, p, batch, s);
+    else if (pl.tile == 256 && pl.loop == KAI0_GEMM_LOOP_QUADRANT) rc = launch_cfg<L_NT, 2, 4, 8, 4, true, 2, 64, 1>(d, p, batch, s);
     else if (pl.tile == 256 && pl.loop == KAI0_GEMM_LOOP_RING) rc = launch_cfg<L_TN, 2, 4, 8, 4, true, 4, 32, 3>(d, p, batch, s);
     else if (pl.tile == 256) rc = launch_cfg<L_NN | L_TT, 2, 4, 8, 4, false>(d, p, batch, s);
     else if (pl.waves == 8) rc = launch_cfg<L_NT, 4, 2, 2, 4, false, 4>(d, p, batch, s);
diff --git a/kai0_amd/ops.py b/kai0_amd/ops.py
--- a/kai0_amd/ops.py
+++ b/kai0_amd/ops.py
@@ -61,6 +61,7 @@
     accumulate: bool = False, a_off_elems: int = 0, b_off_elems: int = 0, c_off_elems: int = 0, split_k: int = 1,
     aux1: torch.Tensor | None = None, aux2: torch.Tensor | None = None, segs=None, rowvec=None, rv=(0, 0, 1),
     B2: torch.Tensor | None = None, pre_out2: torch.Tensor | None = None, norm=None, nt_out: bool = False, rope=None,
+    ct: torch.Tensor | None = None, ldct: int = 0, ct2: torch.Tensor | None = None, ldct2: int = 0,
     _plan: "_lib.GemmPlan | None" = None,
 ) -> torch.Tensor:
     for t in (A, B, out):
@@ -104,6 +105,10 @@
             raise TypeError("gemm: B2 must be a bf16 HIP tensor")
         d.B2 = B2.data_ptr()
     d.pre_out2 = _p(pre_out2)
+    for name, t in (("ct", ct), ("ct2", ct2)):
+        if t is not None and (t.dtype != BF16 or not t.is_cuda):
+            raise TypeError(f"gemm: {name} must be a bf16 HIP tensor")
+    d.ct, d.ldct, d.ct2, d.ldct2 = _p(ct), ldct, _p(ct2), ldct2
     if gate is not None:
         d.gate = gate.data_ptr()
         d.gate_rpb = gate_rpb
@@ -144,11 +149,17 @@
     return out
 
 
+_gemm = gemm
+
+
 def gemm_plan(A: torch.Tensor, B: torch.Tensor, out: torch.Tensor, **kw) -> dict:
     pl = _lib.GemmPlan()
-    gemm(A, B, out, _plan=pl, **kw)
-    return {"tile": pl.tile, "waves": pl.waves, "loop": _lib.GEMM_LOOPS[pl.loop], "tiles_m": pl.tiles_m, "tiles_n": pl.tiles_n,
+    _gemm(A, B, out, _plan=pl, **kw)
+    plan = {"tile": pl.tile, "waves": pl.waves, "loop": _lib.GEMM_LOOPS[pl.loop], "tiles_m": pl.tiles_m, "tiles_n": pl.tiles_n,
             "k_chunk": pl.k_chunk, "simple_epilogue": bool(pl.simple_epilogue)}
+    if kw.get("ct") is not None:
+        plan["transposed_store"] = bool(pl.transposed_store)
+    return plan
 
 
 def skinny_split_k(N: int, K: int) -> int:
@@ -888,6 +899,20 @@
     return old
 
 
+_MLP_WGRAD_NT = True
+_MLP_WGRAD_NT_MIN_ROWS = 4096
+
+
+def set_mlp_wgrad_nt(on: bool) -> bool:
+    global _MLP_WGRAD_NT
+    old, _MLP_WGRAD_NT = _MLP_WGRAD_NT, bool(on)
+    return old
+
+
+def _mlp_wgrad_nt(rows: int) -> bool:
+    return _MLP_WGRAD_NT and rows >= _MLP_WGRAD_NT_MIN_ROWS and rows % 8 == 0
+
+
 class GegluMlpFn(torch.autograd.Function):
 
     @staticmethod
@@ -897,15 +922,23 @@
         F = wg.shape[0]
         u = torch.empty((M, F), dtype=BF16, device=x.device)
         h = torch.empty((M, F), dtype=BF16, device=x.device)
-        if _GEGLU_PAIR and F % 32 == 0:
+        pair = _GEGLU_PAIR and F % 32 == 0
+        hT = None
+        if pair:
             g = torch.empty((M, F), dtype=BF16, device=x.device)
-            gemm(x, wg, h, M=M, N=F, K=D, lda=D, ldb=D, ldc=F, act=6, B2=wu, pre_out=g, pre_out2=u)
+            kw = dict(M=M, N=F, K=D, lda=D, ldb=D, ldc=F, act=6, B2=wu, pre_out=g, pre_out2=u)
+            if _mlp_wgrad_nt(M) and ctx.needs_input_grad[3] and gemm_plan(x, wg, h, **kw)["tile"] == 256:
+                hT = torch.empty((F, M), dtype=BF16, device=x.device)
+                kw.update(ct=hT, ldct=M)
+            gemm(x, wg, h, **kw)
         else:
             g = linear_fwd(x, wg)
             gemm(x, wu, h, M=M, N=F, K=D, lda=D, ldb=D, ldc=F, act=2, pre_out=u, aux1=g, split_k=1)
         out = linear_fwd(h, wd, residual=residual)
-        ctx.save_for_backward(x, wg, wu, wd, g, u, h)
+        ctx.save_for_backward(x, wg, wu, wd, g, u, h if hT is None else hT)
         ctx.has_res = residual is not None
+        ctx.nt_gate_up = pair and _mlp_wgrad_nt(M)
+        ctx.h_transposed = hT is not None
         return out
 
     @staticmethod
@@ -921,14 +954,36 @@
             gemm(dy, inp, dw, M=n, N=k, K=M, a_kc=False, b_kc=False, lda=n, ldb=k, ldc=k, split_k=pick_split_k_wgrad(n, k, M), nt_out=True)
             return dw
 
-        dwd = wgrad(dout, h, wd, D, F) if ctx.needs_input_grad[3] else None
+        def wgrad_nt(dyT, inpT, dw, n, k):
+            return gemm(dyT, inpT, dw, M=n, N=k, K=M, lda=M, ldb=M, ldc=k, split_k=pick_split_k_wgrad(n, k, M), nt_out=True)
+
+        dwd = None
+        if ctx.needs_input_grad[3]:
+            dwd = wgrad_nt(transpose(dout), h, _grad_dst(wd, BF16), D, F) if ctx.h_transposed else wgrad(dout, h, wd, D, F)
         dg = torch.empty((M, F), dtype=BF16, device=dev)
         du = torch.empty((M, F), dtype=BF16, device=dev)
         wdt = transpose(wd)
-        gemm(dout, wdt, dg, M=M, N=F, K=D, lda=D, ldb=D, ldc=F, act=3, pre_out=du, aux1=g, aux2=u)
+        kw = dict(M=M, N=F, K=D, lda=D, ldb=D, ldc=F, act=3, pre_out=du, aux1=g, aux2=u)
+        need_g, need_u = ctx.needs_input_grad[1], ctx.needs_input_grad[2]
+        dgduT = None
+        if ctx.nt_gate_up and need_g and need_u and gemm_plan(dout, wdt, dg, **kw)["tile"] == 256:
+            dgduT = torch.empty((2 * F, M), dtype=BF16, device=dev)
+            kw.update(ct=dgduT[:F], ldct=M, ct2=dgduT[F:], ldct2=M)
+        gemm(dout, wdt, dg, **kw)
         del wdt
-        dwg = wgrad(dg, x, wg, F, D) if ctx.needs_input_grad[1] else None
-        dwu = wgrad(du, x, wu, F, D) if ctx.needs_input_grad[2] else None
+        if dgduT is not None:
+            xT = transpose(x)
+            dwg, dwu = _grad_dst(wg, BF16), _grad_dst(wu, BF16)
+            both = _as_rows([dwg, dwu])
+            if both is not None:
+                wgrad_nt(dgduT, xT, both, 2 * F, D)
+            else:
+                wgrad_nt(dgduT[:F], xT, dwg, F, D)
+                wgrad_nt(dgduT[F:], xT, dwu, F, D)
+            del xT, dgduT
+        else:
+            dwg = wgrad(dg, x, wg, F, D) if need_g else None
+            dwu = wgrad(du, x, wu, F, D) if need_u else None
         dx = None
         if ctx.needs_input_grad[0]:
             dx = torch.empty((M, D), dtype=BF16, device=dev)
```

Result: faster. 70.16 samples/s (median of 6 runs) (+1.4%).
